# z3lx/waifu2x-tensorrt

Hardware: AMD Instinct MI355X
Metric: upscaled MPix/s, 1080p->4K swin_unet/art fp16 (higher is better)
Workload: dtype f16; 1 GPU; configs[2]: swin_unet/art scale4 noise3 batch4 tile256 fp16, 1920x1080 frame, blend=0.0625 (45 tiles, 12 batches); synthetic-weight graph of that architecture, frame resident in HBM; frames_per_rank=132, parallelism=frame-sharded x1, no collectives; timing barrier over gloo, mode=frames, tiles_per_network_pass=48, tile_groups_per_pass=2

## Files before the change

include/w2x/c_api.h:

```cpp
#ifndef W2X_C_API_H
#define W2X_C_API_H

#include <stddef.h>
#include <stdint.h>

#ifdef __cplusplus
extern "C" {
#endif

typedef struct w2x_engine w2x_engine;

enum { W2X_PRECISION_TF32 = 0, W2X_PRECISION_FP16 = 1, W2X_PRECISION_FP32 = 2 };

enum { W2X_RESIZE_BICUBIC = 0, W2X_RESIZE_BILINEAR = 1 };
enum { W2X_YUV_BT601 = 0, W2X_YUV_BT709 = 1, W2X_YUV_BT2020 = 2 };
enum { W2X_YUV_LIMITED = 0, W2X_YUV_FULL = 1 };

typedef struct w2x_build_config {
    int deviceId, precision;
    int minBatchSize, optBatchSize, maxBatchSize;
    int minChannels, optChannels, maxChannels;
    int minWidth, optWidth, maxWidth;
    int minHeight, optHeight, maxHeight;
} w2x_build_config;
// ... 17 lines not shown
int w2x_render(w2x_engine* e, const uint8_t* src, int rows, int cols, size_t src_step, uint8_t* dst, size_t dst_step);
int w2x_render16(w2x_engine* e, const uint16_t* src, int rows, int cols, size_t src_step, uint16_t* dst, size_t dst_step);
int w2x_render_resized(w2x_engine* e, const uint8_t* src, int rows, int cols, size_t src_step, uint8_t* dst, int dst_rows, int dst_cols, size_t dst_step, int filter);
int w2x_render16_resized(w2x_engine* e, const uint16_t* src, int rows, int cols, size_t src_step, uint16_t* dst, int dst_rows, int dst_cols, size_t dst_step, int filter);
int w2x_render_strip(w2x_engine* e, const uint8_t* src, int rows, int cols, size_t src_step, uint8_t* dst, size_t dst_step, int part, int parts);
int w2x_render_sharded(w2x_engine* const* engines, int count, const uint8_t* src, int rows, int cols, size_t src_step, uint8_t* dst, size_t dst_step);
int w2x_shard_plan(int in_w, int in_h, int out_w, int out_h, int tile_in, int tile_out, int scaling, double overlap_x, double overlap_y,
                   int part, int parts, int* out16);
int w2x_shard_compute(w2x_engine* e, const uint8_t* src, int rows, int cols, size_t src_step, int part, int parts);
const void* w2x_shard_slab(w2x_engine* e, size_t* bytes);
int w2x_shard_finish(w2x_engine* e, uint8_t* dst, int out_rows, int out_cols, size_t dst_step, int part, int parts, const void* const* slabs, const int* devices);
int w2x_ipc_export(const void* device_ptr, uint8_t* out64);
void* w2x_ipc_open(const uint8_t* handle64, int device);
void w2x_ipc_close(void* p);
int w2x_render_sequence(w2x_engine* e, const uint8_t* const* srcs, int rows, int cols, size_t src_step, uint8_t* const* dsts, size_t dst_step, int count);
int w2x_render_sequence_resized(w2x_engine* e, const uint8_t* const* srcs, int rows, int cols, size_t src_step, uint8_t* const* dsts, int dst_rows, int dst_cols, size_t dst_step,
                                int count, int filter);
int w2x_render_yuv(w2x_engine* e, const void* const* src_planes, const size_t* src_steps, int rows, int cols, int src_bits,
                   void* const* dst_planes, const size_t* dst_steps, int dst_rows, int dst_cols, int dst_bits, int matrix, int range);
int w2x_render_sequence_yuv(w2x_engine* e, const void* const* src_planes, const size_t* src_steps, int rows, int cols, int src_bits,
                            void* const* dst_planes, const size_t* dst_steps, int dst_rows, int dst_cols, int dst_bits, int count, int matrix, int range);
int w2x_render_yuv_resized(w2x_engine* e, const void* const* src_planes, const size_t* src_steps, int rows, int cols, int src_bits,
                           void* const* dst_planes, const size_t* dst_steps, int dst_rows, int dst_cols, int dst_bits, int matrix, int range, int filter);
int w2x_render_sequence_yuv_resized(w2x_engine* e, const void* const* src_planes, const size_t* src_steps, int rows, int cols, int src_bits,
                                    void* const* dst_planes, const size_t* dst_steps, int dst_rows, int dst_cols, int dst_bits, int count, int matrix, int range, int filter);
int w2x_render_rgba(w2x_engine* e, const uint8_t* src, int rows, int cols, size_t src_step, uint8_t* dst, size_t dst_step, int bleed, int skip_uniform_alpha);
int w2x_alpha_bleed_device(w2x_engine* e, const uint8_t* bgra, int rows, int cols, size_t bgra_step, uint8_t* bgr, size_t bgr_step, int radius);
void* w2x_alloc_host(w2x_engine* e, size_t bytes);
void w2x_free_host(w2x_engine* e, void* data);
int w2x_pin_host(w2x_engine* e, void* data, size_t bytes);
void w2x_unpin_host(w2x_engine* e, void* data);
int w2x_strip_plan(int in_w, int in_h, int out_w, int out_h, int tile_in, int tile_out, int scaling, double overlap_x, double overlap_y,
                   int part, int parts, int* out4);
int w2x_infer(w2x_engine* e, const float* input_nchw, float* output_nchw);
int w2x_output_tile_size(w2x_engine* e);
double w2x_plan_flops(w2x_engine* e);
int w2x_pass_tiles(w2x_engine* e);
float w2x_last_render_ms(w2x_engine* e);
float w2x_bench_resident(w2x_engine* e, int iters);
int w2x_resident_output(w2x_engine* e, void* dst, size_t bytes);
int w2x_profile_frame(w2x_engine* e, double* out, int cap);
int w2x_op_times(w2x_engine* e, double* out, int cap);

int w2x_calculate_tiles(int in_w, int in_h, int out_w, int out_h, int tile_in, int tile_out, int scaling,
                        double overlap_x, double overlap_y, int* in_rects, int* out_rects, int cap);
int w2x_tile_weights(int which, int overlap_x, int overlap_y, int size, float* out);
int w2x_resize_weights(int in, int out, int filter, int* first, float* weights, int cap);
int w2x_yuv_plane_sizes(int rows, int cols, int bits, int* plane_rows, int* plane_cols, size_t* plane_bytes);
int w2x_alpha_bleed(const uint8_t* bgr, size_t bgr_step, const uint8_t* alpha, size_t alpha_step, int rows, int cols, int radius, uint8_t* out, size_t out_step);
int w2x_describe_plan(const char* onnx_path, int batch, int tile, char* buf, size_t cap);
int w2x_describe_plan_precision(const char* onnx_path, int batch, int tile, int precision, char* buf, size_t cap);
int w2x_write_engine_file(const char* onnx_path, int batch, int tile, const char* out_path);
int w2x_validate_engine_file(const char* path, char* buf, size_t cap);
int w2x_device_pci_bus_id(int device, char* buf, size_t cap);
void w2x_sha256_hex(const void* data, size_t len, char* out);
const char* w2x_version(void);
int w2x_debug_set(const char* name, int value);

#ifdef __cplusplus
}
#endif
#endif
```

waifu2x-tensorrt_amd/__init__.py:

```python
from .engine import (BuildConfig, RenderConfig, Img2Img, Precision, Severity, lib, lib_path,
                     calculate_tiles, strip_plan, shard_plan, render_sharded, device_pci_bus_id, ipc_open, ipc_close, tile_weights, resize_weights, yuv_plane_sizes, alpha_bleed, describe_plan, write_engine_file, validate_engine_file, sha256_hex, W2xError,
                     debug_switches)

__all__ = ["BuildConfig", "RenderConfig", "Img2Img", "Precision", "Severity", "lib", "lib_path",
           "calculate_tiles", "strip_plan", "shard_plan", "render_sharded", "device_pci_bus_id", "ipc_open", "ipc_close", "tile_weights", "resize_weights", "yuv_plane_sizes", "alpha_bleed", "describe_plan", "write_engine_file", "validate_engine_file", "sha256_hex", "W2xError", "debug_switches"]
```

waifu2x-tensorrt_amd/csrc/c_api.cpp:

```cpp
#include "../../include/w2x/c_api.h"

#include <cstring>
#include <fstream>
#include <vector>
#include <string>

#include "../../include/w2x/img2img.h"
#include "lower.h"
#include "sha256.h"
#include "tiles.h"
#include "kernels.h"

struct w2x_engine {
    w2x::Img2Img engine;
    w2x_message_fn msg = nullptr; void* msg_user = nullptr;
    w2x_progress_fn prog = nullptr; void* prog_user = nullptr;
};

extern "C" {

w2x_engine* w2x_create(void) { try { return new w2x_engine; } catch (...) { return nullptr; } }
void w2x_destroy(w2x_engine* e) { delete e; }

void w2x_set_message_callback(w2x_engine* e, w2x_message_fn fn, void* user) {
    if (!e) return;
    e->msg = fn; e->msg_user = user;
    if (fn) e->engine.setMessageCallback([e](w2x::Severity s, const std::string& m) { if (e->msg) e->msg((int)s, m.c_str(), e->msg_user); });
    else e->engine.setMessageCallback(nullptr);
}
void w2x_set_progress_callback(w2x_engine* e, w2x_progress_fn fn, void* user) {
    if (!e) return;
    e->prog = fn; e->prog_user = user;
    if (fn) e->engine.setProgressCallback([e](int c, int t, double s) { if (e->prog) e->prog(c, t, s, e->prog_user); });
    else e->engine.setProgressCallback(nullptr);
}

int w2x_build(w2x_engine* e, const char* onnx_path, const w2x_build_config* c) {
    if (!e || !onnx_path || !c) return 0;
    w2x::BuildConfig b;
    b.deviceId = c->deviceId; b.precision = c->precision == W2X_PRECISION_FP16 ? w2x::Precision::FP16 : c->precision == W2X_PRECISION_FP32 ? w2x::Precision::FP32 : w2x::Precision::TF32;
    b.minBatchSize = c->minBatchSize; b.optBatchSize = c->optBatchSize; b.maxBatchSize = c->maxBatchSize;
    b.minChannels = c->minChannels; b.optChannels = c->optChannels; b.maxChannels = c->maxChannels;
    b.minWidth = c->minWidth; b.optWidth = c->optWidth; b.maxWidth = c->maxWidth;
    b.minHeight = c->minHeight; b.optHeight = c->optHeight; b.maxHeight = c->maxHeight;
    return e->engine.build(onnx_path, b) ? 1 : 0;
}

int w2x_load(w2x_engine* e, const char* onnx_path, const w2x_render_config* c) {
    if (!e || !onnx_path || !c) return 0;
    w2x::RenderConfig r;
    r.deviceId = c->deviceId; r.precision = c->precision == W2X_PRECISION_FP16 ? w2x::Precision::FP16 : c->precision == W2X_PRECISION_FP32 ? w2x::Precision::FP32 : w2x::Precision::TF32;
    r.batchSize = c->batchSize; r.channels = c->channels; r.height = c->height; r.width = c->width; r.scaling = c->scaling;
    r.overlapX = c->overlapX; r.overlapY = c->overlapY; r.tta = c->tta != 0; r.ttaBugCompat = c->ttaBugCompat != 0;
    return e->engine.load(onnx_path, r) ? 1 : 0;
}

int w2x_render(w2x_engine* e, const uint8_t* src, int rows, int cols, size_t src_step, uint8_t* dst, size_t dst_step) {
    if (!e) return 0;
    w2x::Image s; s.data = const_cast<uint8_t*>(src); s.rows = rows; s.cols = cols; s.step = src_step;
    w2x::Image d; d.data = dst; d.step = dst_step;
// ... 224 lines not shown
    memcpy(out, m.data(), m.size() * sizeof(float));
    return 1;
}

int w2x_describe_plan(const char* onnx_path, int batch, int tile, char* buf, size_t cap) { return w2x_describe_plan_precision(onnx_path, batch, tile, W2X_PRECISION_FP16, buf, cap); }

int w2x_describe_plan_precision(const char* onnx_path, int batch, int tile, int precision, char* buf, size_t cap) {
    std::string s; int ok = 1;
    try {
        w2x::Plan plan = w2x::build_plan(onnx_path, batch, 3, tile, tile, precision != W2X_PRECISION_FP16);
        plan.userB = batch;
        const auto bytes = plan.serialize();
        s = w2x::Plan::deserialize(bytes.data(), bytes.size()).describe();
    }
    catch (const std::exception& e) { s = std::string("ERROR: ") + e.what(); ok = 0; }
    if (buf && cap) { size_t n = s.size() < cap - 1 ? s.size() : cap - 1; memcpy(buf, s.data(), n); buf[n] = 0; }
    return ok;
}

int w2x_validate_engine_file(const char* path, char* buf, size_t cap) {
    std::string s = "ok"; int ok = 1;
    try {
        std::ifstream f(path, std::ios::binary | std::ios::ate);
        if (!f.is_open()) throw std::runtime_error("could not open engine file");
        std::vector<char> bytes((size_t)f.tellg());
        f.seekg(0); f.read(bytes.data(), (std::streamsize)bytes.size());
        (void)w2x::Plan::deserialize((const uint8_t*)bytes.data(), bytes.size());
    } catch (const std::exception& e) { s = e.what(); ok = 0; }
    if (buf && cap) { size_t n = s.size() < cap - 1 ? s.size() : cap - 1; memcpy(buf, s.data(), n); buf[n] = 0; }
    return ok;
}

int w2x_write_engine_file(const char* onnx_path, int batch, int tile, const char* out_path) {
    try {
        w2x::Plan plan = w2x::build_plan(onnx_path, batch, 3, tile, tile);
        plan.userB = batch;
        const auto bytes = plan.serialize();
        std::ofstream f(out_path, std::ios::binary);
        if (!f.is_open()) return 0;
        f.write((const char*)bytes.data(), (std::streamsize)bytes.size());
        return f.good() ? 1 : 0;
    } catch (const std::exception&) { return 0; }
}

int w2x_device_pci_bus_id(int device, char* buf, size_t cap) { return buf && cap >= 16 && w2x::device_pci_bus_id(device, buf, cap) ? 1 : 0; }

void w2x_sha256_hex(const void* data, size_t len, char* out) {
    std::string h = w2x::sha256_hex(data, len);
    memcpy(out, h.c_str(), 65);
}

const char* w2x_version(void) { return "w2x-hip 0.1 (gfx950)"; }

int w2x_debug_set(const char* name, int value) { return w2x::set_switch(name, value) ? 1 : 0; }

}
```

waifu2x-tensorrt_amd/csrc/engine.cpp:

```cpp
#include <hip/hip_runtime.h>
#include <dlfcn.h>

#include <algorithm>
#include <array>
#include <chrono>
#include <cmath>
#include <cstdio>
#include <cstdlib>
#include <cstring>
#include <deque>
#include <filesystem>
#include <fstream>
#include <map>
#include <sstream>
#include <tuple>

#include "../../include/w2x/img2img.h"
#include "common.h"
#include "fragorder.h"
#include "kernels.h"
#include "lower.h"
#include "plan.h"
#include "sha256.h"
#include "switches.h"
#include "tiles.h"

#define W2X_LOG(sev, message) impl->log(sev, message, __FUNCTION__, __LINE__)
#define W2X_LOG_AS(who, sev, message) impl->log(sev, message, who, __LINE__)

namespace w2x {

namespace {

inline void hipAssert(hipError_t e) {
    if (e != hipSuccess) throw std::runtime_error(hipGetErrorString(e));
}

std::string hipGetDeviceName(int deviceId) {
    hipDeviceProp_t prop{};
    hipAssert(hipGetDeviceProperties(&prop, deviceId));
    std::string arch = prop.gcnArchName;
    return arch + " x" + std::to_string(prop.multiProcessorCount);
}

int physical_device(int logical) {
    std::vector<int> map;
    if (const char* e = getenv("W2X_DEVICE_MAP")) { std::stringstream ss(e); std::string tok; while (std::getline(ss, tok, ',')) if (!tok.empty()) map.push_back(atoi(tok.c_str())); }
    return logical >= 0 && logical < (int)map.size() ? map[logical] : logical;
}

struct DeviceGuard {
    int prev = -1, dev = -1;
    explicit DeviceGuard(int d) : dev(d) {
        if (d < 0) return;
        if (hipGetDevice(&prev) != hipSuccess) { (void)hipGetLastError(); prev = -1; }
        if (prev != d) hipAssert(hipSetDevice(d));
    }
    ~DeviceGuard() { if (dev >= 0 && prev >= 0 && prev != dev) (void)hipSetDevice(prev); }
    DeviceGuard(const DeviceGuard&) = delete;
    DeviceGuard& operator=(const DeviceGuard&) = delete;
};

std::string device_ordinal_problem(int logical, int physical) {
    int count = 0;
    if (hipGetDeviceCount(&count) != hipSuccess) { (void)hipGetLastError(); count = 0; }
    if (count <= 0) return "no HIP device is visible to this process (hipGetDeviceCount = 0): this library has no CPU path";
    if (physical >= 0 && physical < count) return "";
    std::string m = "device id " + std::to_string(logical);
    if (physical != logical) m += " (W2X_DEVICE_MAP -> " + std::to_string(physical) + ")";
    return m + " does not exist: this process sees " + std::to_string(count) + " HIP device" + (count == 1 ? "" : "s") + " (valid ids 0.." + std::to_string(count - 1) + ")";
}

}
// ... 100 lines not shown
    MessageCallback messageCallback{};
    ProgressCallback progressCallback{};

    void log(Severity s, const std::string& m) { if (messageCallback) messageCallback(s, m); }
    void log(Severity s, const std::string& m, const std::string& fn, int line) { if (messageCallback) messageCallback(s, "[" + fn + "@" + std::to_string(line) + "] " + m); }
    void log(int current, int total, double speed) { if (progressCallback) progressCallback(current, total, speed); }

    bool loaded = false;
    int device = -1;
    bool poison = false;
    bool check_general = false;
    bool use_graphs = true;
    Plan plan;
    RenderConfig cfg;
    hipStream_t stream = nullptr;
    hipEvent_t ev0 = nullptr, ev1 = nullptr;
    int (*roctx_push)(const char*) = nullptr; int (*roctx_pop)() = nullptr;
    hipEvent_t ev_shard = nullptr;
    static constexpr int kMaxRenderParts = 4;
    hipEvent_t ev_part[kMaxRenderParts] = {nullptr, nullptr, nullptr, nullptr};
    int pipeline_parts = 3;
    size_t shard_halo_slots = 0;
    int shard_rows = 0, shard_cols = 0;
    hipStream_t gstream[3] = {nullptr, nullptr, nullptr};
    hipEvent_t ev_fork = nullptr, ev_join[3] = {nullptr, nullptr, nullptr};
    int groups = 2;
    std::vector<void*> tensors, blobs;
    std::vector<void*> frag_blobs;
    std::vector<void*> perm_blobs;
    std::vector<int> pool_blocks;
    void* arena_base = nullptr; size_t arena_bytes = 0;
    std::vector<GemmParams> gemm;
    int final_op = -1;
    enum LaunchKind { L_OP, L_HEAD, L_STEM, L_UP, L_MLP32, L_ATTN32 };
    struct Launch {
        LaunchKind kind = L_OP;
        int first = 0, last = 0;
        int timed = 0;
        double flops = 0;
        int family = 0;
        std::array<void*, 4> planes{{nullptr, nullptr, nullptr, nullptr}};
    };
    std::vector<Launch> launches;

    bool deep = false;
    uint8_t* d_frame = nullptr; size_t frame_cap = 0;
    uint8_t* d_out = nullptr; size_t out_cap = 0;
    void* d_slab = nullptr; size_t slab_cap = 0;
    void* d_slab2 = nullptr; size_t slab2_cap = 0;
    hipEvent_t ev_g0[2] = {nullptr, nullptr}, ev_cmp[2] = {nullptr, nullptr};
    bool rolling = false;
    bool rolling_ok = true;
    TileSlot* d_slots = nullptr; size_t slots_cap = 0;
    float *d_rampx = nullptr, *d_rampy = nullptr;
    int ovx = 0, ovy = 0;
    float* d_blob_in = nullptr; float* d_blob_out = nullptr;
    uint8_t* d_frame2 = nullptr; size_t frame2_cap = 0;
    uint8_t* d_out2 = nullptr; size_t out2_cap = 0;
    hipStream_t s_up = nullptr, s_dn = nullptr;
    hipEvent_t ev_up[2] = {nullptr, nullptr}, ev_comp[2] = {nullptr, nullptr}, ev_dn[2] = {nullptr, nullptr};
    float* d_canvas = nullptr; size_t canvas_cap = 0;
    struct ResizeTables {
        int inW = 0, inH = 0, outW = 0, outH = 0, filter = 0;
        int *fx = nullptr, *fy = nullptr; float *wx = nullptr, *wy = nullptr;
        int kx = 0, ky = 0, rows_max = 0;
    };
    std::deque<ResizeTables> rs_tables;
    const ResizeTables* rs = nullptr;
    struct YuvJob { YuvCoefs in, out; int in_bits = 8, out_bits = 8, key = 0; };
    const YuvJob* yuv = nullptr;
    uint8_t* d_bgr = nullptr; size_t bgr_cap = 0;
    uint8_t* d_alpha = nullptr; size_t alpha_cap = 0;
    unsigned* d_minmax = nullptr; unsigned* h_minmax = nullptr;
    hipEvent_t ev_minmax = nullptr;
    bool rgba = false;
    std::vector<void*> pinned;
    std::vector<void*> host_allocs;
    std::vector<TileSlot> h_slots;

    bool profiling = false;
    struct Stamp { int kind; hipEvent_t a, b; double flops; int op; };
    std::vector<double> op_ms;
    std::vector<Stamp> stamps;
    void stamp_begin(int kind, double flops, int op = -1) {
        if (!profiling) return;
        Stamp st{kind, nullptr, nullptr, flops, op};
        hipAssert(hipEventCreate(&st.a)); hipAssert(hipEventCreate(&st.b));
        hipAssert(hipEventRecord(st.a, stream));
        stamps.push_back(st);
    }
    void stamp_end() { if (profiling) hipAssert(hipEventRecord(stamps.back().b, stream)); }

    void ensure_copy_streams() {
        if (s_up) return;
        hipAssert(hipStreamCreateWithFlags(&s_up, hipStreamNonBlocking));
        hipAssert(hipStreamCreateWithFlags(&s_dn, hipStreamNonBlocking));
        for (int b = 0; b < 2; ++b) { hipAssert(hipEventCreateWithFlags(&ev_up[b], hipEventDisableTiming)); hipAssert(hipEventCreateWithFlags(&ev_comp[b], hipEventDisableTiming)); hipAssert(hipEventCreateWithFlags(&ev_dn[b], hipEventDisableTiming)); }
    }

    bool one_part_stale = false;
    void one_part_slots() {
        if (!one_part_stale) return;
        const int steps = cfg.tta ? 8 : 1, B = plan.B, S = plan.B / plan.userB;
        const int batchCount = (int)std::lround(std::ceil((double)(last_strip.tile_count * steps) / plan.userB));
        const size_t stepCount = (size_t)((batchCount + S - 1) / S) * B;
        h_slots.resize(stepCount);
        for (size_t st = 0; st < stepCount; ++st) {
            const int ti = (int)(st / steps), aug = (int)(st % steps);
            TileSlot sl{0, 0, aug, 0};
            if (ti < last_strip.tile_count) { sl.x = last_grid.in[last_strip.first_tile + ti].x; sl.y = last_grid.in[last_strip.first_tile + ti].y; sl.valid = 1; }
            h_slots[st] = sl;
        }
        ensure(d_slots, slots_cap, stepCount * sizeof(TileSlot));
        hipAssert(hipMemcpy(d_slots, h_slots.data(), stepCount * sizeof(TileSlot), hipMemcpyHostToDevice));
        ensure(d_slab, slab_cap, stepCount * plan.Tout * plan.Tout * 4 * plan.elt);
        one_part_stale = false;
    }
    int last_rows = 0, last_cols = 0, last_batches = 0;
    TileGrid last_grid;
    StripPlan last_strip;
    float last_ms = 0.f;

    static constexpr int kRgbaKey = 64;
    using GraphKey = std::tuple<const void*, const void*, const void*, const void*, int, int, int, int>;
    struct PassGraphs { hipGraphExec_t g[4] = {nullptr, nullptr, nullptr, nullptr}; int n = 0; };
    std::map<GraphKey, PassGraphs> graphs;
    std::map<GraphKey, int> graph_seen;
    long graph_replays = 0, eager_passes = 0;
    void drop_graphs() {
        for (auto& kv : graphs) for (int k = 0; k < kv.second.n; ++k) if (kv.second.g[k]) (void)hipGraphExecDestroy(kv.second.g[k]);
        graphs.clear(); graph_seen.clear();
    }

    ~Impl() {
        release();
        for (void* h : host_allocs) if (hipHostFree(h) != hipSuccess) (void)hipGetLastError();
    }

    void release() {
        std::unique_ptr<DeviceGuard> guard;
        if (device >= 0) { try { guard.reset(new DeviceGuard(device)); } catch (...) {} }
        drop_graphs();
        if (arena_base) { (void)hipFree(arena_base); arena_base = nullptr; }
        for (void* p : blobs) if (p) (void)hipFree(p);
        for (void* p : frag_blobs) if (p) (void)hipFree(p);
        frag_blobs.clear();
        for (void* p : perm_blobs) if (p) (void)hipFree(p);
        perm_blobs.clear();
        for (const Launch& L : launches) for (void* p : L.planes) if (p) (void)hipFree(p);
        launches.clear();
        tensors.clear(); blobs.clear(); gemm.clear();
        for (void* h : pinned) if (hipHostUnregister(h) != hipSuccess) (void)hipGetLastError();
        pinned.clear();
        for (hipEvent_t* e : {&ev_up[0], &ev_up[1], &ev_comp[0], &ev_comp[1], &ev_dn[0], &ev_dn[1]}) if (*e) { (void)hipEventDestroy(*e); *e = nullptr; }
        if (s_up) { (void)hipStreamDestroy(s_up); s_up = nullptr; }
        if (s_dn) { (void)hipStreamDestroy(s_dn); s_dn = nullptr; }
        frame2_cap = out2_cap = 0;
        for (ResizeTables& t : rs_tables) for (void* q : {(void*)t.fx, (void*)t.fy, (void*)t.wx, (void*)t.wy}) if (q) (void)hipFree(q);
        rs_tables.clear(); rs = nullptr;
        if (d_canvas) { (void)hipFree(d_canvas); d_canvas = nullptr; }
        canvas_cap = 0;
        for (void** q : {(void**)&d_bgr, (void**)&d_alpha, (void**)&d_minmax}) if (*q) { (void)hipFree(*q); *q = nullptr; }
        bgr_cap = alpha_cap = 0; rgba = false;
        if (h_minmax) { if (hipHostFree(h_minmax) != hipSuccess) (void)hipGetLastError(); h_minmax = nullptr; }
        if (ev_minmax) { (void)hipEventDestroy(ev_minmax); ev_minmax = nullptr; }
        for (void** p : {(void**)&d_frame, (void**)&d_out, (void**)&d_frame2, (void**)&d_out2, &d_slab, &d_slab2, (void**)&d_slots, (void**)&d_rampx, (void**)&d_rampy, (void**)&d_blob_in, (void**)&d_blob_out})
            if (*p) { (void)hipFree(*p); *p = nullptr; }
        frame_cap = out_cap = slab_cap = slab2_cap = slots_cap = 0;
        shard_rows = shard_cols = 0; shard_halo_slots = 0; rolling = false; one_part_stale = false;
        last_rows = last_cols = last_batches = 0;
        if (ev0) { (void)hipEventDestroy(ev0); ev0 = nullptr; }
        if (ev1) { (void)hipEventDestroy(ev1); ev1 = nullptr; }
        if (ev_shard) { (void)hipEventDestroy(ev_shard); ev_shard = nullptr; }
        for (hipEvent_t& e : ev_part) if (e) { (void)hipEventDestroy(e); e = nullptr; }
        for (hipEvent_t& e : ev_g0) if (e) { (void)hipEventDestroy(e); e = nullptr; }
        for (hipEvent_t& e : ev_cmp) if (e) { (void)hipEventDestroy(e); e = nullptr; }
        if (ev_fork) { (void)hipEventDestroy(ev_fork); ev_fork = nullptr; }
        for (hipEvent_t& e : ev_join) if (e) { (void)hipEventDestroy(e); e = nullptr; }
        for (hipStream_t& st : gstream) if (st) { (void)hipStreamDestroy(st); st = nullptr; }
        if (stream) { (void)hipStreamDestroy(stream); stream = nullptr; }
        loaded = false;
    }

    TView tview(const View& v) const {
        TView t;
        if (v.t < 0) return t;
        const TensorDesc& d = plan.tensors[v.t];
        t.p = tensors[v.t]; t.Hs = d.H; t.Ws = d.W; t.Cs = d.C; t.y0 = v.y0; t.x0 = v.x0;
        return t;
    }

    struct TensorUse { std::array<int, 6> rd; std::array<int, 3> wr; };
    static TensorUse tensor_use(const Op& op) {
        TensorUse u; u.rd.fill(-1); u.wr.fill(-1);
        switch (op.kind) {
            case OP_GEMM: u.rd = {{op.g.a.t, op.g.res.t, op.g.res2.t, op.g.stats_in, op.g.se_scale, op.g.res_scale}}; u.wr = {{op.g.out.t, op.g.stats_out, op.g.pool_out}}; break;
            case OP_ATTN: u.rd[0] = op.at.qkv; u.wr[0] = op.at.out; break;
            case OP_SE: u.rd[0] = op.se.pool; u.wr[0] = op.se.scale; break;
            case OP_SCALE_ADD: u.rd = {{op.se.pool, op.se.scale, -1, -1, -1, -1}}; u.wr[0] = op.se.pool; break;
            case OP_MLP: u.rd[0] = op.m.x; u.wr = {{op.m.y, op.m.stats_out, -1}}; break;
            case OP_SWINATTN: u.rd[0] = op.sa.x; u.wr = {{op.sa.y, op.sa.stats_out, -1}}; break;
            default: break;
        }
        return u;
    }
    struct Lifetimes { std::vector<int> first, last; };
    Lifetimes lifetimes(const std::vector<Launch>& ls) const {
        const int nops = (int)plan.ops.size();
        Lifetimes lt{std::vector<int>(plan.tensors.size(), nops), std::vector<int>(plan.tensors.size(), -1)};
        for (const Launch& L : ls)
            for (int i = L.first; i <= L.last; ++i) {
                const TensorUse u = tensor_use(plan.ops[i]);
                auto touch = [&](int t) { if (t >= 0) { lt.first[t] = std::min(lt.first[t], L.first); lt.last[t] = std::max(lt.last[t], L.last); } };
                for (int t : u.rd) touch(t);
                for (int t : u.wr) touch(t);
            }
        lt.first[plan.in_tensor] = -1;
        lt.last[plan.out_tensor] = nops;
        return lt;
    }
    static bool passes_on(const Lifetimes& lt, int t, int i) { return t >= 0 && lt.first[t] == i && lt.last[t] == i + 1; }
// ... 190 lines not shown
            if (op.kind != OP_GEMM) continue;
            const GemmOp& g = op.g;
            GemmParams& p = gemm[i];
            p.a = tview(g.a); p.amode = g.amode; p.kh = g.kh; p.kw = g.kw; p.stride = g.stride;
            p.B = plan.B; p.Mrows = g.Mrows; p.aW = g.aW;
            p.win_table = g.win_table >= 0 ? (const int*)blobs[g.win_table] : nullptr;
            p.K = g.K; p.N = g.N; p.Kw = round_up(g.K, 8);
            p.wt = blobs[g.w]; p.wt_frag = frag_blobs[g.w]; p.wt_perm = perm_blobs[g.w]; p.bias = (const float*)blobs[g.bias];
            p.ln = g.ln; p.csum = g.csum >= 0 ? (const float*)blobs[g.csum] : nullptr;
            p.stats_in = g.stats_in >= 0 ? (const float*)tensors[g.stats_in] : nullptr;
            p.act = g.act; p.alpha = g.alpha; p.has_clip = g.has_clip; p.clip_lo = g.clip_lo; p.clip_hi = g.clip_hi;
            p.res = tview(g.res); p.res2 = tview(g.res2); p.out = tview(g.out);
            p.omode = g.omode; p.r = g.r; p.Cout = g.Cout;
            p.stats_out = g.stats_out >= 0 ? (float*)tensors[g.stats_out] : nullptr; p.ln_eps = g.ln_eps;
            p.pool_out = g.pool_out >= 0 ? (float*)tensors[g.pool_out] : nullptr;
            p.a_scale = g.se_scale >= 0 ? (const float*)tensors[g.se_scale] : nullptr;
            p.res_scale = g.res_scale >= 0 ? (const float*)tensors[g.res_scale] : nullptr;
            if ((p.a_scale || p.res_scale) && plan.elt != 2) throw std::runtime_error("plan: folded gates in an fp32 plan");
            if (g.out.t == plan.out_tensor) final_op = (int)i;
            if (p.ln && (!p.stats_in || !p.csum)) throw std::runtime_error("plan: LayerNorm op without statistics");
            if (p.stats_out && p.Cout != p.out.Cs) throw std::runtime_error("plan: statistics over padded rows");
            if (p.pool_out && p.omode != O_ROWS) throw std::runtime_error("plan: pooling on a scattered output");
            if (p.omode == O_PIXSHUF && p.N != p.r * p.r * p.out.Cs) throw std::runtime_error("plan: pixel-shuffle width mismatch");
            if (p.omode != O_PIXSHUF && p.N != p.out.Cs) throw std::runtime_error("plan: output width mismatch");
            if ((p.amode == A_WIN || p.omode == O_WIN) && !p.win_table) throw std::runtime_error("plan: missing window table");
            if (p.a.Cs != 4 && (p.a.Cs % 8)) throw std::runtime_error("plan: unaligned input channels");
        }
        if (final_op < 0) throw std::runtime_error("plan: the output tensor is not produced by a fused op");
        auto head_supported = [&](const GemmParams& g) {
            return g.wt_frag && g.out.Cs == 4 && g.a.y0 == 0 && g.a.x0 == 0 && g.a.Ws == g.aW && (long)g.a.Hs * g.a.Ws == g.Mrows && g.Mrows % 32 == 0 && g.aW >= 32 && pixgemm_supported(g) &&
                   (!g.has_clip || (f16_to_f32(f32_to_f16(g.clip_lo)) == g.clip_lo && f16_to_f32(f32_to_f16(g.clip_hi)) == g.clip_hi));
        };
        launches.clear();
        for (const Launch& L : candidates) {
            const GemmParams& p = gemm[L.last]; const GemmParams& q = gemm[L.first];
            const bool ok = L.kind == L_HEAD ? head_supported(p) : L.kind == L_STEM ? conv48_stem_supported(p, q) || conv3_stem_supported(p, q) : L.kind == L_UP ? conv3_up_supported(p, q) : true;
            if (ok) launches.push_back(L);
            else for (int i = L.first; i <= L.last; ++i) launches.push_back(launch(L_OP, i, i));
        }
        for (Launch& L : launches)
            if (L.kind == L_MLP32 || L.kind == L_ATTN32) {
                const GemmOp& g1 = plan.ops[L.first].g; const GemmOp& g2 = plan.ops[L.last].g;
                upload_planes(plan.blobs[g1.w].data, g1.N, g1.K, L.planes[0], L.planes[1]);
                upload_planes(plan.blobs[g2.w].data, g2.N, g2.K, L.planes[2], L.planes[3]);
            }
        hipAssert(hipStreamSynchronize(stream));
    }

    int ng_now = 1;
    size_t arena_part() const { return ((arena_bytes / ng_now) + 255) / 256 * 256; }
    uint8_t* group_ptr(const void* full, int grp) const {
        return full ? (uint8_t*)arena_base + (size_t)grp * arena_part() + (size_t)((const uint8_t*)full - (const uint8_t*)arena_base) / ng_now : nullptr;
    }
    void run_network(void* out_override, int live = -1, int grp = -1, hipStream_t s = nullptr) {
        if (!s) s = stream;
        const int cap = grp < 0 ? plan.B : plan.B / ng_now;
        if (live < 0 || live > cap) live = cap;
        auto tp = [&](int t) -> uint8_t* { return t < 0 ? nullptr : grp < 0 ? (uint8_t*)tensors[t] : group_ptr(tensors[t], grp); };
        auto gp = [&](int i) {
            GemmParams p = gemm[i];
            p.B = live;
            if (grp >= 0) {
                auto shift = [&](auto*& ptr) { ptr = (std::remove_reference_t<decltype(ptr)>)group_ptr(ptr, grp); };
                shift(p.a.p); shift(p.res.p); shift(p.res2.p); shift(p.out.p); shift(p.stats_in); shift(p.stats_out); shift(p.pool_out); shift(p.a_scale); shift(p.res_scale);
            }
            if (i == final_op && out_override) p.out.p = out_override;
            return p;
        };
        for (const Launch& L : launches) try {
            const Op& op = plan.ops[L.first];
            struct Range { Impl* e; bool on; ~Range() { if (on) e->roctx_pop(); } } range{this, roctx_push != nullptr};
            if (range.on) roctx_push(launch_label(L).c_str());
            auto issue = [&](auto&& f) { stamp_begin(L.family, L.flops, L.timed); hipAssert(f()); stamp_end(); };
            switch (L.kind) {
                case L_HEAD: {
                    const GemmParams g = gp(L.last);
                    MlpParams p = mlp_params(op, live, tp);
                    p.ti_w = g.wt_frag; p.ti_b = g.bias; p.ti_out = g.out.p; p.ti_Hs = g.out.Hs; p.ti_Ws = g.out.Ws; p.ti_Mrows = g.Mrows; p.ti_aW = g.aW;
                    p.ti_clip = g.has_clip; p.ti_lo = g.clip_lo; p.ti_hi = g.clip_hi;
                    issue([&] { return launch_mlp(p, s); });
                    break;
                }
                case L_STEM: case L_UP: {
                    const GemmParams p = gp(L.last), q = gp(L.first);
                    issue([&] { return L.kind == L_UP ? launch_conv3_up(p, q, s) : q.N == 48 ? launch_conv48_stem(p, q, s) : launch_conv3_stem(p, q, s); });
                    break;
                }
                case L_MLP32: {
                    const GemmParams p = gp(L.first), q = gp(L.last);
                    Mlp32Params m;
                    m.x = (const float*)p.a.p; m.y = (float*)q.out.p; m.M = (long)live * p.Mrows; m.C = p.K; m.stats_in = p.stats_in;
                    m.w1h = L.planes[0]; m.w1l = L.planes[1]; m.w2h = L.planes[2]; m.w2l = L.planes[3];
                    m.b1 = p.bias; m.b2 = q.bias; m.stats_out = q.stats_out; m.eps_out = q.ln_eps;
                    issue([&] { return launch_mlp32(m, s); });
                    break;
                }
                case L_ATTN32: {
                    const GemmParams p = gp(L.first), q = gp(L.last);
                    const AttnOp& a = plan.ops[L.first + 1].at;
                    SwinAttn32Params m;
                    m.x = (const float*)p.a.p; m.y = (float*)q.out.p; m.res = (const float*)q.res.p; m.B = live; m.nwin = a.nwin; m.C = p.K; m.pix_per_item = p.Mrows;
                    m.table_in = p.win_table; m.table_out = q.win_table; m.stats_in = p.stats_in;
                    m.wqkv_h = L.planes[0]; m.wqkv_l = L.planes[1]; m.wproj_h = L.planes[2]; m.wproj_l = L.planes[3];
                    m.bqkv = p.bias; m.bproj = q.bias; m.scale = a.scale; m.bias = (const float*)blobs[a.bias]; m.maskid = (const int*)blobs[a.maskid];
                    m.stats_out = q.stats_out; m.eps_out = q.ln_eps;
                    issue([&] { return launch_swinattn32(m, s); });
                    break;
                }
                case L_OP: switch (op.kind) {
                    case OP_GEMM: {
                        const GemmParams p = gp(L.first);
                        if (op.g.pool_out >= 0) pool_blocks[op.g.pool_out] = plan.elt == 2 && conv3_supported(p) ? conv3_tiles(p) : 0;
                        issue([&] { return plan.elt == 4 ? launch_gemm_f32(p, s, cfg.precision == Precision::FP32) : pixgemm_supported(p) ? launch_pixgemm(p, s) : conv3_supported(p) ? launch_conv3(p, s) : conv3h_supported(p) ? launch_conv3h(p, s) : conv48_supported(p) ? launch_conv48(p, s) : stem_supported(p) ? launch_stem(p, s) : launch_gemm(p, s); });
                        if (check_general && plan.elt == 2 && (pixgemm_supported(p) || conv3_supported(p) || conv3h_supported(p) || conv48_supported(p) || stem_supported(p))) check_against_general(p, L.first, live);
                        break;
                    }
                    case OP_ATTN: {
                        const AttnOp& a = op.at;
                        AttnParams p;
                        p.qkv = tp(a.qkv); p.out = tp(a.out); p.B = live; p.nwin = a.nwin; p.heads = a.heads; p.hd = a.hd;
                        p.ntok = a.ws * a.ws; p.scale = a.scale; p.bias = blobs[a.bias]; p.maskid = (const int*)blobs[a.maskid];
                        issue([&] { return plan.elt == 4 ? launch_attn_f32(p, s) : launch_attn(p, s); });
                        break;
                    }
                    case OP_SWINATTN: {
                        const SwinAttnOp& a = op.sa;
                        const TensorDesc& d = plan.tensors[a.x];
                        SwinAttnParams p;
                        p.x = tp(a.x); p.y = tp(a.y); p.table = (const int*)blobs[a.table]; p.H = a.H; p.W = a.W; p.ry = a.ry; p.rx = a.rx; p.B = live; p.nwin = a.nwin; p.C = a.C; p.hd = a.hd;
                        p.wqkv = blobs[a.wqkv]; p.bqkv = (const float*)blobs[a.bqkv]; p.scale = a.scale; p.bias32 = (const float*)blobs[a.bias]; p.maskid = (const int*)blobs[a.maskid];
                        p.wproj = blobs[a.wproj]; p.bproj = (const float*)blobs[a.bproj]; p.eps = a.eps;
                        p.wqkv_frag = frag_blobs[a.wqkv]; p.wproj_frag = frag_blobs[a.wproj];
                        p.stats_out = (float*)tp(a.stats_out); p.eps_out = a.eps_out;
                        if (d.C != a.C || plan.tensors[a.y].C != a.C || d.H * d.W != a.nwin * a.ws * a.ws) throw std::runtime_error("plan: attention geometry mismatch");
                        issue([&] { return launch_swin_attn(p, s); });
                        break;
                    }
                    case OP_MLP: {
                        const MlpParams p = mlp_params(op, live, tp);
                        issue([&] { return launch_mlp(p, s); });
                        break;
                    }
                    case OP_SE: {
                        const SeOp& se = op.se;
                        SeParams p;
                        p.pool = (const float*)tp(se.pool); p.scale = (float*)tp(se.scale); p.B = live; p.C = se.C;
                        p.Cs = plan.tensors[se.pool].C; p.Cmid = se.Cmid; p.inv_count = se.inv_count; p.nblocks = pool_blocks[se.pool] > 0 ? pool_blocks[se.pool] : se.nblocks; p.Mrows = se.Mrows;
                        p.w1 = (const float*)blobs[se.w1]; p.b1 = (const float*)blobs[se.b1]; p.w2 = (const float*)blobs[se.w2]; p.b2 = (const float*)blobs[se.b2];
                        issue([&] { return launch_se(p, s); });
                        break;
                    }
                    case OP_SCALE_ADD: {
                        const TensorDesc& d = plan.tensors[op.se.pool];
                        issue([&] { return launch_scale(tp(op.se.pool), (const float*)tp(op.se.scale), live, d.H * d.W, d.C, plan.elt == 4, s); });
                        break;
                    }
                    default: throw std::runtime_error("plan: unknown op kind");
                }
            }
        } catch (const std::exception& e) {
            throw std::runtime_error("op " + launch_label(L) + ": " + e.what());
        }
    }
    std::string launch_label(const Launch& L) const {
        std::string m = std::to_string(L.first) + (L.last > L.first ? "-" + std::to_string(L.last) : "") + " [";
        for (int i = L.first; i <= L.last; ++i) m += (i > L.first ? " + " : "") + plan.ops[i].name;
        return m + "]";
    }
    template <class TP> MlpParams mlp_params(const Op& op, int live, const TP& tp) const {
        const MlpOp& m = op.m;
        const TensorDesc& d = plan.tensors[m.x];
        MlpParams p;
        p.x = tp(m.x); p.y = tp(m.y); p.M = (long)live * d.H * d.W; p.C = m.C;
        p.w1 = blobs[m.w1]; p.b1 = (const float*)blobs[m.b1]; p.w2 = blobs[m.w2]; p.b2 = (const float*)blobs[m.b2];
        p.w1_frag = frag_blobs[m.w1]; p.w2_frag = frag_blobs[m.w2]; p.frag32 = mlp_frag32(m.C);
        p.eps = m.eps; p.stats_out = (float*)tp(m.stats_out); p.eps_out = m.eps_out;
        if (d.C != m.C || plan.tensors[m.y].C != m.C) throw std::runtime_error("plan: MLP width mismatch");
        return p;
    }
    void check_against_general(const GemmParams& p, int i, int live) {
        const Op& op = plan.ops[i];
        const TensorDesc& od = plan.tensors[op.g.out.t];
        const size_t n = (size_t)live * od.H * od.W * od.C;
        std::vector<uint16_t> a(n), b(n);
        void* tmp = nullptr;
        hipAssert(hipMalloc(&tmp, n * 2));
        hipAssert(hipStreamSynchronize(stream));
        hipAssert(hipMemcpy(a.data(), p.out.p, n * 2, hipMemcpyDeviceToHost));
        hipAssert(hipMemcpy(tmp, p.out.p, n * 2, hipMemcpyDeviceToDevice));
        GemmParams q = p; q.out.p = tmp; q.pool_out = nullptr;
        hipAssert(launch_gemm(q, stream));
        hipAssert(hipStreamSynchronize(stream));
        hipAssert(hipMemcpy(b.data(), tmp, n * 2, hipMemcpyDeviceToHost));
        hipAssert(hipFree(tmp));
        double md = 0; size_t at = 0, bad = 0;
        for (size_t k = 0; k < n; ++k) { const double d = std::fabs(f16_to_f32(a[k]) - f16_to_f32(b[k])); if (d > 0.01) ++bad; if (d > md) { md = d; at = k; } }
        log(Severity::warn, "pixgemm check op " + std::to_string(i) + " [" + op.name + "]: max|d|=" + std::to_string(md) + " at pixel " + std::to_string(at / od.C) +
            " ch " + std::to_string(at % od.C) + " (x=" + std::to_string(at / od.C % od.W) + ", y=" + std::to_string(at / od.C / od.W % od.H) + "), " + std::to_string(bad) + " of " + std::to_string(n) + " off by > 0.01");
    }

    template <class T> void ensure(T*& p, size_t& cap, size_t bytes) {
        if (bytes <= cap) return;
        drop_graphs();
        if (p) hipAssert(hipFree(p));
        p = nullptr; cap = 0;
        hipAssert(hipMalloc((void**)&p, bytes));
        cap = bytes;
    }

    void run_frame(int rows, int cols, const TileGrid& grid, bool report, const StripPlan& sp) {
        run_passes(rows, cols, sp.tile_count, 0, report, 0, true);
        if (rs) { compose_canvas(rows, cols, grid, stream); if (yuv) resample_yuv(stream); else resample(stream); return; }
        if (yuv) { compose_yuv(rows, cols, grid, stream); return; }
        compose_rect(rows, cols, grid, sp.x0, sp.x1, 0, 0, sp.first_tile);
    }

    bool can_roll(int tile_count) const {
        const int steps = cfg.tta ? 8 : 1, B = plan.B;
        const int last_live = tile_count * steps - (tile_count * steps - 1) / B * B;
        return rolling_ok && groups == 2 && use_graphs && !profiling && !check_general && !poison && gstream[0] && last_live >= 8 && B % 2 == 0;
    }
    void run_rolling_frame(int rows, int cols, const TileGrid& grid, const StripPlan& sp, int which, hipEvent_t out_free) {
        for (int k = 0; k < 2; ++k) {
            if (!ev_g0[k]) hipAssert(hipEventCreateWithFlags(&ev_g0[k], hipEventDisableTiming));
            if (!ev_cmp[k]) hipAssert(hipEventCreateWithFlags(&ev_cmp[k], hipEventDisableTiming));
        }
        struct Swap { Impl* e; void* slab; size_t cap; bool on; ~Swap() { if (on) { std::swap(e->d_slab, e->d_slab2); std::swap(e->slab_cap, e->slab2_cap); } e->rolling = false; } } sw{this, d_slab, slab_cap, which == 1};
        if (which == 1) { std::swap(d_slab, d_slab2); std::swap(slab_cap, slab2_cap); }
        rolling = true;
// ... 23 lines not shown
    void run_passes(int rows, int cols, int tile_count, size_t slab_slot0, bool report, size_t slots_off, bool fresh, int batch0 = 0, int batch_total = 0, int pass0 = 0, int pass1 = -1) {
        const int B = plan.B, T = plan.T, To = plan.Tout;
        const int steps = cfg.tta ? 8 : 1;
        const int userB = plan.userB, S = B / userB;
        const int batchCount = (int)std::lround(std::ceil((double)(tile_count * steps) / userB));
        const int passCount = (batchCount + S - 1) / S;
        const size_t slot_bytes = (size_t)To * To * 4 * plan.elt;
        if (poison && fresh) {
            hipAssert(hipMemsetAsync(arena_base, 0x7E, arena_bytes, stream));
            hipAssert(hipMemsetAsync(d_slab, 0x7E, slab_cap, stream));
        }
        const bool graphable = use_graphs && !profiling && !check_general;
        for (int bi = pass0; bi < (pass1 < 0 ? passCount : std::min(pass1, passCount)); ++bi) {
            const auto t0 = std::chrono::steady_clock::now();
            const int live = std::max(0, std::min(B, tile_count * steps - bi * B));
            void* const slab_out = (uint8_t*)d_slab + (slab_slot0 + (size_t)bi * B) * slot_bytes;
            GatherParams gp0;
            gp0.frame = d_frame; gp0.rows = rows; gp0.cols = cols; gp0.step = (size_t)cols * 3 * (deep ? 2 : 1); gp0.deep = deep ? 1 : 0;
            gp0.out = tensors[plan.in_tensor]; gp0.slots = d_slots + slots_off + (size_t)bi * B; gp0.B = B; gp0.T = T; gp0.fp32 = plan.elt == 4;
            const int NG = groups;
            struct NgReset { int& r; ~NgReset() { r = 1; } } ng_reset{ng_now};
            ng_now = NG;
            const bool split = NG > 1 && !profiling && !check_general && live >= 4 * NG && B % NG == 0 && (size_t)NG * arena_part() <= arena_bytes + 1024;
            ng_now = 1;
            int first[5] = {0, 0, 0, 0, 0};
            for (int grp = 0; grp < NG; ++grp) first[grp + 1] = first[grp] + live / NG + (grp < live % NG ? 1 : 0);
            if (split) {
                if (!ev_fork) hipAssert(hipEventCreateWithFlags(&ev_fork, hipEventDisableTiming));
                for (int k = 0; k + 1 < NG; ++k) if (!gstream[k]) {
                    hipAssert(hipStreamCreateWithFlags(&gstream[k], hipStreamNonBlocking));
                    hipAssert(hipEventCreateWithFlags(&ev_join[k], hipEventDisableTiming));
                }
            }
            auto group_stream = [&](int grp) { return grp ? gstream[grp - 1] : stream; };
            auto gather = [&](const GatherParams& gp, hipStream_t gs) {
                if (rgba) {
                    GatherRgbaParams rp;
                    rp.bgr = d_bgr; rp.bgr_step = (size_t)cols * 3; rp.alpha = d_alpha; rp.alpha_step = (size_t)cols; rp.rows = rows; rp.cols = cols;
                    rp.out = gp.out; rp.fp32 = gp.fp32; rp.slots = gp.slots; rp.B = gp.B; rp.T = gp.T;
                    hipAssert(launch_gather_rgba(rp, gs));
                    return;
                }
                if (!yuv) { hipAssert(launch_gather(gp, gs)); return; }
                GatherYuvParams yp;
                yp.src = yuv_layout(d_frame, rows, cols, yuv->in_bits); yp.k = yuv->in;
                yp.out = gp.out; yp.fp32 = gp.fp32; yp.slots = gp.slots; yp.B = gp.B; yp.T = gp.T;
                hipAssert(launch_gather_yuv(yp, gs));
            };
            auto gather_group = [&](int grp, hipStream_t gs) {
                GatherParams gp = gp0;
                gp.out = group_ptr(tensors[plan.in_tensor], grp); gp.slots = gp0.slots + (size_t)first[grp]; gp.B = first[grp + 1] - first[grp];
                gather(gp, gs);
            };
            auto network_group = [&](int grp, hipStream_t gs) { run_network((uint8_t*)slab_out + (size_t)first[grp] * slot_bytes, first[grp + 1] - first[grp], grp, gs); };
            auto fork = [&] { hipAssert(hipEventRecord(ev_fork, stream)); for (int grp = 1; grp < NG; ++grp) hipAssert(hipStreamWaitEvent(gstream[grp - 1], ev_fork, 0)); };
            auto join = [&] { for (int grp = 1; grp < NG; ++grp) { hipAssert(hipEventRecord(ev_join[grp - 1], gstream[grp - 1])); hipAssert(hipStreamWaitEvent(stream, ev_join[grp - 1], 0)); } };
            auto run_pass = [&] {
                if (!split) {
                    stamp_begin(3, 0);
                    gather(gp0, stream);
                    stamp_end();
                    run_network(slab_out, live);
                    return;
                }
                ng_now = NG;
                for (int grp = 0; grp < NG; ++grp) gather_group(grp, stream);
                fork();
                for (int grp = 0; grp < NG; ++grp) network_group(grp, group_stream(grp));
                join();
                ng_now = 1;
            };
            auto run_group = [&](int grp) { ng_now = NG; gather_group(grp, group_stream(grp)); network_group(grp, group_stream(grp)); ng_now = 1; };
            const bool per_group = split;
            const bool no_join = rolling && split;
            auto run_eager = [&] { if (per_group) { fork(); for (int grp = 0; grp < NG; ++grp) run_group(grp); if (!no_join) join(); } else { if (rolling && gstream[0]) { join(); } run_pass(); } };
            if (!graphable) run_eager();
            else {
                const GraphKey key{d_frame, d_slots + slots_off + (size_t)bi * B, slab_out, arena_base, rows, cols, live, rgba ? kRgbaKey : yuv ? yuv->key : deep ? 1 : 0};
                auto replay = [&](const PassGraphs& pg) {
                    if (pg.n == 1) { if (rolling && gstream[0]) join(); hipAssert(hipGraphLaunch(pg.g[0], stream)); return; }
                    fork();
                    for (int grp = 0; grp < pg.n; ++grp) hipAssert(hipGraphLaunch(pg.g[grp], group_stream(grp)));
                    if (!no_join) join();
                };
                auto it = graphs.find(key);
                if (it != graphs.end()) { replay(it->second); ++graph_replays; }
                else if (graph_seen.size() >= 4096 && !graph_seen.count(key)) { graph_seen.clear(); run_eager(); ++eager_passes; }
                else if (graph_seen[key]++ == 0 && !(rolling && !graphs.empty())) { run_eager(); ++eager_passes; }
                else {
                    if (graphs.size() >= 1024) drop_graphs();
                    PassGraphs pg;
                    std::string why;
                    const int ncap = per_group ? NG : 1;
                    for (int c = 0; c < ncap && why.empty(); ++c) {
                        hipStream_t cs = per_group ? group_stream(c) : stream;
                        hipGraph_t graph = nullptr; hipGraphExec_t exec = nullptr;
                        hipError_t ge = hipStreamBeginCapture(cs, hipStreamCaptureModeThreadLocal);
                        if (ge != hipSuccess) { why = std::string("begin capture: ") + hipGetErrorString(ge); break; }
                        try { if (per_group) run_group(c); else run_pass(); } catch (const std::exception& e) { why = std::string("capture: ") + e.what(); }
                        ge = hipStreamEndCapture(cs, &graph);
                        if (why.empty() && ge != hipSuccess) why = std::string("end capture: ") + hipGetErrorString(ge);
                        if (why.empty()) { ge = hipGraphInstantiate(&exec, graph, nullptr, nullptr, 0); if (ge != hipSuccess) why = std::string("instantiation: ") + hipGetErrorString(ge); }
                        if (graph) (void)hipGraphDestroy(graph);
                        if (why.empty()) pg.g[pg.n++] = exec;
                    }
                    if (!why.empty()) {
                        (void)hipGetLastError();
                        for (int c = 0; c < pg.n; ++c) (void)hipGraphExecDestroy(pg.g[c]);
                        use_graphs = false;
                        log(Severity::warn, "hipGraph " + why + " - passes stay on plain launches");
                        run_eager(); ++eager_passes;
                    } else {
                        graphs[key] = pg;
                        replay(pg); ++graph_replays;
                    }
// ... 40 lines not shown
        ComposeYuvParams yp;
        ComposeParams& cp = yp.c;
        cp.tiles = d_slab; cp.fp32 = plan.elt == 4;
        cp.outW = cols * cfg.scaling; cp.outH = rows * cfg.scaling; cp.To = To;
        cp.nx = grid.nx; cp.ny = grid.ny; cp.stride_x = To - grid.outOvX; cp.stride_y = To - grid.outOvY;
        const bool overlapping = cfg.overlapX != 0 || cfg.overlapY != 0;
        cp.ovx = overlapping ? ovx : 0; cp.ovy = overlapping ? ovy : 0;
        cp.ramp_x = d_rampx; cp.ramp_y = d_rampy; cp.tta = cfg.tta ? 1 : 0; cp.tta_bug_compat = cfg.ttaBugCompat ? 1 : 0;
        yp.dst = yuv_layout(d_out, cp.outH, cp.outW, yuv->out_bits); yp.k = yuv->out;
        stamp_begin(4, 0);
        hipAssert(launch_compose_yuv(yp, on));
        stamp_end();
    }
    void upload_and_bleed(const Image& src, int radius) {
        const int rows = src.rows, cols = src.cols;
        ensure(d_frame, frame_cap, (size_t)rows * cols * 4);
        ensure(d_bgr, bgr_cap, (size_t)rows * cols * 3);
        ensure(d_alpha, alpha_cap, (size_t)rows * cols);
        if (!d_minmax) hipAssert(hipMalloc((void**)&d_minmax, 2 * sizeof(unsigned)));
        hipAssert(hipMemcpy2DAsync(d_frame, (size_t)cols * 4, src.data, src.step, (size_t)cols * 4, rows, hipMemcpyHostToDevice, stream));
        hipAssert(hipMemsetAsync(d_minmax, 0, 2 * sizeof(unsigned), stream));
        AlphaBleedParams bp;
        bp.bgra = d_frame; bp.step = (size_t)cols * 4; bp.rows = rows; bp.cols = cols; bp.radius = radius;
        bp.bgr = d_bgr; bp.bgr_step = (size_t)cols * 3; bp.alpha = d_alpha; bp.alpha_step = (size_t)cols; bp.minmax = d_minmax;
        hipAssert(launch_alpha_bleed(bp, stream));
    }
    void compose_rgba(int rows, int cols, const TileGrid& grid, size_t alpha_slot0, bool uniform, unsigned value) {
        const int To = plan.Tout;
        ComposeRgbaParams rp;
        ComposeParams& cp = rp.c;
        cp.tiles = d_slab; cp.fp32 = plan.elt == 4; cp.dst = d_out; cp.dst_step = (size_t)cols * cfg.scaling * 4;
        cp.outW = cols * cfg.scaling; cp.outH = rows * cfg.scaling; cp.To = To;
        cp.nx = grid.nx; cp.ny = grid.ny; cp.stride_x = To - grid.outOvX; cp.stride_y = To - grid.outOvY;
        const bool overlapping = cfg.overlapX != 0 || cfg.overlapY != 0;
        cp.ovx = overlapping ? ovx : 0; cp.ovy = overlapping ? ovy : 0;
        cp.ramp_x = d_rampx; cp.ramp_y = d_rampy; cp.tta = cfg.tta ? 1 : 0; cp.tta_bug_compat = cfg.ttaBugCompat ? 1 : 0;
        rp.alpha_tiles = uniform ? nullptr : (const uint8_t*)d_slab + alpha_slot0 * (size_t)To * To * 4 * plan.elt;
        rp.alpha_value = value;
        hipAssert(launch_compose_rgba(rp, stream));
    }
    void sequence_slots(const TileGrid& grid, const StripPlan& sp) {
        const int steps = cfg.tta ? 8 : 1, B = plan.B, S = plan.B / plan.userB;
        const int batchCount = (int)std::lround(std::ceil((double)(sp.tile_count * steps) / plan.userB));
        const int stepCount = ((batchCount + S - 1) / S) * B;
        h_slots.resize(stepCount);
        for (int st = 0; st < stepCount; ++st) {
            int ti = st / steps, aug = st % steps;
            TileSlot sl{0, 0, aug, 0};
            if (ti < sp.tile_count) { sl.x = grid.in[ti].x; sl.y = grid.in[ti].y; sl.valid = 1; }
            h_slots[st] = sl;
        }
        ensure(d_slots, slots_cap, (size_t)stepCount * sizeof(TileSlot));
        hipAssert(hipMemcpyAsync(d_slots, h_slots.data(), (size_t)stepCount * sizeof(TileSlot), hipMemcpyHostToDevice, stream));
        ensure(d_slab, slab_cap, (size_t)stepCount * plan.Tout * plan.Tout * 4 * plan.elt);
        hipAssert(hipStreamSynchronize(stream));
    }
    template <class Up, class Down>
    float run_sequence(int count, int rows, int cols, const TileGrid& grid, const StripPlan& sp, const Up& up, const Down& down) {
        uint8_t* const frames[2] = {d_frame, d_frame2};
        uint8_t* const outs[2] = {d_out, d_out2};
        struct Restore { Impl* im; uint8_t* f; uint8_t* o; ~Restore() { im->d_frame = f; im->d_out = o; } } restore{this, frames[0], outs[0]};
        const bool roll = count > 1 && can_roll(sp.tile_count);
        if (roll) ensure(d_slab2, slab2_cap, slab_cap);
        hipAssert(hipStreamSynchronize(stream));
        hipAssert(hipEventRecord(ev0, stream));
        for (int i = 0; i < count; ++i) {
            const int b = i & 1;
            if (i >= 2) hipAssert(hipStreamWaitEvent(s_up, ev_comp[b], 0));
            up(i, frames[b], s_up);
            hipAssert(hipEventRecord(ev_up[b], s_up));
            hipAssert(hipStreamWaitEvent(stream, ev_up[b], 0));
            d_frame = frames[b]; d_out = outs[b];
            if (roll) {
                run_rolling_frame(rows, cols, grid, sp, b, i >= 2 ? ev_dn[b] : nullptr);
                hipAssert(hipEventRecord(ev_comp[b], gstream[0]));
            } else {
                if (i >= 2) hipAssert(hipStreamWaitEvent(stream, ev_dn[b], 0));
                run_frame(rows, cols, grid, false, sp);
                hipAssert(hipEventRecord(ev_comp[b], stream));
            }
            hipAssert(hipStreamWaitEvent(s_dn, ev_comp[b], 0));
            down(i, outs[b], s_dn);
            hipAssert(hipEventRecord(ev_dn[b], s_dn));
        }
        if (roll) end_rolling();
        hipAssert(hipEventRecord(ev1, stream));
        hipAssert(hipStreamSynchronize(s_dn));
        hipAssert(hipStreamSynchronize(stream));
        hipAssert(hipStreamSynchronize(s_up));
        float total_ms = 0.f;
        hipAssert(hipEventElapsedTime(&total_ms, ev0, ev1));
        return total_ms;
    }
    static YuvPlanes yuv_layout(uint8_t* base, int rows, int cols, int bits) {
        const size_t bps = bits > 8 ? 2 : 1;
        const int cw = (cols + 1) / 2, ch = (rows + 1) / 2;
        YuvPlanes f;
        f.rows = rows; f.cols = cols; f.bits = bits;
        f.step[0] = ((size_t)cols * bps + 15) / 16 * 16; f.step[1] = f.step[2] = ((size_t)cw * bps + 15) / 16 * 16;
        f.p[0] = base; f.p[1] = base + f.step[0] * rows; f.p[2] = f.p[1] + f.step[1] * ch;
        return f;
    }
    static size_t yuv_bytes(int rows, int cols, int bits) { const YuvPlanes f = yuv_layout(nullptr, rows, cols, bits); return f.step[0] * rows + 2 * f.step[1] * ((rows + 1) / 2); }
    void resample(hipStream_t on) {
        ResampleParams rp;
        rp.canvas = d_canvas; rp.inW = rs->inW; rp.inH = rs->inH;
// ... 268 lines not shown
        impl->ensure_canvas((size_t)rows * s * cols * s * 3 * sizeof(float));
    }
    impl->deep = bps == 2;
    TileGrid grid = calculate_tiles(cols, rows, cols * s, rows * s, plan.T, plan.T, plan.Tout, plan.Tout, s, cfg.overlapX, cfg.overlapY);
    if (grid.count <= 0) { W2X_LOG_AS(who, error, "Tile grid is empty."); return false; }
    for (const Rect& r : grid.out) if (r.w <= 0 || r.h <= 0) { W2X_LOG_AS(who, error, "Tile grid does not fit the output (scaling does not match the model)."); return false; }
    const StripPlan sp = strip_plan(grid, cols * s, plan.Tout, part, parts);
    if (sp.tile_count == 0) return true;
    const int steps = cfg.tta ? 8 : 1, B = plan.B, S = plan.B / plan.userB;
    constexpr int kMaxParts = Impl::kMaxRenderParts;
    int npart = 1;
    int first_of[kMaxParts + 1] = {0, sp.tile_count, 0, 0, 0};
    if (parts == 1 && !resized && impl->pipeline_parts > 1 && sp.tile_count >= 16 && grid.outOvX < plan.Tout - grid.outOvX && grid.outOvY < plan.Tout - grid.outOvY) {
        int q = 1; while ((q * steps) % plan.userB) ++q;
        const int want = std::min({impl->pipeline_parts, kMaxParts, sp.tile_count / 8});
        int n = 0;
        const int body = want >= 2 ? (sp.tile_count - std::max(8, sp.tile_count / 5)) / q * q : 0;
        for (int k = 1; k < want; ++k) {
            const int t = k + 1 == want ? body : (int)((long)k * body / (want - 1)) / q * q;
            if (t > first_of[n] && t < sp.tile_count) first_of[++n] = t;
        }
        first_of[++n] = sp.tile_count;
        npart = n;
    }
    int tiles_of[kMaxParts] = {}, batches_of[kMaxParts] = {}, batches_before[kMaxParts] = {};
    size_t slots_off[kMaxParts] = {}; size_t stepTotal = 0; int batch_total = 0;
    for (int k = 0; k < npart; ++k) {
        tiles_of[k] = first_of[k + 1] - first_of[k];
        batches_of[k] = (int)std::lround(std::ceil((double)(tiles_of[k] * steps) / plan.userB));
        batches_before[k] = batch_total; batch_total += batches_of[k];
        slots_off[k] = stepTotal;
        stepTotal += (size_t)((batches_of[k] + S - 1) / S) * B;
    }
    int x_split = cols;
    if (npart > 1) {
        int xm = 0;
        for (int t = 0; t < first_of[1]; ++t) xm = std::max(xm, grid.in[sp.first_tile + t].x + plan.T);
        if (xm > 0 && xm < cols - 64) x_split = xm;
    }
    hipAssert(hipMemcpy2DAsync(impl->d_frame, (size_t)cols * 3 * bps, src.data, src.step, (size_t)x_split * 3 * bps, rows, hipMemcpyHostToDevice, stream));
    impl->h_slots.resize(stepTotal);
    for (int k = 0; k < npart; ++k) {
        const int t0 = first_of[k];
        const size_t n = (k + 1 < npart ? slots_off[k + 1] : stepTotal) - slots_off[k];
        for (size_t st = 0; st < n; ++st) {
            const int ti = (int)(st / steps), aug = (int)(st % steps);
            TileSlot sl{0, 0, aug, 0};
            if (ti < tiles_of[k]) { sl.x = grid.in[sp.first_tile + t0 + ti].x; sl.y = grid.in[sp.first_tile + t0 + ti].y; sl.valid = 1; }
            impl->h_slots[slots_off[k] + st] = sl;
        }
    }
    impl->ensure(impl->d_slots, impl->slots_cap, stepTotal * sizeof(TileSlot));
    hipAssert(hipMemcpyAsync(impl->d_slots, impl->h_slots.data(), stepTotal * sizeof(TileSlot), hipMemcpyHostToDevice, stream));
    const size_t one_part_steps = (size_t)(((int)std::lround(std::ceil((double)(sp.tile_count * steps) / plan.userB)) + S - 1) / S) * B;
    impl->ensure(impl->d_slab, impl->slab_cap, std::max((size_t)first_of[npart - 1] * steps + (stepTotal - slots_off[npart - 1]), one_part_steps) * plan.Tout * plan.Tout * 4 * plan.elt);

    hipAssert(hipEventRecord(impl->ev0, stream));
    if (npart == 1) {
        impl->run_frame(rows, cols, grid, true, sp);
        hipAssert(hipEventRecord(impl->ev1, stream));
        const int dx0 = resized ? 0 : sp.x0, dx1 = resized ? dst.cols : sp.x1;
        hipAssert(hipMemcpy2DAsync(dst.data + (size_t)dx0 * 3 * bps, dst.step, impl->d_out + (size_t)dx0 * 3 * bps, (size_t)dst.cols * 3 * bps, (size_t)(dx1 - dx0) * 3 * bps, dst.rows, hipMemcpyDeviceToHost, stream));
        hipAssert(hipStreamSynchronize(stream));
    } else {
        impl->ensure_copy_streams();
        for (int k = 0; k < npart; ++k) if (!impl->ev_part[k]) hipAssert(hipEventCreateWithFlags(&impl->ev_part[k], hipEventDisableTiming));
        ShardPlan part_plan[kMaxParts];
        for (int k = 0; k < npart; ++k) {
            ShardPlan q; q.first_tile = first_of[k]; q.tile_count = tiles_of[k];
            const int sx = plan.Tout - grid.outOvX, sy = plan.Tout - grid.outOvY;
            auto x_of = [&](int i) { return i >= grid.nx ? cols * s : i * sx; };
            auto y_of = [&](int j) { return j >= grid.ny ? rows * s : j * sy; };
            auto add = [&](int i0, int i1, int j0, int j1) { if (i0 < i1 && j0 < j1) q.rect[q.nrect++] = Rect{x_of(i0), y_of(j0), x_of(i1) - x_of(i0), y_of(j1) - y_of(j0)}; };
            const int t0 = q.first_tile, t1 = t0 + q.tile_count;
            const int c0 = t0 / grid.ny, r0 = t0 % grid.ny, c1 = t1 / grid.ny, r1 = t1 % grid.ny;
            if (c0 == c1) add(c0, c0 + 1, r0, r1);
            else { int full0 = c0; if (r0) { add(c0, c0 + 1, r0, grid.ny); full0 = c0 + 1; } add(full0, c1, 0, grid.ny); if (r1) add(c1, c1 + 1, 0, r1); }
            part_plan[k] = q;
        }
        hipStream_t dn = impl->s_up;
        auto download_part = [&](int k) {
            hipAssert(hipStreamWaitEvent(dn, impl->ev_part[k], 0));
            for (int r = 0; r < part_plan[k].nrect; ++r) {
                const Rect& rc = part_plan[k].rect[r];
                hipAssert(hipMemcpy2DAsync(dst.data + (size_t)rc.y * dst.step + (size_t)rc.x * 3 * bps, dst.step, impl->d_out + ((size_t)rc.y * dst.cols + rc.x) * 3 * bps, (size_t)dst.cols * 3 * bps,
                                           (size_t)rc.w * 3 * bps, rc.h, hipMemcpyDeviceToHost, dn));
            }
        };
        bool roll = true;
        for (int k = 0; k < npart; ++k) roll = roll && impl->can_roll(tiles_of[k]);
        struct Unroll { Impl* e; ~Unroll() { e->rolling = false; } } unroll{impl.get()};
        if (roll) for (int k = 0; k < 2; ++k) if (!impl->ev_g0[k]) hipAssert(hipEventCreateWithFlags(&impl->ev_g0[k], hipEventDisableTiming));
        for (int k = 0; k < npart; ++k) {
            if (k == 1 && x_split < cols) hipAssert(hipStreamWaitEvent(stream, impl->ev_up[0], 0));
            impl->rolling = roll;
            impl->run_passes(rows, cols, tiles_of[k], (size_t)first_of[k] * steps, true, slots_off[k], k == 0, batches_before[k], batch_total);
            impl->rolling = false;
            if (k == 0 && x_split < cols) {
                hipAssert(hipMemcpy2DAsync(impl->d_frame + (size_t)x_split * 3 * bps, (size_t)cols * 3 * bps, src.data + (size_t)x_split * 3 * bps, src.step, (size_t)(cols - x_split) * 3 * bps, rows,
                                           hipMemcpyHostToDevice, impl->s_dn));
                hipAssert(hipEventRecord(impl->ev_up[0], impl->s_dn));
            }
            hipStream_t cs = stream;
            if (roll) {
                cs = impl->gstream[0];
                hipAssert(hipEventRecord(impl->ev_g0[k & 1], stream));
                hipAssert(hipStreamWaitEvent(cs, impl->ev_g0[k & 1], 0));
            }
            for (int r = 0; r < part_plan[k].nrect; ++r) {
                const Rect& rc = part_plan[k].rect[r];
                impl->compose_rect(rows, cols, grid, rc.x, rc.x + rc.w, rc.y, rc.y + rc.h, 0, cs);
            }
            hipAssert(hipEventRecord(impl->ev_part[k], cs));
            if (k + 1 == npart) { if (roll) impl->end_rolling(); hipAssert(hipEventRecord(impl->ev1, stream)); }
        }
        for (int k = 0; k < npart; ++k) download_part(k);
        hipAssert(hipStreamSynchronize(dn));
        hipAssert(hipStreamSynchronize(stream));
    }
    hipAssert(hipEventElapsedTime(&impl->last_ms, impl->ev0, impl->ev1));
    impl->last_rows = rows; impl->last_cols = cols; impl->last_grid = grid; impl->last_strip = sp;
    impl->one_part_stale = npart > 1;
    if (resized) impl->last_rows = impl->last_cols = 0;
    if (parts == 1 && impl->slab2_cap < impl->slab_cap && impl->can_roll(sp.tile_count)) impl->ensure(impl->d_slab2, impl->slab2_cap, impl->slab_cap);
    return true;
} catch (const std::exception& e) {
    impl->drain_after_error();
    W2X_LOG_AS(who, error, "Render failed unexpectedly: " + std::string(e.what()) + ".");
    return false;
}

struct ShardPeer { const void* slab = nullptr; size_t halo_slots = 0; int device = -1; hipEvent_t ev = nullptr; int first_tile = 0, tile_count = 0; };

static void shard_phase1(Img2Img::Impl& e, const Image& src, const TileGrid& grid, const ShardPlan& sp, bool report) {
    const int rows = src.rows, cols = src.cols, s = e.cfg.scaling, steps = e.cfg.tta ? 8 : 1;
    const size_t slot_bytes = (size_t)e.plan.Tout * e.plan.Tout * 4 * e.plan.elt;
    e.deep = false;
    e.ensure(e.d_frame, e.frame_cap, (size_t)rows * cols * 3);
    e.ensure(e.d_out, e.out_cap, (size_t)rows * s * cols * s * 3);
    hipAssert(hipMemcpy2DAsync(e.d_frame, (size_t)cols * 3, src.data, src.step, (size_t)cols * 3, rows, hipMemcpyHostToDevice, e.stream));
    const int B = e.plan.B, S = e.plan.B / e.plan.userB;
    const int batchCount = (int)std::lround(std::ceil((double)(sp.tile_count * steps) / e.plan.userB));
    const int stepCount = ((batchCount + S - 1) / S) * B;
    e.h_slots.resize(stepCount);
    for (int st = 0; st < stepCount; ++st) {
        const int ti = st / steps, aug = st % steps;
        TileSlot sl{0, 0, aug, 0};
        if (ti < sp.tile_count) { sl.x = grid.in[sp.first_tile + ti].x; sl.y = grid.in[sp.first_tile + ti].y; sl.valid = 1; }
        e.h_slots[st] = sl;
    }
    e.ensure(e.d_slots, e.slots_cap, (size_t)stepCount * sizeof(TileSlot));
    hipAssert(hipMemcpyAsync(e.d_slots, e.h_slots.data(), (size_t)stepCount * sizeof(TileSlot), hipMemcpyHostToDevice, e.stream));
    e.shard_halo_slots = (size_t)(sp.first_tile - sp.halo_first) * steps;
    e.ensure(e.d_slab, e.slab_cap, (e.shard_halo_slots + (size_t)stepCount) * slot_bytes);
    hipAssert(hipEventRecord(e.ev0, e.stream));
    e.run_passes(rows, cols, sp.tile_count, e.shard_halo_slots, report, 0, true);
    if (!e.ev_shard) hipAssert(hipEventCreateWithFlags(&e.ev_shard, hipEventDisableTiming));
    hipAssert(hipEventRecord(e.ev_shard, e.stream));
}

static void shard_phase2(Img2Img::Impl& e, int k, const std::vector<ShardPlan>& sp, const std::vector<ShardPeer>& peers, const TileGrid& grid, int rows, int cols, Image& dst) {
    const int steps = e.cfg.tta ? 8 : 1, To = e.plan.Tout;
    const size_t px = (size_t)4 * e.plan.elt, slot_bytes = (size_t)To * To * px;
    const bool overlapping = e.cfg.overlapX != 0 || e.cfg.overlapY != 0;
    int waited = -1;
    bool peer2d = true;
    for (int g = sp[k].halo_first; g < sp[k].first_tile && overlapping; ++g) {
        int q = k - 1;
        while (q >= 0 && !(sp[q].tile_count > 0 && g >= sp[q].first_tile && g < sp[q].first_tile + sp[q].tile_count)) --q;
        if (q < 0 || !peers[q].slab) throw std::runtime_error("shard plan: tile " + std::to_string(g) + " has no owner");
        const ShardPeer& o = peers[q];
        if (q != waited) {
            if (o.ev) hipAssert(hipStreamWaitEvent(e.stream, o.ev, 0));
            waited = q;
            peer2d = o.device == e.device;
            if (!peer2d) {
                int can = 0;
                if (o.device >= 0 && hipDeviceCanAccessPeer(&can, e.device, o.device) == hipSuccess && can) {
                    const hipError_t pe = hipDeviceEnablePeerAccess(o.device, 0);
                    peer2d = pe == hipSuccess || pe == hipErrorPeerAccessAlreadyEnabled;
                }
                (void)hipGetLastError();
            }
        }
        for (int a = 0; a < steps; ++a) {
            const uint8_t* from = (const uint8_t*)o.slab + (o.halo_slots + (size_t)(g - sp[q].first_tile) * steps + a) * slot_bytes;
            uint8_t* to = (uint8_t*)e.d_slab + ((size_t)(g - sp[k].halo_first) * steps + a) * slot_bytes;
            if (!peer2d) {
                if (o.device >= 0) hipAssert(hipMemcpyPeerAsync(to, e.device, from, o.device, slot_bytes, e.stream));
                else hipAssert(hipMemcpyAsync(to, from, slot_bytes, hipMemcpyDefault, e.stream));
                continue;
            }
            int bx = std::min(To, grid.outOvX), by = std::min(To, grid.outOvY);
            if (steps > 1) bx = by = std::max(bx, by);
            const size_t pitch = (size_t)To * px;
            auto cols_band = [&](int x0) { if (bx > 0) hipAssert(hipMemcpy2DAsync(to + (size_t)x0 * px, pitch, from + (size_t)x0 * px, pitch, (size_t)bx * px, To, hipMemcpyDeviceToDevice, e.stream)); };
            auto rows_band = [&](int y0) { if (by > 0) hipAssert(hipMemcpyAsync(to + (size_t)y0 * pitch, from + (size_t)y0 * pitch, (size_t)by * pitch, hipMemcpyDeviceToDevice, e.stream)); };
            cols_band(To - bx); rows_band(To - by);
            if (steps > 1) { cols_band(0); rows_band(0); }
        }
    }
    for (int r = 0; r < sp[k].nrect; ++r) {
        const Rect& rc = sp[k].rect[r];
        e.compose_rect(rows, cols, grid, rc.x, rc.x + rc.w, rc.y, rc.y + rc.h, sp[k].halo_first);
    }
// ... 280 lines not shown
    const float total_ms = impl->run_sequence(count, rows, cols, grid, sp,
        [&](int i, uint8_t* dev, hipStream_t on) { copy_planes(srcs[i], dev, rows, cols, true, on); },
        [&](int i, uint8_t* dev, hipStream_t on) { copy_planes(dsts[i], dev, out_rows, out_cols, false, on); });
    impl->last_ms = total_ms / count;
    impl->last_rows = impl->last_cols = 0;
    return true;
} catch (const std::exception& e) {
    impl->drain_after_error();
    W2X_LOG_AS(who, error, "Render failed unexpectedly: " + std::string(e.what()) + ".");
    return false;
}

bool Img2Img::renderRgba(const Image& src, Image& dst, const RgbaOptions& opt) try {
    const char* who = "renderRgba";
    if (!impl->loaded) { W2X_LOG_AS(who, error, "Render called before a successful load."); return false; }
    DeviceGuard guard(impl->device);
    const RenderConfig& cfg = impl->cfg;
    const Plan& plan = impl->plan;
    const int rows = src.rows, cols = src.cols, s = cfg.scaling;
    if (src.depth != 8 || dst.depth != 8) { W2X_LOG_AS(who, error, "RGBA input and output images must be 8-bit."); return false; }
    if (!src.data || rows <= 0 || cols <= 0 || src.step < (size_t)cols * 4) { W2X_LOG_AS(who, error, "Input image is empty or has an invalid step."); return false; }
    if (!dst.data || dst.rows != rows * s || dst.cols != cols * s || dst.step < (size_t)dst.cols * 4) {
        W2X_LOG_AS(who, error, "Output image has invalid size: expected " + std::to_string(cols * s) + "x" + std::to_string(rows * s) + ".");
        return false;
    }
    if (opt.bleed < 0 || opt.bleed > kBleedMaxRadius) { W2X_LOG_AS(who, error, "Alpha bleed radius " + std::to_string(opt.bleed) + " is not in [0, " + std::to_string(kBleedMaxRadius) + "]."); return false; }
    hipStream_t stream = impl->stream;
    TileGrid grid = calculate_tiles(cols, rows, cols * s, rows * s, plan.T, plan.T, plan.Tout, plan.Tout, s, cfg.overlapX, cfg.overlapY);
    if (grid.count <= 0) { W2X_LOG_AS(who, error, "Tile grid is empty."); return false; }
    for (const Rect& r : grid.out) if (r.w <= 0 || r.h <= 0) { W2X_LOG_AS(who, error, "Tile grid does not fit the output (scaling does not match the model)."); return false; }
    const int steps = cfg.tta ? 8 : 1, B = plan.B, S = plan.B / plan.userB, N = grid.count;
    auto batches_of = [&](int tiles) { return (int)std::lround(std::ceil((double)(tiles * steps) / plan.userB)); };
    const size_t stepTotal = (size_t)((batches_of(2 * N) + S - 1) / S) * B;
    struct RgbaScope { Impl* im; ~RgbaScope() { im->rgba = false; } } rgba_scope{impl.get()};
    impl->deep = false;
    impl->last_rows = impl->last_cols = 0;
    impl->ensure(impl->d_out, impl->out_cap, (size_t)dst.rows * dst.cols * 4);
    impl->upload_and_bleed(src, opt.bleed);
    if (opt.skipUniformAlpha) {
        if (!impl->h_minmax) hipAssert(hipHostMalloc((void**)&impl->h_minmax, 2 * sizeof(unsigned), hipHostMallocDefault));
        if (!impl->ev_minmax) hipAssert(hipEventCreateWithFlags(&impl->ev_minmax, hipEventDisableTiming));
        hipAssert(hipMemcpyAsync(impl->h_minmax, impl->d_minmax, 2 * sizeof(unsigned), hipMemcpyDeviceToHost, stream));
        hipAssert(hipEventRecord(impl->ev_minmax, stream));
    }
    impl->h_slots.resize(stepTotal);
    for (size_t st = 0; st < stepTotal; ++st) {
        const int ti = (int)(st / steps), aug = (int)(st % steps);
        TileSlot sl{0, 0, aug, 0};
        if (ti < 2 * N) { sl.x = grid.in[ti % N].x; sl.y = grid.in[ti % N].y; sl.valid = ti < N ? kSlotColour : kSlotAlpha; }
        impl->h_slots[st] = sl;
    }
    impl->ensure(impl->d_slots, impl->slots_cap, stepTotal * sizeof(TileSlot));
    hipAssert(hipMemcpyAsync(impl->d_slots, impl->h_slots.data(), stepTotal * sizeof(TileSlot), hipMemcpyHostToDevice, stream));
    impl->ensure(impl->d_slab, impl->slab_cap, stepTotal * plan.Tout * plan.Tout * 4 * plan.elt);
    impl->one_part_stale = false;
    hipAssert(hipEventRecord(impl->ev0, stream));
    impl->rgba = true;
    bool uniform = false; unsigned value = 255;
    if (!opt.skipUniformAlpha) impl->run_passes(rows, cols, 2 * N, 0, true, 0, true);
    else {
        const int F = N * steps / B;
        const auto t0 = std::chrono::steady_clock::now();
        impl->run_passes(rows, cols, 2 * N, 0, false, 0, true, 0, 0, 0, F);
        hipAssert(hipEventSynchronize(impl->ev_minmax));
        uniform = impl->h_minmax[0] + impl->h_minmax[1] == 255u;
        value = impl->h_minmax[0];
        const int tiles = uniform ? N : 2 * N, batchCount = batches_of(tiles);
        const double ms = std::chrono::duration<double, std::milli>(std::chrono::steady_clock::now() - t0).count();
        for (int k = 0; k < std::min(F * S, batchCount); ++k) impl->log(k + 1, batchCount, 1000.0 * F * S / std::max(ms, 1e-6));
        impl->run_passes(rows, cols, tiles, 0, true, 0, false, 0, 0, F, -1);
    }
    impl->compose_rgba(rows, cols, grid, (size_t)N * steps, uniform, value);
    hipAssert(hipEventRecord(impl->ev1, stream));
    hipAssert(hipMemcpy2DAsync(dst.data, dst.step, impl->d_out, (size_t)dst.cols * 4, (size_t)dst.cols * 4, dst.rows, hipMemcpyDeviceToHost, stream));
    hipAssert(hipStreamSynchronize(stream));
    hipAssert(hipEventElapsedTime(&impl->last_ms, impl->ev0, impl->ev1));
    return true;
} catch (const std::exception& e) {
    impl->drain_after_error();
    W2X_LOG_AS("renderRgba", error, "Render failed unexpectedly: " + std::string(e.what()) + ".");
    return false;
}

bool Img2Img::alphaBleed(const Image& bgra, Image& bgr, int radius) try {
    const char* who = "alphaBleed";
    if (!impl->loaded) { W2X_LOG_AS(who, error, "Alpha bleed called before a successful load."); return false; }
    DeviceGuard guard(impl->device);
    const int rows = bgra.rows, cols = bgra.cols;
    if (bgra.depth != 8 || bgr.depth != 8) { W2X_LOG_AS(who, error, "RGBA input and output images must be 8-bit."); return false; }
    if (!bgra.data || rows <= 0 || cols <= 0 || bgra.step < (size_t)cols * 4) { W2X_LOG_AS(who, error, "Input image is empty or has an invalid step."); return false; }
    if (!bgr.data || bgr.rows != rows || bgr.cols != cols || bgr.step < (size_t)cols * 3) { W2X_LOG_AS(who, error, "Output image has invalid size: expected " + std::to_string(cols) + "x" + std::to_string(rows) + "."); return false; }
    if (radius < 0 || radius > kBleedMaxRadius) { W2X_LOG_AS(who, error, "Alpha bleed radius " + std::to_string(radius) + " is not in [0, " + std::to_string(kBleedMaxRadius) + "]."); return false; }
    impl->last_rows = impl->last_cols = 0;
    impl->upload_and_bleed(bgra, radius);
    hipAssert(hipMemcpy2DAsync(bgr.data, bgr.step, impl->d_bgr, (size_t)cols * 3, (size_t)cols * 3, rows, hipMemcpyDeviceToHost, impl->stream));
    hipAssert(hipStreamSynchronize(impl->stream));
    return true;
} catch (const std::exception& e) {
    impl->drain_after_error();
    W2X_LOG_AS("alphaBleed", error, "Alpha bleed failed unexpectedly: " + std::string(e.what()) + ".");
    return false;
}

void* Img2Img::allocHost(size_t bytes) try {
    if (!bytes) return nullptr;
    std::unique_ptr<DeviceGuard> guard;
// ... 132 lines not shown
```

waifu2x-tensorrt_amd/csrc/k_mlp2.hip:

```cpp
#include "kernels.h"
#ifndef W2X_GELU_DEG
#define W2X_GELU_DEG 4
#endif

#include <cstdlib>

#ifndef W2X_MLP192_TT
#define W2X_MLP192_TT 2
#endif
#ifndef W2X_MLP192_NW
#define W2X_MLP192_NW 4
#endif
#ifndef W2X_MLP192_WPS
#define W2X_MLP192_WPS 2
#endif
#ifndef W2X_MLP192_KEEP
#define W2X_MLP192_KEEP 0
#endif

namespace w2x {
namespace {

typedef _Float16 half8 __attribute__((ext_vector_type(8)));
typedef _Float16 half2v __attribute__((ext_vector_type(2)));
// ... 63 lines not shown
}

#define W2X_PHASE_FENCE() asm volatile("" ::: "memory")
#define W2X_RING_FENCE() asm volatile("" ::: "memory")

#ifndef W2X_MLP2Q_PIPE
#define W2X_MLP2Q_PIPE 0
#endif
#ifndef W2X_MLP2Q_EXP
#define W2X_MLP2Q_EXP 0
#endif
#ifndef W2X_MLP2Q_EARLY0
#define W2X_MLP2Q_EARLY0 0
#endif
#ifndef W2X_MLP2Q_SPLITACC
#define W2X_MLP2Q_SPLITACC 0
#endif
template <int C, int TT, int NW>
struct Mlp2Cfg {
    static constexpr int RW = 16 * TT;
    static constexpr int NWV = NW;
    static constexpr int BM = NWV * RW;
    static constexpr int LDX = C + 8;
    static constexpr int PPR = C / 8;
    static constexpr int KS = C / 32;
    static constexpr int NT = C / 16;
    static constexpr int NCH = 2 * C / 32;
    static constexpr int NP = RW * PPR / 64;
    static constexpr int SLAB = RW * LDX * 2;
    static constexpr int NF = 2 * KS + NT;
    static constexpr int WBUF = NF * 1024;
    static constexpr int RING = 6;
    static constexpr bool KEEP = C == 96 || (W2X_MLP192_KEEP && NW != 4);
    static constexpr int WORK = KEEP ? NWV * SLAB + 2 * WBUF : (NWV * SLAB > 2 * WBUF ? NWV * SLAB : 2 * WBUF);
    static constexpr int BIAS_OFF = WORK;
    static constexpr int SMEM = WORK + 3 * C * 4;
    static_assert(NF % NWV == 0 && NF % RING == 0 && 2 * KS >= RING, "fragments per wave / ring slots");
    static_assert(RW * PPR % 64 == 0, "flat piece count");
};

template <int C, int TT, int NW>
__global__ __launch_bounds__(NW * 64, (C == 96 ? 3 : W2X_MLP192_WPS) * NW / 4) void mlp2_kernel(const MlpParams p) {
    using K = Mlp2Cfg<C, TT, NW>;
    constexpr int RW = K::RW, LDX = K::LDX, PPR = K::PPR, KS = K::KS, NT = K::NT, NCH = K::NCH, NP = K::NP, NF = K::NF, RING = K::RING;
    constexpr int NFW = NF / K::NWV;

    extern __shared__ __attribute__((aligned(16))) unsigned char smem[];
    const int tid = threadIdx.x, lane = tid & 63;
    const int wv = __builtin_amdgcn_readfirstlane(tid >> 6);
    const int fr = lane & 15, g = lane >> 4;
    _Float16* Xw = (_Float16*)(smem + wv * K::SLAB);
    unsigned char* const WBb = smem + (K::KEEP ? K::NWV * K::SLAB : 0);

    const long row0 = ((long)blockIdx.x * K::NWV + wv) * RW;
    const long nrows = p.M - row0 < RW ? p.M - row0 : RW;
    const unsigned xbytes = (unsigned)(p.M * (C * 2));
    const __amdgpu_buffer_rsrc_t XB = __builtin_amdgcn_make_buffer_rsrc(const_cast<void*>(p.x), 0, xbytes, 0x00020000);
    const __amdgpu_buffer_rsrc_t YB = __builtin_amdgcn_make_buffer_rsrc(p.y, 0, xbytes, 0x00020000);
    const unsigned vo = nrows > 0 ? (unsigned)row0 * (C * 2) + lane * 16u : 0xFFFFC000u;
    const _Float16* __restrict__ W1 = (const _Float16*)p.w1_frag + lane * 8;
    const _Float16* __restrict__ W2 = (const _Float16*)p.w2_frag + lane * 8;

    auto frag_src = [&](int ch, int f) { return f < 2 * KS ? W1 + (size_t)(ch * 2 * KS + f) * 512 : W2 + (size_t)(ch * NT + (f - 2 * KS)) * 512; };
    auto stage = [&](int ch) {
#pragma unroll
        for (int i = 0; i < NFW; ++i) {
            const int f = wv * NFW + i;
            __builtin_amdgcn_global_load_lds((const void*)frag_src(ch, f), (__attribute__((address_space(3))) void*)(WBb + (size_t)(ch & 1) * K::WBUF + (size_t)f * 1024), 16, 0, 0);
        }
    };
    auto lds_frag = [&](int ch, int j) {
        const int f = j < 2 * KS ? (j & 1) * KS + (j >> 1) : j;
        return *(const half8*)(WBb + (size_t)(ch & 1) * K::WBUF + (size_t)f * 1024 + lane * 16);
    };
    if (K::KEEP) stage(0);
    for (int i = tid; i < 3 * C; i += K::NWV * 64) ((float*)(smem + K::BIAS_OFF))[i] = i < 2 * C ? p.b1[i] : p.b2[i - 2 * C];
    const float* B1s = (const float*)(smem + K::BIAS_OFF) + g * 4;
    const float* B2s = B1s + 2 * C;

    {
        half8 xr[NP];
#pragma unroll
        for (int k = 0; k < NP; ++k) xr[k] = __builtin_bit_cast(half8, __builtin_amdgcn_raw_buffer_load_b128(XB, vo + k * 1024u, 0, 0));
#pragma unroll
        for (int k = 0; k < NP; ++k) {
            const int idx = k * 64 + lane, r = idx / PPR, c = idx - r * PPR;
            *(half8*)(Xw + r * LDX + c * 8) = xr[k];
        }
    }
    W2X_PHASE_FENCE();
    half8 xreg[TT][KS];
#pragma unroll
    for (int tt = 0; tt < TT; ++tt) {
        half8 raw[KS];
        float s = 0.f, q = 0.f;
#pragma unroll
        for (int ks = 0; ks < KS; ++ks) { raw[ks] = *(const half8*)(Xw + (tt * 16 + fr) * LDX + ks * 32 + g * 8); sum_sq8(raw[ks], s, q); }
        s = rows_sum(s);
        q = rows_sum(q);
        const float mean = s * (1.f / C);
        const float rstd = __builtin_amdgcn_rsqf(fmaxf(q * (1.f / C) - mean * mean, 0.f) + p.eps);
        const float nm = -mean * rstd;
#pragma unroll
        for (int ks = 0; ks < KS; ++ks) xreg[tt][ks] = norm8(raw[ks], rstd, nm);
    }
    W2X_PHASE_FENCE();
// ... 376 lines not shown
    for (int nt = 0; nt < NT; ++nt)
#pragma unroll
        for (int q = 0; q < 4; ++q)
            *(half4*)(Xw + r32 * LDX + nt * 32 + q * 8 + h * 4) = (half4){(_Float16)acc2[nt][4 * q], (_Float16)acc2[nt][4 * q + 1], (_Float16)acc2[nt][4 * q + 2], (_Float16)acc2[nt][4 * q + 3]};
    W2X_PHASE_FENCE();
#pragma unroll
    for (int k = 0; k < NP; ++k) {
        const int idx = k * 64 + lane, r = idx / PPR, c = idx - r * PPR;
        const half8 o = *(const half8*)(Xw + r * LDX + c * 8) + xres[k];
        if (!(W2X_MLP2Q_EXP & 32) || o[0] == (_Float16)12345.f) __builtin_amdgcn_raw_buffer_store_b128(__builtin_bit_cast(uint4v, o), YB, vo + k * 1024u, 0, 0);
        if (p.stats_out) *(half8*)(Xw + r * LDX + c * 8) = o;
    }
    W2X_PHASE_FENCE();
    if (p.stats_out && lane < nrows) {
        float s = 0.f, q = 0.f;
#pragma unroll
        for (int c = 0; c < PPR; ++c) sum_sq8(*(const half8*)(Xw + lane * LDX + c * 8), s, q);
        const float mean = s * (1.f / C);
        p.stats_out[2 * (row0 + lane)] = mean;
        p.stats_out[2 * (row0 + lane) + 1] = __builtin_amdgcn_rsqf(fmaxf(q * (1.f / C) - mean * mean, 0.f) + p.eps_out);
    }
}

template <int C, int NW>
hipError_t launch_mlp2q_c(const MlpParams& p, hipStream_t s) {
    using K = Mlp2Cfg<C, 2, NW>;
    constexpr int SMEMQ = W2X_MLP2Q_EARLY0 ? K::NWV * K::SLAB + K::WBUF + 3 * C * 4 : K::SMEM;
    static unsigned lds_ok = 0;
    if (hipError_t e = ensure_dynamic_lds((const void*)mlp2q_kernel<C, NW>, SMEMQ, lds_ok); e != hipSuccess) return e;
    const long max_rows = (long)((0xFFF00000u / (C * 2)) / K::BM) * K::BM;
    for (long r0 = 0; r0 < p.M; r0 += max_rows) {
        MlpParams q = p;
        q.M = p.M - r0 < max_rows ? p.M - r0 : max_rows;
        q.x = (const char*)p.x + (size_t)r0 * C * 2; q.y = (char*)p.y + (size_t)r0 * C * 2;
        if (p.stats_out) q.stats_out = p.stats_out + 2 * r0;
        dim3 grid((unsigned)((q.M + K::BM - 1) / K::BM));
        hipLaunchKernelGGL((mlp2q_kernel<C, NW>), grid, dim3(K::NWV * 64), SMEMQ, s, q);
        if (hipError_t e = hipGetLastError(); e != hipSuccess) return e;
    }
    return hipSuccess;
}

template <int C, int TT, int NW>
hipError_t launch_mlp2_c(const MlpParams& p, hipStream_t s) {
    using K = Mlp2Cfg<C, TT, NW>;
    static unsigned lds_ok = 0;
    if (hipError_t e = ensure_dynamic_lds((const void*)mlp2_kernel<C, TT, NW>, K::SMEM, lds_ok); e != hipSuccess) return e;
    const long max_rows = (long)((0xFFF00000u / (C * 2)) / K::BM) * K::BM;
    for (long r0 = 0; r0 < p.M; r0 += max_rows) {
        MlpParams q = p;
        q.M = p.M - r0 < max_rows ? p.M - r0 : max_rows;
        q.x = (const char*)p.x + (size_t)r0 * C * 2; q.y = (char*)p.y + (size_t)r0 * C * 2;
        if (p.stats_out) q.stats_out = p.stats_out + 2 * r0;
        dim3 grid((unsigned)((q.M + K::BM - 1) / K::BM));
        hipLaunchKernelGGL((mlp2_kernel<C, TT, NW>), grid, dim3(K::NWV * 64), K::SMEM, s, q);
        if (hipError_t e = hipGetLastError(); e != hipSuccess) return e;
    }
    return hipSuccess;
}

}

bool mlp96q_supported(const MlpParams& p);
hipError_t launch_mlp96q(const MlpParams& p, hipStream_t s);

hipError_t launch_mlp2(const MlpParams& p, hipStream_t s) {
    if (p.C == 96 && p.frag32) return mlp96q_supported(p) ? launch_mlp96q(p, s) : hipErrorInvalidValue;
    if (p.C == 96) return launch_mlp2_c<96, 2, 4>(p, s);
    if (p.C == 192 && p.frag32) return launch_mlp2q_c<192, 4>(p, s);
    if (p.C == 192) return launch_mlp2_c<192, W2X_MLP192_TT, W2X_MLP192_NW>(p, s);
    return hipErrorInvalidValue;
}

}
```

waifu2x-tensorrt_amd/csrc/k_mlp96q.hip:

```cpp
#include "kernels.h"
#ifndef W2X_GELU_DEG
#define W2X_GELU_DEG 4
#endif

#include <algorithm>

#ifndef W2X_MLP_EXP
#define W2X_MLP_EXP 0
#endif
#ifndef W2X_MLP_PREFETCH
#define W2X_MLP_PREFETCH 1
#endif
#ifndef W2X_MLP96_PRIO
#define W2X_MLP96_PRIO 1
#endif
#ifndef W2X_MLP_STAGGER
#define W2X_MLP_STAGGER 0
#endif
#ifndef W2X_MLP_PFCH
#define W2X_MLP_PFCH 5
#endif

namespace w2x {
namespace {
// ... 88 lines not shown
constexpr int NF = KS;
static_assert(NF == NT * 2, "one ring serves both products");
constexpr int WBYTES = (W1F + W2F) * 1024;
constexpr int BIAS_OFF = WBYTES + NWV * SLAB;
#ifndef W2X_MLP96_DYN
#define W2X_MLP96_DYN 1
#endif
static_assert(!W2X_MLP96_DYN || W2X_MLP_PREFETCH, "the tile counter is read where the next tile's rows are requested: without the prefetch a wave would stop after its first tile");
constexpr int CTR_OFF = BIAS_OFF + 3 * C * 4;
constexpr int SMEM96Q = CTR_OFF + 16;
static_assert(RW * PPR % 64 == 0, "flat piece count");
static_assert(SMEM96Q <= 160 * 1024, "LDS budget");

template <bool TOIMG>
__global__ __launch_bounds__(NTHR, 3) void mlp96q_kernel(const MlpParams p, int ntiles) {
    extern __shared__ __attribute__((aligned(16))) unsigned char smem[];
    const int tid = threadIdx.x, lane = tid & 63;
    const int wv = __builtin_amdgcn_readfirstlane(tid >> 6);
    const int r32 = lane & 31, h = lane >> 5;
    const _Float16* WL = (const _Float16*)smem + lane * 8;
    _Float16* Xw = (_Float16*)(smem + WBYTES + wv * SLAB);

    {
        const uint4v* w1 = (const uint4v*)p.w1_frag;
        const uint4v* w2 = (const uint4v*)p.w2_frag;
        uint4v* dst = (uint4v*)smem;
        constexpr int N1 = W1F * 64, NALL = (W1F + W2F) * 64;
#pragma unroll
        for (int k = 0; k < NALL / NTHR; ++k) {
            const int i = k * NTHR + tid;
            dst[i] = i < N1 ? w1[i] : w2[i - N1];
        }
        if (tid < 3 * C) ((float*)(smem + BIAS_OFF))[tid] = tid < 2 * C ? p.b1[tid] : p.b2[tid - 2 * C];
        if (tid == 0) *(int*)(smem + CTR_OFF) = 0;
    }
#if W2X_MLP_STAGGER
    for (int k = 0; k < (wv >> 2) * W2X_MLP_STAGGER; ++k) __builtin_amdgcn_s_sleep(127);
#endif
    const float* B1s = (const float*)(smem + BIAS_OFF) + h * 4;
    const float* B2s = B1s + 2 * C;
    __syncthreads();

    half8 wr[NF];
#pragma unroll
    for (int i = 0; i < NF; ++i) wr[i] = *(const half8*)(WL + (size_t)i * 512);
    const int gw = blockIdx.x * NWV + wv, nw = gridDim.x * NWV;
    const unsigned xbytes = (unsigned)(p.M * (C * 2));
    const __amdgpu_buffer_rsrc_t XB = make_rsrc(p.x, xbytes), YB = make_rsrc(p.y, xbytes);
    constexpr unsigned TILE_BYTES = RW * C * 2;
    half8 xr[NP];
#define W2X_FETCH(TILE) { const unsigned vo = (unsigned)((W2X_MLP_EXP & 1) ? ((TILE) & 63) : (TILE)) * TILE_BYTES + lane * 16u;   \
        _Pragma("unroll") for (int k = 0; k < NP; ++k) xr[k] = __builtin_bit_cast(half8, __builtin_amdgcn_raw_buffer_load_b128(XB, vo + k * 1024u, 0, W2X_LD_LAST_AUX)); }
    constexpr bool DYN = W2X_MLP96_DYN && !TOIMG;
    auto grab = [&]() -> int {
        int t = 0;
        if (lane == 0) t = atomicAdd((int*)(smem + CTR_OFF), 1);
        t = __builtin_amdgcn_readfirstlane(t);
        const int tl = (blockIdx.x + (t / NWV) * (int)gridDim.x) * NWV + t % NWV;
        return tl < ntiles ? tl : ntiles;
    };
    int tile = gw, next_tile = ntiles;
    if constexpr (DYN) tile = grab();
    if (tile < ntiles) W2X_FETCH(tile)
#if W2X_MLP_PREFETCH
#pragma unroll
    for (int k = 0; k < NP; ++k) __builtin_amdgcn_raw_buffer_store_b128(uint4v{}, YB, 0xFFFFF000u + k * 16u, 0, 0);
#endif
#pragma unroll 1
    for (; tile < ntiles; tile = DYN ? next_tile : tile + nw) {
        const long row0 = (long)((W2X_MLP_EXP & 1) ? (tile & 63) : tile) * RW;
        const long nrows = p.M - row0 < RW ? p.M - row0 : RW;
#if !W2X_MLP_PREFETCH
        W2X_FETCH(tile)
#endif
#pragma unroll
        for (int k = 0; k < NP; ++k) {
            const int idx = k * 64 + lane, r = idx / PPR, c = idx - r * PPR;
            *(half8*)(Xw + r * LDX + c * 8) = xr[k];
        }
        W2X_PHASE_FENCE();
#if defined(W2X_MLP96_PRIO) && W2X_MLP96_PRIO == 6
        __builtin_amdgcn_s_setprio(1);
#endif
        half8 xreg[KS];
        {
            half8 raw[KS];
            float s = 0.f, q = 0.f;
#pragma unroll
            for (int ks = 0; ks < KS; ++ks) { raw[ks] = *(const half8*)(Xw + r32 * LDX + ks * 16 + h * 8); sum_sq8(raw[ks], s, q); }
            halves_sum2(s, q);
            const float mean = s * (1.f / C);
            const float rstd = __builtin_amdgcn_rsqf(fmaxf(q * (1.f / C) - mean * mean, 0.f) + p.eps);
            const float nm = -mean * rstd;
#pragma unroll
            for (int ks = 0; ks < KS; ++ks) xreg[ks] = norm8(raw[ks], rstd, nm);
        }
        float16v acc2[NT];
#pragma unroll
        for (int nt = 0; nt < NT; ++nt)
#pragma unroll
            for (int q = 0; q < 4; ++q) {
                const float4v b = *(const float4v*)(B2s + nt * 32 + q * 8);
#pragma unroll
                for (int j = 0; j < 4; ++j) acc2[nt][4 * q + j] = b[j];
            }
#if defined(W2X_MLP96_PRIO) && (W2X_MLP96_PRIO == 1 || W2X_MLP96_PRIO == 5)
        __builtin_amdgcn_s_setprio(1);
#elif defined(W2X_MLP96_PRIO) && W2X_MLP96_PRIO == 2
        __builtin_amdgcn_s_setprio(0);
#elif defined(W2X_MLP96_PRIO) && W2X_MLP96_PRIO == 4
        __builtin_amdgcn_s_setprio(3);
#endif
#pragma unroll
        for (int ch = 0; ch < NCH; ++ch) {
            float16v acc1;
#pragma unroll
            for (int q = 0; q < 4; ++q) {
                const float4v b = *(const float4v*)(B1s + ch * 32 + q * 8);
#pragma unroll
                for (int j = 0; j < 4; ++j) acc1[4 * q + j] = b[j];
            }
#pragma unroll
            for (int i = 0; i < NF; ++i) {
                if (!(W2X_MLP_EXP & 4)) acc1 = __builtin_amdgcn_mfma_f32_32x32x16_f16(wr[i], xreg[i], acc1, 0, 0, 0);
                else acc1[i] += (float)xreg[i][0] + (float)wr[i][0];
                if (!(W2X_MLP_EXP & 8)) wr[i] = *(const half8*)(WL + (size_t)(W1F + ch * NF + i) * 512);
                W2X_RING_FENCE();
            }
#if W2X_MLP_PREFETCH
            if (ch == W2X_MLP_PFCH) {
                if constexpr (DYN) { next_tile = grab(); W2X_FETCH(next_tile) } else { W2X_FETCH(tile + nw) }
                W2X_RING_FENCE();
            }
#endif
            half8 a2[2];
#if defined(W2X_MLP96_PRIO) && W2X_MLP96_PRIO == 3
            __builtin_amdgcn_s_setprio(1);
#elif defined(W2X_MLP96_PRIO) && W2X_MLP96_PRIO == 5
            __builtin_amdgcn_s_setprio(0);
#endif
#pragma unroll
            for (int s2 = 0; s2 < 2; ++s2) {
                if (W2X_MLP_EXP & 2) {
                    a2[s2] = (half8){(_Float16)acc1[8 * s2], (_Float16)acc1[8 * s2 + 1], (_Float16)acc1[8 * s2 + 2], (_Float16)acc1[8 * s2 + 3],
                                     (_Float16)acc1[8 * s2 + 4], (_Float16)acc1[8 * s2 + 5], (_Float16)acc1[8 * s2 + 6], (_Float16)acc1[8 * s2 + 7]};
                    continue;
                }
                const float2v g0 = gelu_fast2((float2v){acc1[8 * s2 + 0], acc1[8 * s2 + 1]});
                const float2v g1 = gelu_fast2((float2v){acc1[8 * s2 + 2], acc1[8 * s2 + 3]});
                const float2v g2 = gelu_fast2((float2v){acc1[8 * s2 + 4], acc1[8 * s2 + 5]});
                const float2v g3 = gelu_fast2((float2v){acc1[8 * s2 + 6], acc1[8 * s2 + 7]});
                a2[s2] = (half8){(_Float16)g0[0], (_Float16)g0[1], (_Float16)g1[0], (_Float16)g1[1],
                                 (_Float16)g2[0], (_Float16)g2[1], (_Float16)g3[0], (_Float16)g3[1]};
            }
#if defined(W2X_MLP96_PRIO) && W2X_MLP96_PRIO == 3
            __builtin_amdgcn_s_setprio(0);
#elif defined(W2X_MLP96_PRIO) && W2X_MLP96_PRIO == 5
            __builtin_amdgcn_s_setprio(1);
#endif
            const int nch = ch + 1 < NCH ? ch + 1 : 0;
#pragma unroll
            for (int i = 0; i < NF; ++i) {
                if (!(W2X_MLP_EXP & 4)) acc2[i >> 1] = __builtin_amdgcn_mfma_f32_32x32x16_f16(wr[i], a2[i & 1], acc2[i >> 1], 0, 0, 0);
                else acc2[i >> 1][i] += (float)a2[i & 1][0] + (float)wr[i][1];
                if (!(W2X_MLP_EXP & 8)) wr[i] = *(const half8*)(WL + (size_t)(nch * NF + i) * 512);
                W2X_RING_FENCE();
            }
        }
#if defined(W2X_MLP96_PRIO) && (W2X_MLP96_PRIO == 1 || W2X_MLP96_PRIO >= 4)
        __builtin_amdgcn_s_setprio(0);
#elif defined(W2X_MLP96_PRIO) && W2X_MLP96_PRIO == 2
        __builtin_amdgcn_s_setprio(1);
#endif
        W2X_PHASE_FENCE();
        half8 wfh[2][3];
        if (TOIMG) {
#pragma unroll
            for (int t = 0; t < 2; ++t)
#pragma unroll
                for (int ks = 0; ks < 3; ++ks) wfh[t][ks] = *(const half8*)((const _Float16*)p.ti_w + lane * 8 + (size_t)(t * 3 + ks) * 512);
            W2X_RING_FENCE();
        }
        half8 xres[NP];
#pragma unroll
// ... 60 lines not shown
                            asm("v_pk_max_f16 %0, %1, %2\n\tv_pk_min_f16 %0, %0, %3" : "=&v"(v23) : "v"(v23), "v"(lo2), "v"(hi2));
                        }
                        const half4 px = {v01[0], v01[1], v23[0], v23[1]};
                        if (ok) *(half4*)(Og + ((size_t)(oy * 4 + 2 * th + t) * p.ti_Ws + ox * 4 + g4) * 4) = px;
                    }
                }
            }
        }
        if (!TOIMG && p.stats_out) {
#pragma unroll
            for (int k = 0; k < NP; ++k) {
                const int idx = k * 64 + lane, r = idx / PPR, c = idx - r * PPR;
                *(half8*)(Xw + r * LDX + c * 8) = *(const half8*)(Xw + r * LDX + c * 8) + xres[k];
            }
        }
        W2X_PHASE_FENCE();
        if (!TOIMG && p.stats_out && lane < nrows) {
            float s = 0.f, q = 0.f;
#pragma unroll
            for (int c = 0; c < PPR; ++c) sum_sq8(*(const half8*)(Xw + lane * LDX + c * 8), s, q);
            const float mean = s * (1.f / C);
            p.stats_out[2 * (row0 + lane)] = mean;
            p.stats_out[2 * (row0 + lane) + 1] = __builtin_amdgcn_rsqf(fmaxf(q * (1.f / C) - mean * mean, 0.f) + p.eps_out);
        }
        W2X_PHASE_FENCE();
    }
#undef W2X_FETCH
}

}

bool mlp96q_supported(const MlpParams& p) { return p.C == C && p.w1_frag && p.w2_frag && p.frag32 && (!p.ti_w || (p.ti_b && p.ti_out && !p.stats_out && p.ti_Mrows > 0 && p.ti_Mrows % RW == 0 && p.ti_aW >= RW && p.M < 0x7FFFFFFFl &&
                                                                 (!p.ti_clip || ((float)(_Float16)p.ti_lo == p.ti_lo && (float)(_Float16)p.ti_hi == p.ti_hi)))); }

hipError_t launch_mlp96q(const MlpParams& p, hipStream_t s) {
    static unsigned lds_ok = 0;
    static unsigned lds_ok_t = 0;
    if (hipError_t e = p.ti_w ? ensure_dynamic_lds((const void*)mlp96q_kernel<true>, SMEM96Q, lds_ok_t) : ensure_dynamic_lds((const void*)mlp96q_kernel<false>, SMEM96Q, lds_ok); e != hipSuccess) return e;
    static int cus[32] = {0};
    int dev = 0;
    if (hipError_t e = hipGetDevice(&dev); e != hipSuccess) return e;
    int ncu = __atomic_load_n(&cus[dev & 31], __ATOMIC_RELAXED);
    if (ncu == 0) {
        if (hipError_t e = hipDeviceGetAttribute(&ncu, hipDeviceAttributeMultiprocessorCount, dev); e != hipSuccess) return e;
        __atomic_store_n(&cus[dev & 31], ncu, __ATOMIC_RELAXED);
    }
    const long max_tiles = std::min<long>((long)(kMaxBufBytes / (RW * C * 2)), 0xFFFFFFFFl / (RW * C * 2) - (long)ncu * NWV);
    const long max_rows = max_tiles * RW;
    for (long r0 = 0; r0 < p.M; r0 += max_rows) {
        MlpParams q = p;
        q.M = std::min(max_rows, p.M - r0);
        q.x = (const char*)p.x + (size_t)r0 * C * 2; q.y = (char*)p.y + (size_t)r0 * C * 2;
        if (p.stats_out) q.stats_out = p.stats_out + 2 * r0;
        const long ntiles = (q.M + RW - 1) / RW;
        const int grid = (int)std::min<long>((ntiles + NWV - 1) / NWV, ncu);
        if ((ntiles + (long)grid * NWV) * (long)(RW * C * 2) > 0xFFFFFFFFl) return hipErrorInvalidValue;
        if (p.ti_w) {
            q.ti_row0 = r0;
            hipLaunchKernelGGL(mlp96q_kernel<true>, dim3(grid), dim3(NTHR), SMEM96Q, s, q, (int)ntiles);
        } else hipLaunchKernelGGL(mlp96q_kernel<false>, dim3(grid), dim3(NTHR), SMEM96Q, s, q, (int)ntiles);
        if (hipError_t e = hipGetLastError(); e != hipSuccess) return e;
    }
    return hipSuccess;
}

}
```

waifu2x-tensorrt_amd/csrc/k_swinattn192u.hip:

```cpp
#include "kernels.h"

#include <algorithm>

namespace w2x {
namespace {

typedef _Float16 half8 __attribute__((ext_vector_type(8)));
typedef _Float16 half4 __attribute__((ext_vector_type(4)));
typedef _Float16 half2v __attribute__((ext_vector_type(2)));
typedef float float4v __attribute__((ext_vector_type(4)));
typedef float float2v __attribute__((ext_vector_type(2)));

__device__ __forceinline__ void sum_sq8(const half8 v, float& s, float& q) {
    const half2v one = {(_Float16)1.f, (_Float16)1.f};
    s = 0.f; q = 0.f;
#pragma unroll
    for (int k = 0; k < 4; ++k) {
        const half2v h = {v[2 * k], v[2 * k + 1]};
        s = __builtin_amdgcn_fdot2(h, one, s, false);
        q = __builtin_amdgcn_fdot2(h, h, q, false);
    }
}
typedef unsigned uint4v __attribute__((ext_vector_type(4)));
typedef int int2v __attribute__((ext_vector_type(2)));
// ... 34 lines not shown
        "v_max_f32 %0, %0, %3\n\tv_max_f32 %1, %1, %4\n\tv_max_f32 %2, %2, %5\n\t"
        "v_mov_b32 %3, %0\n\tv_mov_b32 %4, %1\n\tv_mov_b32 %5, %2\n\t"
        "v_permlane32_swap_b32 %0, %3\n\tv_permlane32_swap_b32 %1, %4\n\tv_permlane32_swap_b32 %2, %5\n\t"
        "v_max_f32 %0, %0, %3\n\tv_max_f32 %1, %1, %4\n\tv_max_f32 %2, %2, %5"
        : "+v"(a0), "+v"(a1), "+v"(a2), "=&v"(b0), "=&v"(b1), "=&v"(b2));
}
__device__ __forceinline__ float group_sum32(float v) {
    v += __builtin_bit_cast(float, __builtin_amdgcn_update_dpp(0, __builtin_bit_cast(int, v), 0xB1, 0xF, 0xF, true));
    v += __builtin_bit_cast(float, __builtin_amdgcn_update_dpp(0, __builtin_bit_cast(int, v), 0x4E, 0xF, 0xF, true));
    v += __builtin_bit_cast(float, __builtin_amdgcn_update_dpp(0, __builtin_bit_cast(int, v), 0x141, 0xF, 0xF, true));
    v += __builtin_bit_cast(float, __builtin_amdgcn_update_dpp(0, __builtin_bit_cast(int, v), 0x140, 0xF, 0xF, true));
    float a = v, b = v; swap16(a, b);
    return a + b;
}

#ifndef W2X_A192U_RING
#define W2X_A192U_RING 6
#endif
#ifndef W2X_A192U_WPC
#define W2X_A192U_WPC 3
#endif
#ifndef W2X_A192U_EXP
#define W2X_A192U_EXP 0
#endif
#ifndef W2X_A192U_BIAS_EARLY
#define W2X_A192U_BIAS_EARLY 1
#endif
constexpr int C = 192, HD = 32, NH = 6, NTOK = 36, G = 2, R = G * NTOK, RT = 5, RP = RT * 16;
constexpr int SLAB = 48, RPX = G * SLAB;
constexpr int LDX = C + 8;
constexpr int XS = RPX * LDX;
constexpr int NPAD = G * 12;
constexpr int DUMMY = XS * 2;
constexpr int PIX_OFF = DUMMY + LDX * 2;
constexpr int BQ_OFF = PIX_OFF + (R + NPAD) * 8;
constexpr int SMEM192U = BQ_OFF + 3 * C * 4;
constexpr int LPR = 32, PPR = C / 8, RPP = 256 / LPR, NPASS = R / RPP;
static_assert(R % RPP == 0, "row passes");
static_assert(RP * LDX <= XS, "the head-output tile and the output tile fit where the slabs were");
static_assert(SMEM192U * W2X_A192U_WPC <= 160 * 1024, "LDS per CU");

__device__ __forceinline__ int slab_row(int t) { return t < 32 ? t : 32 + 4 * (t - 32); }

__global__ __launch_bounds__(256, W2X_A192U_WPC) void swin_attn192u_kernel(const SwinAttnParams p) {
    extern __shared__ __attribute__((aligned(16))) unsigned char smem[];
    _Float16* Xs = (_Float16*)smem;
    int2v* Pix = (int2v*)(smem + PIX_OFF);

    const int tid = threadIdx.x, lane = tid & 63;
    const int wv = __builtin_amdgcn_readfirstlane(tid >> 6);
    const int fr = lane & 15, g = lane >> 4;

    const int iw0 = blockIdx.x * G, iw1 = iw0 + 1, itotal = p.B * p.nwin;
    const bool wok0 = iw0 < itotal, wok1 = iw1 < itotal;
    const int HW = p.nwin * NTOK;
    const int wb0 = iw0 / p.nwin, wb1 = iw1 / p.nwin;
    const int pixbase0 = wb0 * HW, pixbase1 = wb1 * HW;
    const int wl0 = iw0 - wb0 * p.nwin, wl1 = iw1 - wb1 * p.nwin;
    const int nwx = p.W / 6;
    const int wy0 = wl0 / nwx, wx0 = wl0 - wy0 * nwx, wy1 = wl1 / nwx, wx1 = wl1 - wy1 * nwx;
    const unsigned xbytes = (unsigned)p.B * (unsigned)HW * (C * 2);
    const __amdgpu_buffer_rsrc_t X = make_rsrc(p.x, xbytes), Y = make_rsrc(p.y, xbytes);
    const _Float16* __restrict__ Wqkv = (const _Float16*)p.wqkv_frag;
    const _Float16* __restrict__ Wproj = (const _Float16*)p.wproj_frag;
    const float4v zero4 = {0.f, 0.f, 0.f, 0.f};
    const half8 zero8 = {};

    const int hA = wv, hC = 4 + (wv >> 1), wC = wv & 1;
    const int amask0 = wok0 ? p.maskid[wl0] : 0, amask1 = wok1 ? p.maskid[wl1] : 0;

    constexpr int RING = W2X_A192U_RING, NFRAG = 108;
    const __amdgpu_buffer_rsrc_t WQ = make_rsrc(Wqkv, 3u * C * C * 2u), WP = make_rsrc(Wproj, (unsigned)C * C * 2u);
    const unsigned wl16 = lane * 16u;
    auto wfrag = [&](int q) {
        const int u = q / 36, j = q - u * 36;
        const int H = u < 2 ? hA : hC;
        const int M = j < 24 ? (j & 1) : 2, ks = j < 24 ? j >> 2 : (j - 24) >> 1, ft = j < 24 ? (j >> 1) & 1 : (j - 24) & 1;
        return __builtin_bit_cast(half8, __builtin_amdgcn_raw_buffer_load_b128(WQ, wl16, (unsigned)((M * NH + H) * 12 + ft * 6 + ks) * 1024u, 0));
    };
    float4v bq_stage = zero4;
    if (tid < 3 * C / 4) bq_stage = *(const float4v*)(p.bqkv + tid * 4);
    const float* Bq = (const float*)(smem + BQ_OFF);
    half8 wr[RING];
#pragma unroll
    for (int i = 0; i < RING; ++i) wr[i] = wfrag(i);
#define W2X_RING_NEXT(Q) do { if ((Q) + RING < NFRAG) { wr[(Q) % RING] = wfrag((Q) + RING); asm volatile("" ::: "memory"); } } while (0)

    if (tid < R + NPAD) {
        int pix = -1, srow;
        if (tid >= R) {
            const int k = tid - R, w = k >= 12 ? 1 : 0, kk = k - 12 * w;
            srow = (w * SLAB + 33 + (kk / 3) * 4 + (kk % 3)) * LDX * 2;
        } else {
            const int w = tid >= NTOK ? 1 : 0, t = tid - w * NTOK;
            srow = (w * SLAB + slab_row(t)) * LDX * 2;
            if (w == 0 ? wok0 : wok1) {
                if (p.ry >= 0) {
                    const int ty = t / 6, tx = t - ty * 6;
                    int y = (w == 0 ? wy0 : wy1) * 6 + ty + p.ry, x = (w == 0 ? wx0 : wx1) * 6 + tx + p.rx;
                    y -= y >= p.H ? p.H : 0; x -= x >= p.W ? p.W : 0;
                    pix = (w == 0 ? pixbase0 : pixbase1) + y * p.W + x;
                } else pix = (w == 0 ? pixbase0 : pixbase1) + p.table[(w == 0 ? wl0 : wl1) * NTOK + t];
            }
        }
        Pix[tid] = (int2v){pix < 0 ? (int)kNoRow : (int)((unsigned)pix * (unsigned)(C * 2)), srow};
    }
    if (tid < 3 * C / 4) *(float4v*)(smem + BQ_OFF + tid * 16) = bq_stage;
    __syncthreads();

    {
        const int li = tid & (LPR - 1), rsub = tid / LPR;
        const unsigned lane_off = li < PPR ? li * 16u : kNoRow;
        half8 xr[NPASS];
// ... 232 lines not shown
        }
#pragma unroll
        for (int mt = 0; mt < RT; ++mt) {
            const half8 of = *(const half8*)(Os + (mt * 16 + fr) * LDX + ks * 32 + g * 8);
#pragma unroll
            for (int t = 0; t < 3; ++t) acc[mt][t] = __builtin_amdgcn_mfma_f32_16x16x32_f16(wp[ks & 1][t], of, acc[mt][t], 0, 0, 0);
        }
    }
    __syncthreads();
#pragma unroll
    for (int mt = 0; mt < RT; ++mt)
#pragma unroll
        for (int t = 0; t < 3; ++t)
            *(half4*)(Xs + (mt * 16 + fr) * LDX + (wv * 3 + t) * 16 + g * 4) = (half4){(_Float16)acc[mt][t][0], (_Float16)acc[mt][t][1], (_Float16)acc[mt][t][2], (_Float16)acc[mt][t][3]};
    __syncthreads();

    {
        const int li = li_r, rsub = rsub_r;
#pragma unroll
        for (int ps = 0; ps < NPASS; ++ps) {
            const int r = ps * RPP + rsub;
            const bool ok = my_off[ps] != kNoRow;
            half8 o = *(const half8*)(Xs + r * LDX + li * 8) + xres[ps];
            __builtin_amdgcn_raw_buffer_store_b128(__builtin_bit_cast(uint4v, o), Y, my_off[ps], 0, W2X_ST_AUX);
            if (p.stats_out) {
                if (!ok) o = half8{};
                const size_t pix = my_off[ps] / (C * 2);
                float s, q;
                sum_sq8(o, s, q);
                s = group_sum32(s);
                q = group_sum32(q);
                const float mean = s * (1.f / C);
                if (ok && li == 0) { p.stats_out[2 * pix] = mean; p.stats_out[2 * pix + 1] = __builtin_amdgcn_rsqf(fmaxf(q * (1.f / C) - mean * mean, 0.f) + p.eps_out); }
            }
        }
    }
}

}

hipError_t launch_swin_attn192u(const SwinAttnParams& p, hipStream_t s) {
    auto kern = swin_attn192u_kernel;
    static unsigned lds_ok = 0;
    if (hipError_t e = ensure_dynamic_lds((const void*)kern, SMEM192U, lds_ok); e != hipSuccess) return e;
    const size_t img_bytes = (size_t)p.nwin * NTOK * C * 2;
    if (img_bytes == 0 || img_bytes > kMaxBufBytes) return hipErrorInvalidValue;
    const int per_run = (int)std::min<size_t>((size_t)p.B, kMaxBufBytes / img_bytes);
    for (int b0 = 0; b0 < p.B; b0 += per_run) {
        SwinAttnParams q = p;
        q.B = std::min(per_run, p.B - b0);
        q.x = (const char*)p.x + (size_t)b0 * img_bytes;
        q.y = (char*)p.y + (size_t)b0 * img_bytes;
        if (p.stats_out) q.stats_out = p.stats_out + (size_t)b0 * p.nwin * NTOK * 2;
        const long total_win = (long)q.B * q.nwin;
        hipLaunchKernelGGL(kern, dim3((unsigned)((total_win + G - 1) / G)), dim3(256), SMEM192U, s, q);
        if (hipError_t e = hipGetLastError(); e != hipSuccess) return e;
    }
    return hipSuccess;
}

}
```

waifu2x-tensorrt_amd/csrc/k_swinattn96.hip:

```cpp
#include "kernels.h"

#include <algorithm>


namespace w2x {
namespace {

typedef _Float16 half8 __attribute__((ext_vector_type(8)));
typedef _Float16 half4 __attribute__((ext_vector_type(4)));
typedef _Float16 half2v __attribute__((ext_vector_type(2)));
typedef float float4v __attribute__((ext_vector_type(4)));
typedef float float2v __attribute__((ext_vector_type(2)));
typedef int int2v __attribute__((ext_vector_type(2)));
typedef unsigned uint4v __attribute__((ext_vector_type(4)));

constexpr unsigned kNoRow = 0xFFFFFFFFu;
constexpr size_t kMaxBufBytes = 0xFFFFFF00u;
__device__ __forceinline__ __amdgpu_buffer_rsrc_t make_rsrc(const void* p, unsigned bytes) {
    return __builtin_amdgcn_make_buffer_rsrc(const_cast<void*>(p), 0, bytes, 0x00020000);
}

__device__ __forceinline__ void sum_sq8(const half8 v, float& s, float& q) {
    const half2v one = {(_Float16)1.f, (_Float16)1.f};
    s = 0.f; q = 0.f;
// ... 69 lines not shown
constexpr int SMEM96 = BQ_OFF + 3 * C * 4;
constexpr int DUMMY = XS * 2;
constexpr int LPR = 16, PPR = C / 8, RPP = NTHR / LPR, NPASS = RP / RPP;
static_assert(NPASS == 5, "the row sums are reduced as 3 + 2 passes");

__device__ __forceinline__ int slab_row(int t) { return t < 32 ? t : 32 + 4 * (t - 32); }

__device__ __forceinline__ void probs(const float4v s0, const float4v s1, float s2, float mx, half8& p01, half4& p2) {
    const float2v m2 = {mx, mx};
    const float2v a0 = (float2v){s0[0], s0[1]} - m2, a1 = (float2v){s0[2], s0[3]} - m2;
    const float2v c0 = (float2v){s1[0], s1[1]} - m2, c1 = (float2v){s1[2], s1[3]} - m2;
    p01 = (half8){(_Float16)__builtin_amdgcn_exp2f(a0[0]), (_Float16)__builtin_amdgcn_exp2f(a0[1]), (_Float16)__builtin_amdgcn_exp2f(a1[0]), (_Float16)__builtin_amdgcn_exp2f(a1[1]),
                  (_Float16)__builtin_amdgcn_exp2f(c0[0]), (_Float16)__builtin_amdgcn_exp2f(c0[1]), (_Float16)__builtin_amdgcn_exp2f(c1[0]), (_Float16)__builtin_amdgcn_exp2f(c1[1])};
    p2 = (half4){(_Float16)__builtin_amdgcn_exp2f(s2 - mx), (_Float16)0.f, (_Float16)0.f, (_Float16)0.f};
}
__device__ __forceinline__ half4 lo4(const half8 v) { return (half4){v[0], v[1], v[2], v[3]}; }
__device__ __forceinline__ half4 hi4(const half8 v) { return (half4){v[4], v[5], v[6], v[7]}; }
struct KeysAcc { float4v a, b; };
__device__ __forceinline__ KeysAcc keys_product(const half8 a01, const half4 a2, const half8 p01, const half4 p2, const KeysAcc acc) {
    KeysAcc o;
    o.a = __builtin_amdgcn_mfma_f32_16x16x32_f16(a01, p01, acc.a, 0, 0, 0);
    o.b = __builtin_amdgcn_mfma_f32_16x16x16f16(a2, p2, acc.b, 0, 0, 0);
    return o;
}
__device__ __forceinline__ half4 scaled_output(const KeysAcc o, float inv, const float4v bv) {
    const float2v i2 = {inv, inv};
    float2v o0 = __builtin_elementwise_fma((float2v){o.a[0], o.a[1]}, i2, (float2v){bv[0], bv[1]});
    float2v o1 = __builtin_elementwise_fma((float2v){o.a[2], o.a[3]}, i2, (float2v){bv[2], bv[3]});
    o0 = __builtin_elementwise_fma((float2v){o.b[0], o.b[1]}, i2, o0);
    o1 = __builtin_elementwise_fma((float2v){o.b[2], o.b[3]}, i2, o1);
    return (half4){(_Float16)o0[0], (_Float16)o0[1], (_Float16)o1[0], (_Float16)o1[1]};
}
__device__ __forceinline__ float keys_sum(const half8 p01, const half4 p2) {
    const float4v zero4 = {0.f, 0.f, 0.f, 0.f};
    const half4 ones = {(_Float16)1.f, (_Float16)1.f, (_Float16)1.f, (_Float16)1.f};
    float4v l = __builtin_amdgcn_mfma_f32_16x16x16f16(ones, lo4(p01), zero4, 0, 0, 0);
    l = __builtin_amdgcn_mfma_f32_16x16x16f16(ones, hi4(p01), l, 0, 0, 0);
    return __builtin_amdgcn_mfma_f32_16x16x16f16(ones, p2, l, 0, 0, 0)[0];
}

__global__ __launch_bounds__(NTHR, 4) void swin_attn96_kernel(const SwinAttnParams p) {
    extern __shared__ __attribute__((aligned(16))) unsigned char smem[];
    _Float16* Xs = (_Float16*)smem;
    _Float16* Os = Xs + XS;
    int2v* Pix = (int2v*)(Os + OS);
    int* Cls = (int*)(Pix + RP + NPAD);

    const int tid = threadIdx.x, lane = tid & 63;
    const int wv = __builtin_amdgcn_readfirstlane(tid >> 6);
    const int fr = lane & 15, g = lane >> 4;

    const int wl0 = blockIdx.x * G;
    const int HW = p.nwin * NTOK;
    const unsigned xbytes = (unsigned)p.B * (unsigned)HW * (C * 2);
    const __amdgpu_buffer_rsrc_t X = make_rsrc(p.x, xbytes), Y = make_rsrc(p.y, xbytes);
    const _Float16* __restrict__ Wqkv = (const _Float16*)p.wqkv_frag;
    const _Float16* __restrict__ Wproj = (const _Float16*)p.wproj_frag;
    const float4v zero4 = {0.f, 0.f, 0.f, 0.f};
    const half8 zero8 = {};

    const int hA = wv, hC = 4 + (wv >> 1), wC = wv & 1;

    half8 wq[3], wk[3], wv_[3];
    const __amdgpu_buffer_rsrc_t WQ = make_rsrc(Wqkv, 3u * C * C * 2u), WP = make_rsrc(Wproj, (unsigned)C * C * 2u);
    const __amdgpu_buffer_rsrc_t BP = make_rsrc(p.bproj, (unsigned)C * 4u), RB = make_rsrc(p.bias32, 0x7FFFFFF0u);
    const unsigned l16 = lane * 16u, l4 = lane * 4u, g16 = (lane >> 4) * 16u;
#define W2X_WFRAG(SEL, H, KS) __builtin_bit_cast(half8, __builtin_amdgcn_raw_buffer_load_b128(WQ, l16, (unsigned)(((SEL) * NH + (H)) * 3 + (KS)) * 1024u, 0))
#define W2X_BQKV(OFF) (*(const float4v*)((const float*)(smem + BQ_OFF) + (OFF) + g * 4))
    if (tid < 3 * C / 4) *(float4v*)(smem + BQ_OFF + tid * 16) = *(const float4v*)(p.bqkv + tid * 4);
#define W2X_LOAD_W(H)                                                                           \
    _Pragma("unroll") for (int ks = 0; ks < 3; ++ks) {                                          \
        wq[ks] = W2X_WFRAG(0, H, ks);                                                           \
        wk[ks] = W2X_WFRAG(1, H, ks);                                                           \
        wv_[ks] = W2X_WFRAG(2, H, ks);                                                          \
    }
    W2X_LOAD_W(hA)

    if (tid < RP + NPAD) {
        int pix = -1, srow = DUMMY;
        if (tid >= RP) {
            const int k = tid - RP, w = k >= 12 ? 1 : 0, kk = k - 12 * w;
            srow = (w * SLAB + 33 + (kk / 3) * 4 + (kk % 3)) * LDX * 2;
        } else if (tid < R) {
            const int w = tid >= NTOK ? 1 : 0, t = tid - w * NTOK;
            const int wl = wl0 + w;
            srow = (w * SLAB + slab_row(t)) * LDX * 2;
            if (wl < p.nwin) {
                if (p.ry >= 0) {
                    const int nwx = p.W / 6;
                    const int wy = (int)(((float)wl + 0.5f) * __builtin_amdgcn_rcpf((float)nwx)), wx = wl - wy * nwx;
                    const int ty = (t * 43) >> 8, tx = t - ty * 6;
                    int y = wy * 6 + ty + p.ry, x = wx * 6 + tx + p.rx;
                    y -= y >= p.H ? p.H : 0; x -= x >= p.W ? p.W : 0;
                    pix = (int)blockIdx.y * HW + y * p.W + x;
                } else pix = (int)blockIdx.y * HW + p.table[wl * NTOK + t];
                if (t == 0) Cls[w] = p.maskid[wl];
            } else if (t == 0) Cls[w] = 0;
        }
        Pix[tid] = (int2v){pix < 0 ? (int)kNoRow : (int)((unsigned)pix * (unsigned)(C * 2)), srow};
    }
    __syncthreads();

    {
        const int li = tid & (LPR - 1), rsub = tid / LPR;
        const unsigned lane_off = li < PPR ? li * 16u : kNoRow;
        half8 xr[NPASS];
        int srow[NPASS];
#pragma unroll
        for (int ps = 0; ps < NPASS; ++ps) {
            const int2v pr = Pix[ps * RPP + rsub];
            srow[ps] = pr[1];
            xr[ps] = __builtin_bit_cast(half8, __builtin_amdgcn_raw_buffer_load_b128(X, __builtin_elementwise_add_sat((unsigned)pr[0], lane_off), 0, 0));
        }
        float sm[NPASS], sq[NPASS];
#pragma unroll
        for (int ps = 0; ps < 3; ++ps) sum_sq8(xr[ps], sm[ps], sq[ps]);
        group_sum16_x6(sm[0], sq[0], sm[1], sq[1], sm[2], sq[2]);
#pragma unroll
        for (int ps = 3; ps < 5; ++ps) sum_sq8(xr[ps], sm[ps], sq[ps]);
        group_sum16_x4(sm[3], sq[3], sm[4], sq[4]);
#pragma unroll
        for (int ps = 0; ps < NPASS; ++ps) {
            const float mean = sm[ps] * (1.f / C);
            const float rstd = __builtin_amdgcn_rsqf(fmaxf(sq[ps] * (1.f / C) - mean * mean, 0.f) + p.eps);
            *(half8*)(smem + (li < PPR ? srow[ps] + li * 16 : DUMMY)) = norm8(xr[ps], rstd, -mean * rstd);
        }
#pragma unroll
        for (int k = 0; k < (NPAD + RPP - 1) / RPP; ++k) {
            const int pr = k * RPP + rsub;
            if (pr < NPAD) *(half8*)(smem + (li < PPR ? Pix[RP + pr][1] + li * 16 : DUMMY)) = zero8;
        }
    }
    __syncthreads();

    const float qscale = p.scale * 1.44269504088896341f;
    const float2v qs2 = {qscale, qscale};
    const half4 zeroh4 = {};
    const int xoff = fr * LDX + g * 8;
    const int ul = fr >> 2, ql = fr & 3;
    const int wl_ = ul == 1 ? 1 : ul == 2 ? wC : 0;
// ... 128 lines not shown
        }
#pragma unroll
        for (int ks = 0; ks < 3; ++ks) {
            const half8 of = *(const half8*)(Os + mt * 16 * LDX + xoff + ks * 32);
#pragma unroll
            for (int t = 0; t < 3; ++t) acc[t] = __builtin_amdgcn_mfma_f32_16x16x32_f16(wf[t][ks], of, acc[t], 0, 0, 0);
        }
#pragma unroll
        for (int t = 0; t < 3; ++t)
            *(half4*)(Xs + (mt * 16 + fr) * LDX + (n3 + t) * 16 + g * 4) = (half4){(_Float16)acc[t][0], (_Float16)acc[t][1], (_Float16)acc[t][2], (_Float16)acc[t][3]};
    }
    __syncthreads();

    {
        const int li = tid & (LPR - 1), rsub = tid / LPR;
        const unsigned lane_off = li < PPR ? li * 16u : kNoRow;
        unsigned my_off[NPASS];
#pragma unroll
        for (int ps = 0; ps < NPASS; ++ps) my_off[ps] = __builtin_elementwise_add_sat((unsigned)Pix[ps * RPP + rsub][0], lane_off);
#pragma unroll
        for (int ps = 0; ps < NPASS; ++ps) {
            const int r = ps * RPP + rsub;
            const bool ok = my_off[ps] != kNoRow;
            half8 o = *(const half8*)(Xs + r * LDX + li * 8) + xres[ps];
            __builtin_amdgcn_raw_buffer_store_b128(__builtin_bit_cast(uint4v, o), Y, my_off[ps], 0, W2X_ST_AUX);
            if (p.stats_out) {
                if (!ok) o = half8{};
                const size_t pix = my_off[ps] / (C * 2);
                float s, q;
                sum_sq8(o, s, q);
                s = group_sum16(s);
                q = group_sum16(q);
                const float mean = s * (1.f / C);
                if (ok && li == 0) { p.stats_out[2 * (size_t)pix] = mean; p.stats_out[2 * (size_t)pix + 1] = __builtin_amdgcn_rsqf(fmaxf(q * (1.f / C) - mean * mean, 0.f) + p.eps_out); }
            }
        }
    }
}

}

hipError_t launch_swin_attn96(const SwinAttnParams& p, hipStream_t s) {
    static unsigned lds_ok = 0;
    if (hipError_t e = ensure_dynamic_lds((const void*)swin_attn96_kernel, SMEM96, lds_ok); e != hipSuccess) return e;
    const size_t img_bytes = (size_t)p.nwin * NTOK * C * 2;
    if (img_bytes == 0 || img_bytes > kMaxBufBytes) return hipErrorInvalidValue;
    const int per_run = (int)std::min<size_t>((size_t)p.B, kMaxBufBytes / img_bytes);
    for (int b0 = 0; b0 < p.B; b0 += per_run) {
        SwinAttnParams q = p;
        q.B = std::min(per_run, p.B - b0);
        q.x = (const char*)p.x + (size_t)b0 * img_bytes;
        q.y = (char*)p.y + (size_t)b0 * img_bytes;
        if (p.stats_out) q.stats_out = p.stats_out + (size_t)b0 * p.nwin * NTOK * 2;
        hipLaunchKernelGGL(swin_attn96_kernel, dim3((unsigned)((q.nwin + G - 1) / G), (unsigned)q.B), dim3(NTHR), SMEM96, s, q);
        if (hipError_t e = hipGetLastError(); e != hipSuccess) return e;
    }
    return hipSuccess;
}

}
```

waifu2x-tensorrt_amd/csrc/kernels.h:

```cpp
#pragma once
#include <hip/hip_runtime.h>

#include "support.h"
#include "switches.h"
#include <cstdint>

namespace w2x {

constexpr int kGemmBM = 128;

inline hipError_t ensure_dynamic_lds(const void* fn, int bytes, unsigned& done_mask) {
    int dev = 0;
    hipError_t e = hipGetDevice(&dev);
    if (e != hipSuccess) return e;
    const unsigned bit = 1u << (dev & 31);
    if (__atomic_load_n(&done_mask, __ATOMIC_ACQUIRE) & bit) return hipSuccess;
    e = hipFuncSetAttribute(fn, hipFuncAttributeMaxDynamicSharedMemorySize, bytes);
    if (e == hipSuccess) __atomic_fetch_or(&done_mask, bit, __ATOMIC_RELEASE);
    return e;
}

#ifndef W2X_ST_AUX
#define W2X_ST_AUX 2
#endif
#ifndef W2X_LD_LAST_AUX
#define W2X_LD_LAST_AUX 2
#endif
#ifdef __HIPCC__
template <class T> __device__ __forceinline__ void w2x_store_out(T* p, const T v) {
#if W2X_ST_AUX == 2
    __builtin_nontemporal_store(v, p);
#else
    *p = v;
#endif
}
#endif

struct TView {
    void* p = nullptr;
    int Hs = 0, Ws = 0, Cs = 0;
    int y0 = 0, x0 = 0;
};

struct GemmParams {
    TView a;
    int amode = 0, kh = 1, kw = 1, stride = 1;
    int B = 0, Mrows = 0, aW = 0;
    const int* win_table = nullptr;
    int K = 0, N = 0, Kw = 0;
    const void* wt = nullptr;
    const void* wt_frag = nullptr;
    const void* wt_perm = nullptr;
    const float* bias = nullptr;
    const float* csum = nullptr;
    const float* stats_in = nullptr;
    int ln = 0;
    int act = 0; float alpha = 0.f;
    int has_clip = 0; float clip_lo = 0.f, clip_hi = 0.f;
    const float* a_scale = nullptr;
    const float* res_scale = nullptr;
    TView res, res2;
    TView out;
    int omode = 0, r = 1, Cout = 0;
    float* stats_out = nullptr; float ln_eps = 1e-5f;
    float* pool_out = nullptr;
};

struct AttnParams {
    const void* qkv = nullptr; void* out = nullptr;
    int B = 0, nwin = 0, heads = 0, hd = 0, ntok = 0;
    float scale = 1.f;
    const void* bias = nullptr;
    const int* maskid = nullptr;
};

struct MlpParams {
    const void* x = nullptr; void* y = nullptr;
    long M = 0; int C = 0;
    const void* w1 = nullptr;
    const float* b1 = nullptr;
    const void* w2 = nullptr;
    const float* b2 = nullptr;
    float eps = 1e-5f;
    float* stats_out = nullptr; float eps_out = 1e-5f;
    const void* w1_frag = nullptr; const void* w2_frag = nullptr;
    bool frag32 = false;
    const void* ti_w = nullptr;
    const float* ti_b = nullptr;
    void* ti_out = nullptr; int ti_Hs = 0, ti_Ws = 0, ti_Mrows = 0, ti_aW = 0;
    int ti_clip = 0; float ti_lo = 0.f, ti_hi = 0.f;
    long ti_row0 = 0;
};

struct SwinAttnParams {
    const void* x = nullptr; void* y = nullptr;
    const int* table = nullptr;
    int H = 0, W = 0, ry = -1, rx = -1;
    int B = 0, nwin = 0, C = 0, hd = 0;
    const void* wqkv = nullptr;
    const float* bqkv = nullptr;
    float scale = 1.f;
    const float* bias32 = nullptr;
    const int* maskid = nullptr;
    const void* wproj = nullptr;
    const float* bproj = nullptr;
    float eps = 1e-5f;
    float* stats_out = nullptr; float eps_out = 1e-5f;
    const void* wqkv_frag = nullptr; const void* wproj_frag = nullptr;
};

struct SeParams {
    const float* pool = nullptr; float* scale = nullptr;
    int B = 0, C = 0, Cs = 0, Cmid = 0; float inv_count = 0.f;
    int nblocks = 0, Mrows = 0;
    const float *w1 = nullptr, *b1 = nullptr, *w2 = nullptr, *b2 = nullptr;
};

struct TileSlot { int x, y, aug, valid; };

struct GatherParams {
    const uint8_t* frame = nullptr; int rows = 0, cols = 0; size_t step = 0;
    int deep = 0;
    void* out = nullptr;
    int fp32 = 0;
    const TileSlot* slots = nullptr;
    int B = 0, T = 0;
};

struct ComposeParams {
    const void* tiles = nullptr;
    int fp32 = 0;
    uint8_t* dst = nullptr; size_t dst_step = 0;
    int deep = 0;
    int outW = 0, outH = 0;
    int To = 0;
    int nx = 0, ny = 0;
    int stride_x = 0, stride_y = 0;
    int ovx = 0, ovy = 0;
    const float* ramp_x = nullptr;
    const float* ramp_y = nullptr;
    int tta = 0;
    int tta_bug_compat = 0;
    int x0 = 0, x1 = 0; long first_tile = 0;
    int y0 = 0, y1 = 0;
};

hipError_t launch_gemm(const GemmParams& p, hipStream_t s);
bool pixgemm_supported(const GemmParams& p);
hipError_t launch_pixgemm(const GemmParams& p, hipStream_t s);
bool conv3_supported(const GemmParams& p);
bool stem_supported(const GemmParams& p);
hipError_t launch_stem(const GemmParams& p, hipStream_t s);
hipError_t launch_conv3(const GemmParams& p, hipStream_t s);
bool conv3h_supported(const GemmParams& p);
hipError_t launch_conv3h(const GemmParams& p, hipStream_t s);
bool conv48_supported(const GemmParams& p);
hipError_t launch_conv48(const GemmParams& p, hipStream_t s);
bool conv48_stem_supported(const GemmParams& p, const GemmParams& ps);
hipError_t launch_conv48_stem(const GemmParams& p, const GemmParams& ps, hipStream_t s);
bool conv3_stem_supported(const GemmParams& p, const GemmParams& ps);
hipError_t launch_conv3_stem(const GemmParams& p, const GemmParams& ps, hipStream_t s);
// ... 149 lines not shown
```

waifu2x-tensorrt_amd/csrc/support.cpp:

```cpp
#include "support.h"

namespace w2x {

bool swin_attn_supported(int C, int heads, int hd, int ws) {
    return ws == 6 && heads * hd == C && ((C == 96 && hd == 16) || (C == 192 && hd == 32));
}
bool mlp_supported(int C) { return C == 96 || C == 192; }
bool gemm_row_stats_supported(int N) { return N == 32 || N == 48 || N == 64 || N == 96 || N == 128 || N == 192; }
bool attn_supported(int hd, int ntok) {
    if (ntok != 36 && ntok != 64) return false;
    return hd == 8 || hd == 16 || hd == 24 || hd == 32 || hd == 48 || hd == 64;
}

}

#include <algorithm>
#include <cstdlib>
#include <cstring>

#include "switches.h"

namespace w2x {

namespace {
struct Field { const char* name; int Switches::*i; bool Switches::*b; const char* env; int lo, hi; };
const Field kFields[] = {
    {"superbatch", &Switches::superbatch, nullptr, "W2X_SUPERBATCH", 0, 4096},
    {"groups", &Switches::groups, nullptr, "W2X_GROUPS", 1, 4},
    {"render_parts", &Switches::render_parts, nullptr, "W2X_RENDER_PARTS", 1, 4},
    {"no_graph", nullptr, &Switches::no_graph, "W2X_NO_GRAPH", 0, 1},
    {"no_rolling", nullptr, &Switches::no_rolling, "W2X_NO_ROLLING", 0, 1},
    {"poison", nullptr, &Switches::poison, "W2X_POISON", 0, 1},
    {"check_general", nullptr, &Switches::check_general, "W2X_CHECK_GENERAL", 0, 1},
    {"roctx", nullptr, &Switches::roctx, "W2X_ROCTX", 0, 1},
    {"no_fuse", nullptr, &Switches::no_fuse, nullptr, 0, 1},
    {"no_fuse_attn", nullptr, &Switches::no_fuse_attn, nullptr, 0, 1},
    {"no_se_fold", nullptr, &Switches::no_se_fold, nullptr, 0, 1},
    {"no_fuse_head", nullptr, &Switches::no_fuse_head, nullptr, 0, 1},
    {"no_fuse_stem", nullptr, &Switches::no_fuse_stem, nullptr, 0, 1},
    {"no_fuse_up", nullptr, &Switches::no_fuse_up, nullptr, 0, 1},
    {"no_conv3h_walk", nullptr, &Switches::no_conv3h_walk, nullptr, 0, 1},
    {"no_pixgemm", nullptr, &Switches::no_pixgemm, nullptr, 0, 1},
    {"no_conv3", nullptr, &Switches::no_conv3, nullptr, 0, 1},
    {"no_conv3h", nullptr, &Switches::no_conv3h, nullptr, 0, 1},
    {"no_conv48", nullptr, &Switches::no_conv48, nullptr, 0, 1},
    {"no_stem", nullptr, &Switches::no_stem, nullptr, 0, 1},
    {"attn_valu", nullptr, &Switches::attn_valu, nullptr, 0, 1},
};
void assign(Switches& s, const Field& f, long v) {
    v = std::min<long>(f.hi, std::max<long>(f.lo, v));
    if (f.i) s.*(f.i) = (int)v; else s.*(f.b) = v != 0;
}
}

Switches& switches() { static Switches s; return s; }

void switches_from_env() {
    Switches& s = switches();
    const Switches d;
    for (const Field& f : kFields) {
        if (!f.env) continue;
        const char* e = getenv(f.env);
        if (f.i) s.*(f.i) = e ? (int)std::min<long>(f.hi, std::max<long>(f.lo, atol(e))) : d.*(f.i);
        else s.*(f.b) = e != nullptr;
    }
}

bool set_switch(const char* name, long value) {
    if (!name) return false;
    for (const Field& f : kFields) if (!strcmp(f.name, name)) { assign(switches(), f, value); return true; }
    return false;
}

std::string switches_nondefault() {
    const Switches& s = switches();
    const Switches d;
    std::string out;
    for (const Field& f : kFields) {
        const bool same = f.i ? s.*(f.i) == d.*(f.i) : s.*(f.b) == d.*(f.b);
        if (same) continue;
        if (!out.empty()) out += ' ';
        out += f.name;
        if (f.i) out += "=" + std::to_string(s.*(f.i));
    }
    return out;
}

}
```

waifu2x-tensorrt_amd/csrc/switches.h:

```cpp
#pragma once
#include <string>

namespace w2x {

struct Switches {
    int superbatch = 0;
    int groups = 2;
    int render_parts = 3;
    bool no_graph = false;
    bool no_rolling = false;
    bool poison = false;
    bool check_general = false;
    bool roctx = false;
    bool no_fuse = false;
    bool no_fuse_attn = false;
    bool no_se_fold = false;
    bool no_fuse_head = false;
    bool no_fuse_stem = false;
    bool no_fuse_up = false;
    bool no_conv3h_walk = false;
    bool no_pixgemm = false, no_conv3 = false, no_conv3h = false, no_conv48 = false, no_stem = false;
    bool attn_valu = false;
};

Switches& switches();
void switches_from_env();
bool set_switch(const char* name, long value);
std::string switches_nondefault();

}
```

waifu2x-tensorrt_amd/engine.py:

```python
from __future__ import annotations

import ctypes as C
import enum
import os
from dataclasses import dataclass

import numpy as np

_HERE = os.path.dirname(os.path.abspath(__file__))
lib_path = os.path.join(_HERE, "libw2x.so")


class W2xError(RuntimeError):
    pass


class Precision(enum.IntEnum):
    TF32 = 0
    FP16 = 1
    FP32 = 2


RESIZE_FILTERS = {"bicubic": 0, "bilinear": 1}

# ... 103 lines not shown
    L.w2x_set_message_callback.argtypes = [vp, _MSG_FN, vp]
    L.w2x_set_progress_callback.argtypes = [vp, _PROG_FN, vp]
    L.w2x_build.argtypes = [vp, C.c_char_p, C.POINTER(_BuildConfig)]; L.w2x_build.restype = C.c_int
    L.w2x_load.argtypes = [vp, C.c_char_p, C.POINTER(_RenderConfig)]; L.w2x_load.restype = C.c_int
    L.w2x_render.argtypes = [vp, vp, C.c_int, C.c_int, C.c_size_t, vp, C.c_size_t]; L.w2x_render.restype = C.c_int
    L.w2x_render16.argtypes = [vp, vp, C.c_int, C.c_int, C.c_size_t, vp, C.c_size_t]; L.w2x_render16.restype = C.c_int
    L.w2x_render_resized.argtypes = [vp, vp, C.c_int, C.c_int, C.c_size_t, vp, C.c_int, C.c_int, C.c_size_t, C.c_int]; L.w2x_render_resized.restype = C.c_int
    L.w2x_render16_resized.argtypes = [vp, vp, C.c_int, C.c_int, C.c_size_t, vp, C.c_int, C.c_int, C.c_size_t, C.c_int]; L.w2x_render16_resized.restype = C.c_int
    L.w2x_render_sequence_resized.argtypes = [vp, vp, C.c_int, C.c_int, C.c_size_t, vp, C.c_int, C.c_int, C.c_size_t, C.c_int, C.c_int]; L.w2x_render_sequence_resized.restype = C.c_int
    L.w2x_resize_weights.argtypes = [C.c_int, C.c_int, C.c_int, vp, vp, C.c_int]; L.w2x_resize_weights.restype = C.c_int
    L.w2x_render_yuv.argtypes = [vp, vp, vp, C.c_int, C.c_int, C.c_int, vp, vp, C.c_int, C.c_int, C.c_int, C.c_int, C.c_int]; L.w2x_render_yuv.restype = C.c_int
    L.w2x_render_sequence_yuv.argtypes = [vp, vp, vp, C.c_int, C.c_int, C.c_int, vp, vp, C.c_int, C.c_int, C.c_int, C.c_int, C.c_int, C.c_int]
    L.w2x_render_sequence_yuv.restype = C.c_int
    L.w2x_render_yuv_resized.argtypes = L.w2x_render_yuv.argtypes + [C.c_int]; L.w2x_render_yuv_resized.restype = C.c_int
    L.w2x_render_sequence_yuv_resized.argtypes = L.w2x_render_sequence_yuv.argtypes + [C.c_int]; L.w2x_render_sequence_yuv_resized.restype = C.c_int
    L.w2x_render_rgba.argtypes = [vp, vp, C.c_int, C.c_int, C.c_size_t, vp, C.c_size_t, C.c_int, C.c_int]; L.w2x_render_rgba.restype = C.c_int
    L.w2x_alpha_bleed_device.argtypes = [vp, vp, C.c_int, C.c_int, C.c_size_t, vp, C.c_size_t, C.c_int]; L.w2x_alpha_bleed_device.restype = C.c_int
    L.w2x_alpha_bleed.argtypes = [vp, C.c_size_t, vp, C.c_size_t, C.c_int, C.c_int, C.c_int, vp, C.c_size_t]; L.w2x_alpha_bleed.restype = C.c_int
    L.w2x_yuv_plane_sizes.argtypes = [C.c_int, C.c_int, C.c_int, vp, vp, vp]; L.w2x_yuv_plane_sizes.restype = C.c_int
    L.w2x_render_strip.argtypes = [vp, vp, C.c_int, C.c_int, C.c_size_t, vp, C.c_size_t, C.c_int, C.c_int]; L.w2x_render_strip.restype = C.c_int
    L.w2x_render_sequence.argtypes = [vp, vp, C.c_int, C.c_int, C.c_size_t, vp, C.c_size_t, C.c_int]; L.w2x_render_sequence.restype = C.c_int
    L.w2x_alloc_host.argtypes = [vp, C.c_size_t]; L.w2x_alloc_host.restype = vp
    L.w2x_free_host.argtypes = [vp, vp]; L.w2x_free_host.restype = None
    L.w2x_pin_host.argtypes = [vp, vp, C.c_size_t]; L.w2x_pin_host.restype = C.c_int
    L.w2x_unpin_host.argtypes = [vp, vp]; L.w2x_unpin_host.restype = None
    L.w2x_strip_plan.argtypes = [C.c_int] * 7 + [C.c_double, C.c_double, C.c_int, C.c_int, vp]; L.w2x_strip_plan.restype = C.c_int
    L.w2x_render_sharded.argtypes = [vp, C.c_int, vp, C.c_int, C.c_int, C.c_size_t, vp, C.c_size_t]; L.w2x_render_sharded.restype = C.c_int
    L.w2x_shard_compute.argtypes = [vp, vp, C.c_int, C.c_int, C.c_size_t, C.c_int, C.c_int]; L.w2x_shard_compute.restype = C.c_int
    L.w2x_shard_slab.argtypes = [vp, vp]; L.w2x_shard_slab.restype = vp
    L.w2x_shard_finish.argtypes = [vp, vp, C.c_int, C.c_int, C.c_size_t, C.c_int, C.c_int, vp, vp]; L.w2x_shard_finish.restype = C.c_int
    L.w2x_ipc_export.argtypes = [vp, vp]; L.w2x_ipc_export.restype = C.c_int
    L.w2x_ipc_open.argtypes = [vp, C.c_int]; L.w2x_ipc_open.restype = vp
    L.w2x_ipc_close.argtypes = [vp]; L.w2x_ipc_close.restype = None
    L.w2x_shard_plan.argtypes = [C.c_int] * 7 + [C.c_double, C.c_double, C.c_int, C.c_int, vp]; L.w2x_shard_plan.restype = C.c_int
    L.w2x_infer.argtypes = [vp, vp, vp]; L.w2x_infer.restype = C.c_int
    L.w2x_output_tile_size.argtypes = [vp]; L.w2x_output_tile_size.restype = C.c_int
    L.w2x_pass_tiles.argtypes = [vp]; L.w2x_pass_tiles.restype = C.c_int
    L.w2x_plan_flops.argtypes = [vp]; L.w2x_plan_flops.restype = C.c_double
    L.w2x_last_render_ms.argtypes = [vp]; L.w2x_last_render_ms.restype = C.c_float
    L.w2x_bench_resident.argtypes = [vp, C.c_int]; L.w2x_bench_resident.restype = C.c_float
    L.w2x_resident_output.argtypes = [vp, vp, C.c_size_t]; L.w2x_resident_output.restype = C.c_int
    L.w2x_profile_frame.argtypes = [vp, vp, C.c_int]; L.w2x_profile_frame.restype = C.c_int
    L.w2x_op_times.argtypes = [vp, vp, C.c_int]; L.w2x_op_times.restype = C.c_int
    L.w2x_calculate_tiles.argtypes = [C.c_int] * 7 + [C.c_double, C.c_double, vp, vp, C.c_int]; L.w2x_calculate_tiles.restype = C.c_int
    L.w2x_tile_weights.argtypes = [C.c_int, C.c_int, C.c_int, C.c_int, vp]; L.w2x_tile_weights.restype = C.c_int
    L.w2x_describe_plan.argtypes = [C.c_char_p, C.c_int, C.c_int, C.c_char_p, C.c_size_t]; L.w2x_describe_plan.restype = C.c_int
    L.w2x_describe_plan_precision.argtypes = [C.c_char_p, C.c_int, C.c_int, C.c_int, C.c_char_p, C.c_size_t]; L.w2x_describe_plan_precision.restype = C.c_int
    L.w2x_write_engine_file.argtypes = [C.c_char_p, C.c_int, C.c_int, C.c_char_p]; L.w2x_write_engine_file.restype = C.c_int
    L.w2x_validate_engine_file.argtypes = [C.c_char_p, C.c_char_p, C.c_size_t]; L.w2x_validate_engine_file.restype = C.c_int
    L.w2x_device_pci_bus_id.argtypes = [C.c_int, C.c_char_p, C.c_size_t]; L.w2x_device_pci_bus_id.restype = C.c_int
    L.w2x_sha256_hex.argtypes = [vp, C.c_size_t, C.c_char_p]
    L.w2x_version.restype = C.c_char_p
    L.w2x_debug_set.argtypes = [C.c_char_p, C.c_int]; L.w2x_debug_set.restype = C.c_int
    _lib = L
    return L


EXPORTED_SYMBOLS = [
    "w2x_create", "w2x_destroy", "w2x_set_message_callback", "w2x_set_progress_callback", "w2x_build", "w2x_load",
    "w2x_render", "w2x_render16", "w2x_infer", "w2x_output_tile_size", "w2x_plan_flops", "w2x_pass_tiles", "w2x_last_render_ms", "w2x_bench_resident", "w2x_resident_output", "w2x_profile_frame", "w2x_op_times",
    "w2x_render_resized", "w2x_render16_resized", "w2x_render_sequence_resized", "w2x_resize_weights",
    "w2x_render_yuv", "w2x_render_sequence_yuv", "w2x_yuv_plane_sizes", "w2x_render_yuv_resized", "w2x_render_sequence_yuv_resized",
    "w2x_render_rgba", "w2x_alpha_bleed_device", "w2x_alpha_bleed",
    "w2x_render_strip", "w2x_strip_plan", "w2x_render_sharded", "w2x_shard_plan", "w2x_shard_compute", "w2x_shard_slab", "w2x_shard_finish", "w2x_ipc_export", "w2x_ipc_open", "w2x_ipc_close", "w2x_render_sequence", "w2x_alloc_host", "w2x_free_host", "w2x_pin_host", "w2x_unpin_host", "w2x_calculate_tiles", "w2x_tile_weights", "w2x_describe_plan", "w2x_describe_plan_precision", "w2x_write_engine_file", "w2x_validate_engine_file", "w2x_device_pci_bus_id", "w2x_sha256_hex", "w2x_version", "w2x_debug_set"]


class Img2Img:

    def __init__(self):
        self._L = lib()
        self._h = self._L.w2x_create()
        if not self._h:
            raise W2xError("w2x_create failed")
        self.messages: list[tuple[int, str]] = []
        self._user_msg = None
        self._user_prog = None
        self._msg_cb = _MSG_FN(self._on_msg)
        self._prog_cb = _PROG_FN(self._on_prog)
        self._L.w2x_set_message_callback(self._h, self._msg_cb, None)
        self._L.w2x_set_progress_callback(self._h, self._prog_cb, None)

    def _on_msg(self, sev, msg, _):
        m = msg.decode(errors="replace")
        self.messages.append((sev, m))
        if self._user_msg:
            self._user_msg(Severity(sev), m)

    def _on_prog(self, cur, total, speed, _):
        if self._user_prog:
            self._user_prog(cur, total, speed)

    def close(self):
        if self._h:
            self._L.w2x_destroy(self._h)
            self._h = None

    def __del__(self):
        try:
            self.close()
        except Exception:
            pass

    def setMessageCallback(self, cb):
        self._user_msg = cb

    def setProgressCallback(self, cb):
        self._user_prog = cb

    def last_error(self) -> str:
        errs = [m for s, m in self.messages if s <= Severity.error]
        return errs[-1] if errs else ""

    def build(self, path: str, config: BuildConfig) -> bool:
        c = _BuildConfig(*[int(getattr(config, f[0])) for f in _BuildConfig._fields_])
        return bool(self._L.w2x_build(self._h, os.fsencode(path), C.byref(c)))

# ... 426 lines not shown
    return n, a[:n].copy(), b[:n].copy()


def tile_weights(which, ovx, ovy, size):
    L = lib()
    out = np.empty((size, size), np.float32)
    if not L.w2x_tile_weights(which, ovx, ovy, size, out.ctypes.data):
        raise W2xError("bad arguments")
    return out


def resize_weights(in_size: int, out_size: int, filter: str = "bicubic"):
    L = lib()
    fid = _filter_id(filter)
    taps = L.w2x_resize_weights(int(in_size), int(out_size), fid, None, None, 0)
    if taps <= 0:
        raise W2xError(f"invalid resize {in_size} -> {out_size}")
    first = np.zeros(out_size, np.int32)
    w = np.zeros((out_size, taps), np.float32)
    if L.w2x_resize_weights(int(in_size), int(out_size), fid, first.ctypes.data, w.ctypes.data, w.size) != taps:
        raise W2xError("w2x_resize_weights failed")
    return first, w


def alpha_bleed(bgr: np.ndarray, alpha: np.ndarray, radius: int) -> np.ndarray:
    if bgr.dtype != np.uint8 or bgr.ndim != 3 or bgr.shape[2] != 3 or (bgr.size and (bgr.strides[2] != 1 or bgr.strides[1] != 3)):
        raise ValueError("bgr must be a uint8 [rows, cols, 3] array with packed pixels")
    if alpha.dtype != np.uint8 or alpha.shape != bgr.shape[:2] or (alpha.size and alpha.strides[1] != 1):
        raise ValueError("alpha must be a uint8 [rows, cols] array of the frame's size with packed rows")
    out = np.empty(bgr.shape, np.uint8)
    if not lib().w2x_alpha_bleed(bgr.ctypes.data if bgr.size else None, bgr.strides[0], alpha.ctypes.data if alpha.size else None, alpha.strides[0],
                                 bgr.shape[0], bgr.shape[1], int(radius), out.ctypes.data if out.size else None, out.strides[0]):
        raise W2xError(f"invalid alpha bleed: a {bgr.shape[1]}x{bgr.shape[0]} frame at radius {radius}")
    return out


def yuv_plane_sizes(rows: int, cols: int, bits: int):
    pr, pc, pb = (C.c_int * 3)(), (C.c_int * 3)(), (C.c_size_t * 3)()
    if not lib().w2x_yuv_plane_sizes(int(rows), int(cols), int(bits), pr, pc, pb):
        raise W2xError(f"invalid YUV frame {rows}x{cols} at {bits} bits")
    return list(pr), list(pc), list(pb)


def describe_plan(onnx_path, batch, tile, precision=None) -> str:
    L = lib()
    buf = C.create_string_buffer(1 << 20)
    ok = L.w2x_describe_plan_precision(os.fsencode(onnx_path), batch, tile, int(Precision.FP16 if precision is None else precision), buf, len(buf))
    s = buf.value.decode(errors="replace")
    if not ok:
        raise W2xError(s)
    return s


def write_engine_file(onnx_path, batch, tile, out_path) -> bool:
    return bool(lib().w2x_write_engine_file(os.fsencode(onnx_path), batch, tile, os.fsencode(out_path)))


def validate_engine_file(path) -> tuple[bool, str]:
    buf = C.create_string_buffer(4096)
    ok = lib().w2x_validate_engine_file(os.fsencode(path), buf, len(buf))
    return bool(ok), buf.value.decode(errors="replace")


def sha256_hex(data: bytes) -> str:
    L = lib()
    out = C.create_string_buffer(65)
    L.w2x_sha256_hex(data, len(data), out)
    return out.value.decode()
```

Measured before the change: 4476 MPix/s.

## Skip MLP and attention work on dead regions of cropped edge tiles

Adds a backward liveness analysis over the plan that computes, for each op, the output extents that actually feed the kept region of each tile. Per-slot extents are uploaded to the device and passed to the MLP and Swin attention kernels, which exit early for row blocks lying wholly outside the live area. This targets wasted compute on partially cropped edge tiles. It adds host-side extent computation with caching, an extra upload per setup, and per-block checks in the kernels.

```diff
diff --git a/include/w2x/c_api.h b/include/w2x/c_api.h
--- a/include/w2x/c_api.h
+++ b/include/w2x/c_api.h
@@ -93,6 +93,9 @@
 int w2x_describe_plan_precision(const char* onnx_path, int batch, int tile, int precision, char* buf, size_t cap);
 int w2x_write_engine_file(const char* onnx_path, int batch, int tile, const char* out_path);
 int w2x_validate_engine_file(const char* path, char* buf, size_t cap);
+enum { W2X_EXTENT_INTS = 25 };
+int w2x_dead_skip_extents(const char* onnx_path, int batch, int tile, int in_w, int in_h, int scaling, double overlap_x, double overlap_y, int tile_index, int tta,
+                          int* out, int cap);
 int w2x_device_pci_bus_id(int device, char* buf, size_t cap);
 void w2x_sha256_hex(const void* data, size_t len, char* out);
 const char* w2x_version(void);
diff --git a/waifu2x-tensorrt_amd/__init__.py b/waifu2x-tensorrt_amd/__init__.py
--- a/waifu2x-tensorrt_amd/__init__.py
+++ b/waifu2x-tensorrt_amd/__init__.py
@@ -1,6 +1,6 @@
 from .engine import (BuildConfig, RenderConfig, Img2Img, Precision, Severity, lib, lib_path,
-                     calculate_tiles, strip_plan, shard_plan, render_sharded, device_pci_bus_id, ipc_open, ipc_close, tile_weights, resize_weights, yuv_plane_sizes, alpha_bleed, describe_plan, write_engine_file, validate_engine_file, sha256_hex, W2xError,
+                     calculate_tiles, strip_plan, shard_plan, render_sharded, device_pci_bus_id, ipc_open, ipc_close, tile_weights, resize_weights, yuv_plane_sizes, alpha_bleed, describe_plan, dead_skip_extents, write_engine_file, validate_engine_file, sha256_hex, W2xError,
                      debug_switches)
 
 __all__ = ["BuildConfig", "RenderConfig", "Img2Img", "Precision", "Severity", "lib", "lib_path",
-           "calculate_tiles", "strip_plan", "shard_plan", "render_sharded", "device_pci_bus_id", "ipc_open", "ipc_close", "tile_weights", "resize_weights", "yuv_plane_sizes", "alpha_bleed", "describe_plan", "write_engine_file", "validate_engine_file", "sha256_hex", "W2xError", "debug_switches"]
+           "calculate_tiles", "strip_plan", "shard_plan", "render_sharded", "device_pci_bus_id", "ipc_open", "ipc_close", "tile_weights", "resize_weights", "yuv_plane_sizes", "alpha_bleed", "describe_plan", "dead_skip_extents", "write_engine_file", "validate_engine_file", "sha256_hex", "W2xError", "debug_switches"]
diff --git a/waifu2x-tensorrt_amd/csrc/c_api.cpp b/waifu2x-tensorrt_amd/csrc/c_api.cpp
--- a/waifu2x-tensorrt_amd/csrc/c_api.cpp
+++ b/waifu2x-tensorrt_amd/csrc/c_api.cpp
@@ -1,4 +1,5 @@
 #include "../../include/w2x/c_api.h"
+#include <mutex>
 
 #include <cstring>
 #include <fstream>
@@ -6,6 +7,7 @@
 #include <string>
 
 #include "../../include/w2x/img2img.h"
+#include "liveness.h"
 #include "lower.h"
 #include "sha256.h"
 #include "tiles.h"
@@ -336,6 +338,44 @@
 
 const char* w2x_version(void) { return "w2x-hip 0.1 (gfx950)"; }
 
+int w2x_dead_skip_extents(const char* onnx_path, int batch, int tile, int in_w, int in_h, int scaling, double overlap_x, double overlap_y, int tile_index, int tta,
+                          int* out, int cap) {
+    try {
+        static std::mutex mu;
+        static std::string key;
+        static w2x::Plan plan;
+        std::lock_guard<std::mutex> lock(mu);
+        const std::string k = std::string(onnx_path ? onnx_path : "") + "|" + std::to_string(batch) + "|" + std::to_string(tile);
+        if (k != key) { plan = w2x::build_plan(onnx_path, batch, 3, tile, tile, false); plan.userB = batch; key = k; }
+        const int nops = (int)plan.ops.size();
+        if (!out || cap < nops * W2X_EXTENT_INTS) return -nops;
+        int kept_w = plan.Tout, kept_h = plan.Tout;
+        bool all = tta != 0 || tile_index < 0 || w2x::switches().no_dead_skip;
+        if (tile_index >= 0) {
+            const w2x::TileGrid g = w2x::calculate_tiles(in_w, in_h, in_w * scaling, in_h * scaling, tile, tile, plan.Tout, plan.Tout, scaling, overlap_x, overlap_y);
+            if (tile_index >= g.count) return 0;
+            kept_w = g.out[tile_index].w; kept_h = g.out[tile_index].h;
+        }
+        const std::vector<w2x::OpExtent> ext = w2x::dead_skip_extents(plan, kept_w, kept_h, all);
+        for (int i = 0; i < nops; ++i) {
+            const w2x::Op& op = plan.ops[i]; const w2x::OpExtent& e = ext[i];
+            int* o = out + (size_t)i * W2X_EXTENT_INTS;
+            int in_t = -1, out_t = -1, res_t = -1, kh = 1, kw = 1, stride = 1, x0 = 0, y0 = 0, r = 1;
+            if (op.kind == w2x::OP_GEMM) {
+                in_t = op.g.a.t; out_t = op.g.out.t; res_t = op.g.res.t; x0 = op.g.a.x0; y0 = op.g.a.y0;
+                if (op.g.amode == w2x::A_CONV) { kh = op.g.kh; kw = op.g.kw; stride = op.g.stride; }
+                if (op.g.omode == w2x::O_PIXSHUF) r = op.g.r;
+            } else if (op.kind == w2x::OP_MLP) { in_t = op.m.x; out_t = op.m.y; }
+            else if (op.kind == w2x::OP_SWINATTN) { in_t = op.sa.x; out_t = op.sa.y; }
+            auto dim = [&](int t, bool w) { return t >= 0 && t < (int)plan.tensors.size() ? (w ? plan.tensors[t].W : plan.tensors[t].H) : 0; };
+            const int v[W2X_EXTENT_INTS] = {op.kind, e.x.n, e.y.n, e.x.c, e.x.w, e.y.c, e.y.w, e.rx, e.ry, e.ws, in_t, out_t, res_t, kh, kw, stride, x0, y0, r,
+                                            dim(in_t, true), dim(in_t, false), dim(out_t, true), dim(out_t, false), (int)e.live_units(), (int)e.total_units()};
+            for (int k = 0; k < W2X_EXTENT_INTS; ++k) o[k] = v[k];
+        }
+        return nops;
+    } catch (const std::exception&) { return 0; }
+}
+
 int w2x_debug_set(const char* name, int value) { return w2x::set_switch(name, value) ? 1 : 0; }
 
 }
diff --git a/waifu2x-tensorrt_amd/csrc/engine.cpp b/waifu2x-tensorrt_amd/csrc/engine.cpp
--- a/waifu2x-tensorrt_amd/csrc/engine.cpp
+++ b/waifu2x-tensorrt_amd/csrc/engine.cpp
@@ -19,6 +19,7 @@
 #include "common.h"
 #include "fragorder.h"
 #include "kernels.h"
+#include "liveness.h"
 #include "lower.h"
 #include "plan.h"
 #include "sha256.h"
@@ -225,6 +226,41 @@
     bool rolling = false;
     bool rolling_ok = true;
     TileSlot* d_slots = nullptr; size_t slots_cap = 0;
+    LiveExt* d_live = nullptr; size_t live_cap = 0, live_stride = 0;
+    std::vector<LiveExt> h_live;
+    std::map<std::pair<int, int>, std::vector<OpExtent>> live_cache;
+    void upload_live(const TileGrid& grid, size_t count, hipStream_t on) {
+        const size_t nops = plan.ops.size();
+        if (!count || !nops) return;
+        if (count > live_stride) {
+            ensure(d_live, live_cap, (nops * count + 8) * sizeof(LiveExt));
+            live_stride = count;
+        }
+        const bool all = switches().no_dead_skip || check_general || cfg.tta;
+        std::map<std::pair<int, int>, int> tile_at;
+        if (!all) for (int t = 0; t < grid.count; ++t) tile_at[{grid.in[t].x, grid.in[t].y}] = t;
+        auto extents = [&](int w, int h) -> const std::vector<OpExtent>& {
+            auto it = live_cache.find({w, h});
+            if (it == live_cache.end()) it = live_cache.emplace(std::make_pair(w, h), dead_skip_extents(plan, w, h, false)).first;
+            return it->second;
+        };
+        const std::vector<OpExtent>& whole = extents(plan.Tout, plan.Tout);
+        h_live.resize(nops * count);
+        for (size_t st = 0; st < count; ++st) {
+            const TileSlot& sl = h_slots[st];
+            const std::vector<OpExtent>* e = &whole;
+            if (!all && sl.valid && sl.aug == 0) {
+                const auto it = tile_at.find({sl.x, sl.y});
+                if (it != tile_at.end()) e = &extents(grid.out[it->second].w, grid.out[it->second].h);
+            }
+            for (size_t i = 0; i < nops; ++i) {
+                const OpExtent& x = (*e)[i];
+                auto u16 = [](int v) { return (uint16_t)std::min(std::max(v, 0), 65535); };
+                h_live[i * count + st] = x.all() ? LiveExt{65535, 0, 65535, 0} : LiveExt{u16(x.x.c), u16(x.x.w), u16(x.y.c), u16(x.y.w)};
+            }
+        }
+        hipAssert(hipMemcpy2DAsync(d_live, live_stride * sizeof(LiveExt), h_live.data(), count * sizeof(LiveExt), count * sizeof(LiveExt), nops, hipMemcpyHostToDevice, on));
+    }
     float *d_rampx = nullptr, *d_rampy = nullptr;
     int ovx = 0, ovy = 0;
     float* d_blob_in = nullptr; float* d_blob_out = nullptr;
@@ -286,6 +322,8 @@
         }
         ensure(d_slots, slots_cap, stepCount * sizeof(TileSlot));
         hipAssert(hipMemcpy(d_slots, h_slots.data(), stepCount * sizeof(TileSlot), hipMemcpyHostToDevice));
+        upload_live(last_grid, stepCount, stream);
+        hipAssert(hipStreamSynchronize(stream));
         ensure(d_slab, slab_cap, stepCount * plan.Tout * plan.Tout * 4 * plan.elt);
         one_part_stale = false;
     }
@@ -337,9 +375,10 @@
         bgr_cap = alpha_cap = 0; rgba = false;
         if (h_minmax) { if (hipHostFree(h_minmax) != hipSuccess) (void)hipGetLastError(); h_minmax = nullptr; }
         if (ev_minmax) { (void)hipEventDestroy(ev_minmax); ev_minmax = nullptr; }
-        for (void** p : {(void**)&d_frame, (void**)&d_out, (void**)&d_frame2, (void**)&d_out2, &d_slab, &d_slab2, (void**)&d_slots, (void**)&d_rampx, (void**)&d_rampy, (void**)&d_blob_in, (void**)&d_blob_out})
+        for (void** p : {(void**)&d_frame, (void**)&d_out, (void**)&d_frame2, (void**)&d_out2, &d_slab, &d_slab2, (void**)&d_slots, (void**)&d_live, (void**)&d_rampx, (void**)&d_rampy, (void**)&d_blob_in, (void**)&d_blob_out})
             if (*p) { (void)hipFree(*p); *p = nullptr; }
         frame_cap = out_cap = slab_cap = slab2_cap = slots_cap = 0;
+        live_cap = live_stride = 0; live_cache.clear();
         shard_rows = shard_cols = 0; shard_halo_slots = 0; rolling = false; one_part_stale = false;
         last_rows = last_cols = last_batches = 0;
         if (ev0) { (void)hipEventDestroy(ev0); ev0 = nullptr; }
@@ -636,11 +675,12 @@
     uint8_t* group_ptr(const void* full, int grp) const {
         return full ? (uint8_t*)arena_base + (size_t)grp * arena_part() + (size_t)((const uint8_t*)full - (const uint8_t*)arena_base) / ng_now : nullptr;
     }
-    void run_network(void* out_override, int live = -1, int grp = -1, hipStream_t s = nullptr) {
+    void run_network(void* out_override, int live = -1, int grp = -1, hipStream_t s = nullptr, const LiveExt* ext = nullptr) {
         if (!s) s = stream;
         const int cap = grp < 0 ? plan.B : plan.B / ng_now;
         if (live < 0 || live > cap) live = cap;
         auto tp = [&](int t) -> uint8_t* { return t < 0 ? nullptr : grp < 0 ? (uint8_t*)tensors[t] : group_ptr(tensors[t], grp); };
+        auto lv = [&](int i) -> const LiveExt* { return ext ? ext + (size_t)i * live_stride : nullptr; };
         auto gp = [&](int i) {
             GemmParams p = gemm[i];
             p.B = live;
@@ -660,6 +700,7 @@
                 case L_HEAD: {
                     const GemmParams g = gp(L.last);
                     MlpParams p = mlp_params(op, live, tp);
+                    p.live = lv(L.last);
                     p.ti_w = g.wt_frag; p.ti_b = g.bias; p.ti_out = g.out.p; p.ti_Hs = g.out.Hs; p.ti_Ws = g.out.Ws; p.ti_Mrows = g.Mrows; p.ti_aW = g.aW;
                     p.ti_clip = g.has_clip; p.ti_lo = g.clip_lo; p.ti_hi = g.clip_hi;
                     issue([&] { return launch_mlp(p, s); });
@@ -716,12 +757,14 @@
                         p.wproj = blobs[a.wproj]; p.bproj = (const float*)blobs[a.bproj]; p.eps = a.eps;
                         p.wqkv_frag = frag_blobs[a.wqkv]; p.wproj_frag = frag_blobs[a.wproj];
                         p.stats_out = (float*)tp(a.stats_out); p.eps_out = a.eps_out;
+                        p.live = lv(L.first);
                         if (d.C != a.C || plan.tensors[a.y].C != a.C || d.H * d.W != a.nwin * a.ws * a.ws) throw std::runtime_error("plan: attention geometry mismatch");
                         issue([&] { return launch_swin_attn(p, s); });
                         break;
                     }
                     case OP_MLP: {
-                        const MlpParams p = mlp_params(op, live, tp);
+                        MlpParams p = mlp_params(op, live, tp);
+                        p.live = lv(L.first);
                         issue([&] { return launch_mlp(p, s); });
                         break;
                     }
@@ -759,6 +802,7 @@
         p.w1 = blobs[m.w1]; p.b1 = (const float*)blobs[m.b1]; p.w2 = blobs[m.w2]; p.b2 = (const float*)blobs[m.b2];
         p.w1_frag = frag_blobs[m.w1]; p.w2_frag = frag_blobs[m.w2]; p.frag32 = mlp_frag32(m.C);
         p.eps = m.eps; p.stats_out = (float*)tp(m.stats_out); p.eps_out = m.eps_out;
+        p.live_W = d.W; p.live_H = d.H;
         if (d.C != m.C || plan.tensors[m.y].C != m.C) throw std::runtime_error("plan: MLP width mismatch");
         return p;
     }
@@ -888,7 +932,8 @@
                 gp.out = group_ptr(tensors[plan.in_tensor], grp); gp.slots = gp0.slots + (size_t)first[grp]; gp.B = first[grp + 1] - first[grp];
                 gather(gp, gs);
             };
-            auto network_group = [&](int grp, hipStream_t gs) { run_network((uint8_t*)slab_out + (size_t)first[grp] * slot_bytes, first[grp + 1] - first[grp], grp, gs); };
+            const LiveExt* const ext0 = d_live && slots_off + (size_t)(bi + 1) * B <= live_stride ? d_live + slots_off + (size_t)bi * B : nullptr;
+            auto network_group = [&](int grp, hipStream_t gs) { run_network((uint8_t*)slab_out + (size_t)first[grp] * slot_bytes, first[grp + 1] - first[grp], grp, gs, ext0 ? ext0 + first[grp] : nullptr); };
             auto fork = [&] { hipAssert(hipEventRecord(ev_fork, stream)); for (int grp = 1; grp < NG; ++grp) hipAssert(hipStreamWaitEvent(gstream[grp - 1], ev_fork, 0)); };
             auto join = [&] { for (int grp = 1; grp < NG; ++grp) { hipAssert(hipEventRecord(ev_join[grp - 1], gstream[grp - 1])); hipAssert(hipStreamWaitEvent(stream, ev_join[grp - 1], 0)); } };
             auto run_pass = [&] {
@@ -896,7 +941,7 @@
                     stamp_begin(3, 0);
                     gather(gp0, stream);
                     stamp_end();
-                    run_network(slab_out, live);
+                    run_network(slab_out, live, -1, nullptr, ext0);
                     return;
                 }
                 ng_now = NG;
@@ -1043,6 +1088,7 @@
         }
         ensure(d_slots, slots_cap, (size_t)stepCount * sizeof(TileSlot));
         hipAssert(hipMemcpyAsync(d_slots, h_slots.data(), (size_t)stepCount * sizeof(TileSlot), hipMemcpyHostToDevice, stream));
+        upload_live(grid, (size_t)stepCount, stream);
         ensure(d_slab, slab_cap, (size_t)stepCount * plan.Tout * plan.Tout * 4 * plan.elt);
         hipAssert(hipStreamSynchronize(stream));
     }
@@ -1417,6 +1463,7 @@
     }
     impl->ensure(impl->d_slots, impl->slots_cap, stepTotal * sizeof(TileSlot));
     hipAssert(hipMemcpyAsync(impl->d_slots, impl->h_slots.data(), stepTotal * sizeof(TileSlot), hipMemcpyHostToDevice, stream));
+    impl->upload_live(grid, stepTotal, stream);
     const size_t one_part_steps = (size_t)(((int)std::lround(std::ceil((double)(sp.tile_count * steps) / plan.userB)) + S - 1) / S) * B;
     impl->ensure(impl->d_slab, impl->slab_cap, std::max((size_t)first_of[npart - 1] * steps + (stepTotal - slots_off[npart - 1]), one_part_steps) * plan.Tout * plan.Tout * 4 * plan.elt);
 
@@ -1516,6 +1563,7 @@
     }
     e.ensure(e.d_slots, e.slots_cap, (size_t)stepCount * sizeof(TileSlot));
     hipAssert(hipMemcpyAsync(e.d_slots, e.h_slots.data(), (size_t)stepCount * sizeof(TileSlot), hipMemcpyHostToDevice, e.stream));
+    e.upload_live(grid, (size_t)stepCount, e.stream);
     e.shard_halo_slots = (size_t)(sp.first_tile - sp.halo_first) * steps;
     e.ensure(e.d_slab, e.slab_cap, (e.shard_halo_slots + (size_t)stepCount) * slot_bytes);
     hipAssert(hipEventRecord(e.ev0, e.stream));
@@ -1902,6 +1950,7 @@
     }
     impl->ensure(impl->d_slots, impl->slots_cap, stepTotal * sizeof(TileSlot));
     hipAssert(hipMemcpyAsync(impl->d_slots, impl->h_slots.data(), stepTotal * sizeof(TileSlot), hipMemcpyHostToDevice, stream));
+    impl->upload_live(grid, stepTotal, stream);
     impl->ensure(impl->d_slab, impl->slab_cap, stepTotal * plan.Tout * plan.Tout * 4 * plan.elt);
     impl->one_part_stale = false;
     hipAssert(hipEventRecord(impl->ev0, stream));
diff --git a/waifu2x-tensorrt_amd/csrc/k_mlp2.hip b/waifu2x-tensorrt_amd/csrc/k_mlp2.hip
--- a/waifu2x-tensorrt_amd/csrc/k_mlp2.hip
+++ b/waifu2x-tensorrt_amd/csrc/k_mlp2.hip
@@ -139,6 +139,10 @@
     _Float16* Xw = (_Float16*)(smem + wv * K::SLAB);
     unsigned char* const WBb = smem + (K::KEEP ? K::NWV * K::SLAB : 0);
 
+    if (p.live) {
+        const long g0 = (long)blockIdx.x * K::BM, left = p.M - g0;
+        if (!live_rows(p.live, p.live_row0 + g0, left < K::BM ? (int)left : K::BM, p.live_W, p.live_H)) return;
+    }
     const long row0 = ((long)blockIdx.x * K::NWV + wv) * RW;
     const long nrows = p.M - row0 < RW ? p.M - row0 : RW;
     const unsigned xbytes = (unsigned)(p.M * (C * 2));
@@ -621,6 +625,7 @@
         q.M = p.M - r0 < max_rows ? p.M - r0 : max_rows;
         q.x = (const char*)p.x + (size_t)r0 * C * 2; q.y = (char*)p.y + (size_t)r0 * C * 2;
         if (p.stats_out) q.stats_out = p.stats_out + 2 * r0;
+        q.live_row0 = p.live_row0 + r0;
         dim3 grid((unsigned)((q.M + K::BM - 1) / K::BM));
         hipLaunchKernelGGL((mlp2_kernel<C, TT, NW>), grid, dim3(K::NWV * 64), K::SMEM, s, q);
         if (hipError_t e = hipGetLastError(); e != hipSuccess) return e;
diff --git a/waifu2x-tensorrt_amd/csrc/k_mlp96q.hip b/waifu2x-tensorrt_amd/csrc/k_mlp96q.hip
--- a/waifu2x-tensorrt_amd/csrc/k_mlp96q.hip
+++ b/waifu2x-tensorrt_amd/csrc/k_mlp96q.hip
@@ -164,22 +164,34 @@
 #define W2X_FETCH(TILE) { const unsigned vo = (unsigned)((W2X_MLP_EXP & 1) ? ((TILE) & 63) : (TILE)) * TILE_BYTES + lane * 16u;   \
         _Pragma("unroll") for (int k = 0; k < NP; ++k) xr[k] = __builtin_bit_cast(half8, __builtin_amdgcn_raw_buffer_load_b128(XB, vo + k * 1024u, 0, W2X_LD_LAST_AUX)); }
     constexpr bool DYN = W2X_MLP96_DYN && !TOIMG;
+    auto tile_live = [&](int tl) -> bool {
+        if (!p.live || tl >= ntiles) return true;
+        const long r0 = (long)tl * RW, left = p.M - r0;
+        return live_rows(p.live, p.live_row0 + r0, left < RW ? (int)left : RW, p.live_W, p.live_H);
+    };
     auto grab = [&]() -> int {
-        int t = 0;
-        if (lane == 0) t = atomicAdd((int*)(smem + CTR_OFF), 1);
-        t = __builtin_amdgcn_readfirstlane(t);
-        const int tl = (blockIdx.x + (t / NWV) * (int)gridDim.x) * NWV + t % NWV;
+        int tl;
+        do {
+            int t = 0;
+            if (lane == 0) t = atomicAdd((int*)(smem + CTR_OFF), 1);
+            t = __builtin_amdgcn_readfirstlane(t);
+            tl = (blockIdx.x + (t / NWV) * (int)gridDim.x) * NWV + t % NWV;
+        } while (!tile_live(tl));
+        return tl < ntiles ? tl : ntiles;
+    };
+    auto stride_from = [&](int tl) -> int {
+        while (!tile_live(tl)) tl += nw;
         return tl < ntiles ? tl : ntiles;
     };
     int tile = gw, next_tile = ntiles;
-    if constexpr (DYN) tile = grab();
+    if constexpr (DYN) tile = grab(); else tile = stride_from(gw);
     if (tile < ntiles) W2X_FETCH(tile)
 #if W2X_MLP_PREFETCH
 #pragma unroll
     for (int k = 0; k < NP; ++k) __builtin_amdgcn_raw_buffer_store_b128(uint4v{}, YB, 0xFFFFF000u + k * 16u, 0, 0);
 #endif
 #pragma unroll 1
-    for (; tile < ntiles; tile = DYN ? next_tile : tile + nw) {
+    for (; tile < ntiles; tile = (DYN || W2X_MLP_PREFETCH) ? next_tile : stride_from(tile + nw)) {
         const long row0 = (long)((W2X_MLP_EXP & 1) ? (tile & 63) : tile) * RW;
         const long nrows = p.M - row0 < RW ? p.M - row0 : RW;
 #if !W2X_MLP_PREFETCH
@@ -241,7 +253,8 @@
             }
 #if W2X_MLP_PREFETCH
             if (ch == W2X_MLP_PFCH) {
-                if constexpr (DYN) { next_tile = grab(); W2X_FETCH(next_tile) } else { W2X_FETCH(tile + nw) }
+                if constexpr (DYN) next_tile = grab(); else next_tile = stride_from(tile + nw);
+                W2X_FETCH(next_tile)
                 W2X_RING_FENCE();
             }
 #endif
@@ -408,6 +421,7 @@
         q.M = std::min(max_rows, p.M - r0);
         q.x = (const char*)p.x + (size_t)r0 * C * 2; q.y = (char*)p.y + (size_t)r0 * C * 2;
         if (p.stats_out) q.stats_out = p.stats_out + 2 * r0;
+        q.live_row0 = p.live_row0 + r0;
         const long ntiles = (q.M + RW - 1) / RW;
         const int grid = (int)std::min<long>((ntiles + NWV - 1) / NWV, ncu);
         if ((ntiles + (long)grid * NWV) * (long)(RW * C * 2) > 0xFFFFFFFFl) return hipErrorInvalidValue;
diff --git a/waifu2x-tensorrt_amd/csrc/k_swinattn192u.hip b/waifu2x-tensorrt_amd/csrc/k_swinattn192u.hip
--- a/waifu2x-tensorrt_amd/csrc/k_swinattn192u.hip
+++ b/waifu2x-tensorrt_amd/csrc/k_swinattn192u.hip
@@ -110,13 +110,20 @@
     const int fr = lane & 15, g = lane >> 4;
 
     const int iw0 = blockIdx.x * G, iw1 = iw0 + 1, itotal = p.B * p.nwin;
-    const bool wok0 = iw0 < itotal, wok1 = iw1 < itotal;
+    bool wok0 = iw0 < itotal, wok1 = iw1 < itotal;
     const int HW = p.nwin * NTOK;
     const int wb0 = iw0 / p.nwin, wb1 = iw1 / p.nwin;
     const int pixbase0 = wb0 * HW, pixbase1 = wb1 * HW;
     const int wl0 = iw0 - wb0 * p.nwin, wl1 = iw1 - wb1 * p.nwin;
     const int nwx = p.W / 6;
     const int wy0 = wl0 / nwx, wx0 = wl0 - wy0 * nwx, wy1 = wl1 / nwx, wx1 = wl1 - wy1 * nwx;
+    if (p.live && p.ry >= 0) {
+        int y0 = wy0 * 6 + p.ry, x0 = wx0 * 6 + p.rx, y1 = wy1 * 6 + p.ry, x1 = wx1 * 6 + p.rx;
+        y0 -= y0 >= p.H ? p.H : 0; x0 -= x0 >= p.W ? p.W : 0; y1 -= y1 >= p.H ? p.H : 0; x1 -= x1 >= p.W ? p.W : 0;
+        wok0 = wok0 && live_token(live_ext_load(p.live, wb0), x0, y0, p.W, p.H);
+        wok1 = wok1 && live_token(live_ext_load(p.live, wb1), x1, y1, p.W, p.H);
+        if (!wok0 && !wok1) return;
+    }
     const unsigned xbytes = (unsigned)p.B * (unsigned)HW * (C * 2);
     const __amdgpu_buffer_rsrc_t X = make_rsrc(p.x, xbytes), Y = make_rsrc(p.y, xbytes);
     const _Float16* __restrict__ Wqkv = (const _Float16*)p.wqkv_frag;
@@ -455,6 +462,7 @@
         q.x = (const char*)p.x + (size_t)b0 * img_bytes;
         q.y = (char*)p.y + (size_t)b0 * img_bytes;
         if (p.stats_out) q.stats_out = p.stats_out + (size_t)b0 * p.nwin * NTOK * 2;
+        if (p.live) q.live = p.live + b0;
         const long total_win = (long)q.B * q.nwin;
         hipLaunchKernelGGL(kern, dim3((unsigned)((total_win + G - 1) / G)), dim3(256), SMEM192U, s, q);
         if (hipError_t e = hipGetLastError(); e != hipSuccess) return e;
diff --git a/waifu2x-tensorrt_amd/csrc/k_swinattn96.hip b/waifu2x-tensorrt_amd/csrc/k_swinattn96.hip
--- a/waifu2x-tensorrt_amd/csrc/k_swinattn96.hip
+++ b/waifu2x-tensorrt_amd/csrc/k_swinattn96.hip
@@ -145,6 +145,17 @@
 
     const int wl0 = blockIdx.x * G;
     const int HW = p.nwin * NTOK;
+    bool lv0 = true, lv1 = wl0 + 1 < p.nwin;
+    if (p.live && p.ry >= 0) {
+        const LiveExt e = live_ext_load(p.live, (int)blockIdx.y);
+        const int nwx = p.W / 6, wy = wl0 / nwx, wx = wl0 - wy * nwx;
+        const int wy1 = wx + 1 == nwx ? wy + 1 : wy, wx1 = wx + 1 == nwx ? 0 : wx + 1;
+        int y0 = wy * 6 + p.ry, x0 = wx * 6 + p.rx, y1 = wy1 * 6 + p.ry, x1 = wx1 * 6 + p.rx;
+        y0 -= y0 >= p.H ? p.H : 0; x0 -= x0 >= p.W ? p.W : 0; y1 -= y1 >= p.H ? p.H : 0; x1 -= x1 >= p.W ? p.W : 0;
+        lv0 = live_token(e, x0, y0, p.W, p.H);
+        lv1 = lv1 && live_token(e, x1, y1, p.W, p.H);
+        if (!lv0 && !lv1) return;
+    }
     const unsigned xbytes = (unsigned)p.B * (unsigned)HW * (C * 2);
     const __amdgpu_buffer_rsrc_t X = make_rsrc(p.x, xbytes), Y = make_rsrc(p.y, xbytes);
     const _Float16* __restrict__ Wqkv = (const _Float16*)p.wqkv_frag;
@@ -178,7 +189,7 @@
             const int w = tid >= NTOK ? 1 : 0, t = tid - w * NTOK;
             const int wl = wl0 + w;
             srow = (w * SLAB + slab_row(t)) * LDX * 2;
-            if (wl < p.nwin) {
+            if (w ? lv1 : lv0) {
                 if (p.ry >= 0) {
                     const int nwx = p.W / 6;
                     const int wy = (int)(((float)wl + 0.5f) * __builtin_amdgcn_rcpf((float)nwx)), wx = wl - wy * nwx;
@@ -413,6 +424,7 @@
         q.x = (const char*)p.x + (size_t)b0 * img_bytes;
         q.y = (char*)p.y + (size_t)b0 * img_bytes;
         if (p.stats_out) q.stats_out = p.stats_out + (size_t)b0 * p.nwin * NTOK * 2;
+        if (p.live) q.live = p.live + b0;
         hipLaunchKernelGGL(swin_attn96_kernel, dim3((unsigned)((q.nwin + G - 1) / G), (unsigned)q.B), dim3(NTHR), SMEM96, s, q);
         if (hipError_t e = hipGetLastError(); e != hipSuccess) return e;
     }
diff --git a/waifu2x-tensorrt_amd/csrc/kernels.h b/waifu2x-tensorrt_amd/csrc/kernels.h
--- a/waifu2x-tensorrt_amd/csrc/kernels.h
+++ b/waifu2x-tensorrt_amd/csrc/kernels.h
@@ -33,6 +33,30 @@
 #else
     *p = v;
 #endif
+}
+#endif
+
+struct LiveExt { uint16_t cx, wx, cy, wy; };
+#ifdef __HIPCC__
+__device__ __forceinline__ LiveExt live_ext_load(const LiveExt* t, int slot) {
+    typedef const unsigned long long __attribute__((address_space(4)))* cptr;
+    const unsigned long long v = ((cptr)(unsigned long long)t)[slot];
+    return LiveExt{(uint16_t)v, (uint16_t)(v >> 16), (uint16_t)(v >> 32), (uint16_t)(v >> 48)};
+}
+__device__ __forceinline__ bool live_token(const LiveExt e, int x, int y, int W, int H) { return (x < e.cx || x >= W - e.wx) && (y < e.cy || y >= H - e.wy); }
+__device__ __forceinline__ bool live_rows(const LiveExt* t, long r0, int n, int W, int H) {
+    const int HW = W * H;
+    if (n > HW) return true;
+    const int img = (int)(r0 / HW);
+    int r = (int)(r0 - (long)img * HW);
+    LiveExt e = live_ext_load(t, img);
+    for (int left = n; left > 0;) {
+        if (r >= HW) { r -= HW; e = live_ext_load(t, img + 1); }
+        const int y = r / W, x0 = r - y * W, x1 = x0 + left < W ? x0 + left : W;
+        if ((y < e.cy || y >= H - e.wy) && (x0 < e.cx || x1 > W - e.wx)) return true;
+        left -= x1 - x0; r += x1 - x0;
+    }
+    return false;
 }
 #endif
 
@@ -90,6 +114,8 @@
     void* ti_out = nullptr; int ti_Hs = 0, ti_Ws = 0, ti_Mrows = 0, ti_aW = 0;
     int ti_clip = 0; float ti_lo = 0.f, ti_hi = 0.f;
     long ti_row0 = 0;
+    const LiveExt* live = nullptr; int live_W = 0, live_H = 0;
+    long live_row0 = 0;
 };
 
 struct SwinAttnParams {
@@ -107,6 +133,7 @@
     float eps = 1e-5f;
     float* stats_out = nullptr; float eps_out = 1e-5f;
     const void* wqkv_frag = nullptr; const void* wproj_frag = nullptr;
+    const LiveExt* live = nullptr;
 };
 
 struct SeParams {
diff --git a/waifu2x-tensorrt_amd/csrc/liveness.cpp b/waifu2x-tensorrt_amd/csrc/liveness.cpp
--- /dev/null
+++ b/waifu2x-tensorrt_amd/csrc/liveness.cpp
@@ -0,0 +1,142 @@
+#include "liveness.h"
+
+#include <algorithm>
+
+namespace w2x {
+
+namespace {
+
+using Axis = std::vector<char>;
+
+Axis expand(const AxisExt& e) {
+    Axis a(e.n, 0);
+    for (int i = 0; i < e.n; ++i) a[i] = i < e.c || i >= e.n - e.w;
+    return a;
+}
+AxisExt to_ext(const Axis& a) {
+    const int n = (int)a.size();
+    AxisExt e; e.n = n;
+    while (e.c < n && a[e.c]) ++e.c;
+    if (e.c == n) return e;
+    while (e.w < n - e.c && a[n - 1 - e.w]) ++e.w;
+    for (int i = e.c; i < n - e.w; ++i) if (a[i]) { e.c = n; e.w = 0; break; }
+    return e;
+}
+int count(const AxisExt& e) { return e.c >= e.n ? e.n : e.c + e.w; }
+int live_windows(const AxisExt& e, int r, int ws) {
+    int k = 0;
+    for (int i = 0; i < e.n / ws; ++i) { const int t = (ws * i + r) % e.n; k += t < e.c || t >= e.n - e.w; }
+    return k;
+}
+void unite(Axis& into, const Axis& a) {
+    if (into.empty()) { into = a; return; }
+    for (size_t i = 0; i < into.size() && i < a.size(); ++i) into[i] |= a[i];
+}
+
+struct Unsupported {};
+
+}
+
+long OpExtent::live_units() const { return ws > 0 ? (long)live_windows(x, rx, ws) * live_windows(y, ry, ws) : (long)count(x) * count(y); }
+long OpExtent::total_units() const { return ws > 0 ? (long)(x.n / ws) * (y.n / ws) : (long)x.n * y.n; }
+
+std::vector<OpExtent> dead_skip_extents(const Plan& plan, int kept_w, int kept_h, bool force_all) {
+    const int nops = (int)plan.ops.size(), nt = (int)plan.tensors.size();
+    std::vector<OpExtent> ext(nops);
+    auto row_map = [&](const Op& op, int& W, int& H) {
+        W = H = 0;
+        if (op.kind == OP_GEMM) { W = op.g.aW; H = op.g.aW > 0 ? op.g.Mrows / op.g.aW : 0; }
+        else if (op.kind == OP_MLP && op.m.x >= 0 && op.m.x < nt) { W = plan.tensors[op.m.x].W; H = plan.tensors[op.m.x].H; }
+        else if (op.kind == OP_SWINATTN) { W = op.sa.W; H = op.sa.H; }
+    };
+    auto set_all = [&] {
+        for (int i = 0; i < nops; ++i) {
+            int W, H; row_map(plan.ops[i], W, H);
+            OpExtent e; e.x = AxisExt{W, W, 0}; e.y = AxisExt{H, H, 0};
+            if (plan.ops[i].kind == OP_SWINATTN) { e.ry = plan.ops[i].sa.ry; e.rx = plan.ops[i].sa.rx; e.ws = plan.ops[i].sa.ws; }
+            ext[i] = e;
+        }
+    };
+    set_all();
+    if (force_all || nops == 0 || plan.elt != 2 || plan.out_tensor < 0 || plan.out_tensor >= nt) return ext;
+    if (kept_w >= plan.Tout && kept_h >= plan.Tout) return ext;
+    if (kept_w <= 0 || kept_h <= 0) return ext;
+    try {
+        std::vector<Axis> nx(nt), ny(nt);
+        auto whole = [&](const View& v) { if (v.t < 0 || v.t >= nt) throw Unsupported{}; const TensorDesc& d = plan.tensors[v.t]; return v.y0 == 0 && v.x0 == 0 && v.H == d.H && v.W == d.W; };
+        auto need = [&](int t, const Axis& ax, const Axis& ay) {
+            if (t < 0 || t >= nt || (int)ax.size() != plan.tensors[t].W || (int)ay.size() != plan.tensors[t].H) throw Unsupported{};
+            unite(nx[t], ax); unite(ny[t], ay);
+        };
+        {
+            const TensorDesc& d = plan.tensors[plan.out_tensor];
+            if (d.W != plan.Tout || d.H != plan.Tout) throw Unsupported{};
+            Axis ax(d.W, 0), ay(d.H, 0);
+            for (int i = 0; i < std::min(kept_w, d.W); ++i) ax[i] = 1;
+            for (int i = 0; i < std::min(kept_h, d.H); ++i) ay[i] = 1;
+            need(plan.out_tensor, ax, ay);
+        }
+        for (int i = nops - 1; i >= 0; --i) {
+            const Op& op = plan.ops[i];
+            int W, H; row_map(op, W, H);
+            if (W <= 0 || H <= 0) throw Unsupported{};
+            OpExtent e; Axis rx_, ry_;
+            if (op.kind == OP_GEMM) {
+                const GemmOp& g = op.g;
+                if (g.ln || g.stats_in >= 0 || g.stats_out >= 0 || g.pool_out >= 0 || g.se_scale >= 0 || g.res_scale >= 0 || g.res2.t >= 0 || g.amode == A_WIN || g.omode == O_WIN ||
+                    (long)W * H != g.Mrows || !whole(g.out)) throw Unsupported{};
+                const int r = g.omode == O_PIXSHUF ? g.r : 1;
+                if (r < 1 || g.out.W != W * r || g.out.H != H * r) throw Unsupported{};
+                const Axis& ox = nx[g.out.t]; const Axis& oy = ny[g.out.t];
+                if (ox.empty() || oy.empty()) throw Unsupported{};
+                rx_.assign(W, 0); ry_.assign(H, 0);
+                for (int k = 0; k < W * r; ++k) if (ox[k]) rx_[k / r] = 1;
+                for (int k = 0; k < H * r; ++k) if (oy[k]) ry_[k / r] = 1;
+                e.x = to_ext(rx_); e.y = to_ext(ry_);
+                rx_ = expand(e.x); ry_ = expand(e.y);
+                if (g.res.t >= 0) {
+                    if (!whole(g.res) || g.res.W != W * r || g.res.H != H * r) throw Unsupported{};
+                    Axis ax(W * r), ay(H * r);
+                    for (int k = 0; k < W * r; ++k) ax[k] = rx_[k / r];
+                    for (int k = 0; k < H * r; ++k) ay[k] = ry_[k / r];
+                    need(g.res.t, ax, ay);
+                }
+                const int s = g.amode == A_CONV ? g.stride : 1, kw = g.amode == A_CONV ? g.kw : 1, kh = g.amode == A_CONV ? g.kh : 1;
+                if (g.a.t < 0 || g.a.t >= nt || s < 1 || kw < 1 || kh < 1) throw Unsupported{};
+                const TensorDesc& d = plan.tensors[g.a.t];
+                if (g.a.x0 < 0 || g.a.y0 < 0 || g.a.x0 + (W - 1) * s + kw > d.W || g.a.y0 + (H - 1) * s + kh > d.H) throw Unsupported{};
+                Axis ax(d.W, 0), ay(d.H, 0);
+                for (int k = 0; k < W; ++k) if (rx_[k]) for (int j = 0; j < kw; ++j) ax[g.a.x0 + s * k + j] = 1;
+                for (int k = 0; k < H; ++k) if (ry_[k]) for (int j = 0; j < kh; ++j) ay[g.a.y0 + s * k + j] = 1;
+                need(g.a.t, ax, ay);
+            } else if (op.kind == OP_MLP) {
+                const MlpOp& m = op.m;
+                if (m.stats_out >= 0 || m.y < 0 || m.y >= nt || plan.tensors[m.y].W != W || plan.tensors[m.y].H != H || nx[m.y].empty()) throw Unsupported{};
+                e.x = to_ext(nx[m.y]); e.y = to_ext(ny[m.y]);
+                need(m.x, expand(e.x), expand(e.y));
+            } else if (op.kind == OP_SWINATTN) {
+                const SwinAttnOp& a = op.sa;
+                if (a.stats_out >= 0 || a.ry < 0 || a.rx < 0 || a.ws <= 0 || W % a.ws || H % a.ws || a.y < 0 || a.y >= nt || plan.tensors[a.y].W != W || plan.tensors[a.y].H != H ||
+                    a.x < 0 || a.x >= nt || plan.tensors[a.x].W != W || plan.tensors[a.x].H != H || nx[a.y].empty()) throw Unsupported{};
+                auto windows = [&](const Axis& o, int n, int roll) {
+                    Axis out(n, 0);
+                    for (int k = 0; k < n / a.ws; ++k) {
+                        bool any = false;
+                        for (int j = 0; j < a.ws; ++j) any = any || o[(a.ws * k + j + roll) % n];
+                        if (any) for (int j = 0; j < a.ws; ++j) out[(a.ws * k + j + roll) % n] = 1;
+                    }
+                    return out;
+                };
+                e.x = to_ext(windows(nx[a.y], W, a.rx)); e.y = to_ext(windows(ny[a.y], H, a.ry));
+                e.ry = a.ry; e.rx = a.rx; e.ws = a.ws;
+                need(a.x, expand(e.x), expand(e.y));
+            } else throw Unsupported{};
+            ext[i] = e;
+        }
+    } catch (const Unsupported&) {
+        set_all();
+    }
+    return ext;
+}
+
+}
diff --git a/waifu2x-tensorrt_amd/csrc/liveness.h b/waifu2x-tensorrt_amd/csrc/liveness.h
--- /dev/null
+++ b/waifu2x-tensorrt_amd/csrc/liveness.h
@@ -0,0 +1,19 @@
+#pragma once
+#include <vector>
+
+#include "plan.h"
+
+namespace w2x {
+
+struct AxisExt { int n = 0, c = 0, w = 0; };
+struct OpExtent {
+    AxisExt x, y;
+    int ry = -1, rx = -1, ws = 0;
+    bool all() const { return x.c >= x.n && y.c >= y.n; }
+    long live_units() const;
+    long total_units() const;
+};
+
+std::vector<OpExtent> dead_skip_extents(const Plan& plan, int kept_w, int kept_h, bool force_all = false);
+
+}
diff --git a/waifu2x-tensorrt_amd/csrc/support.cpp b/waifu2x-tensorrt_amd/csrc/support.cpp
--- a/waifu2x-tensorrt_amd/csrc/support.cpp
+++ b/waifu2x-tensorrt_amd/csrc/support.cpp
@@ -46,6 +46,7 @@
     {"no_conv48", nullptr, &Switches::no_conv48, nullptr, 0, 1},
     {"no_stem", nullptr, &Switches::no_stem, nullptr, 0, 1},
     {"attn_valu", nullptr, &Switches::attn_valu, nullptr, 0, 1},
+    {"no_dead_skip", nullptr, &Switches::no_dead_skip, nullptr, 0, 1},
 };
 void assign(Switches& s, const Field& f, long v) {
     v = std::min<long>(f.hi, std::max<long>(f.lo, v));
diff --git a/waifu2x-tensorrt_amd/csrc/switches.h b/waifu2x-tensorrt_amd/csrc/switches.h
--- a/waifu2x-tensorrt_amd/csrc/switches.h
+++ b/waifu2x-tensorrt_amd/csrc/switches.h
@@ -21,6 +21,7 @@
     bool no_conv3h_walk = false;
     bool no_pixgemm = false, no_conv3 = false, no_conv3h = false, no_conv48 = false, no_stem = false;
     bool attn_valu = false;
+    bool no_dead_skip = false;
 };
 
 Switches& switches();
diff --git a/waifu2x-tensorrt_amd/engine.py b/waifu2x-tensorrt_amd/engine.py
--- a/waifu2x-tensorrt_amd/engine.py
+++ b/waifu2x-tensorrt_amd/engine.py
@@ -179,6 +179,7 @@
     L.w2x_sha256_hex.argtypes = [vp, C.c_size_t, C.c_char_p]
     L.w2x_version.restype = C.c_char_p
     L.w2x_debug_set.argtypes = [C.c_char_p, C.c_int]; L.w2x_debug_set.restype = C.c_int
+    L.w2x_dead_skip_extents.argtypes = [C.c_char_p] + [C.c_int] * 5 + [C.c_double, C.c_double, C.c_int, C.c_int, vp, C.c_int]; L.w2x_dead_skip_extents.restype = C.c_int
     _lib = L
     return L
 
@@ -188,7 +189,7 @@
     "w2x_render", "w2x_render16", "w2x_infer", "w2x_output_tile_size", "w2x_plan_flops", "w2x_pass_tiles", "w2x_last_render_ms", "w2x_bench_resident", "w2x_resident_output", "w2x_profile_frame", "w2x_op_times",
     "w2x_render_resized", "w2x_render16_resized", "w2x_render_sequence_resized", "w2x_resize_weights",
     "w2x_render_yuv", "w2x_render_sequence_yuv", "w2x_yuv_plane_sizes", "w2x_render_yuv_resized", "w2x_render_sequence_yuv_resized",
-    "w2x_render_rgba", "w2x_alpha_bleed_device", "w2x_alpha_bleed",
+    "w2x_render_rgba", "w2x_alpha_bleed_device", "w2x_alpha_bleed", "w2x_dead_skip_extents",
     "w2x_render_strip", "w2x_strip_plan", "w2x_render_sharded", "w2x_shard_plan", "w2x_shard_compute", "w2x_shard_slab", "w2x_shard_finish", "w2x_ipc_export", "w2x_ipc_open", "w2x_ipc_close", "w2x_render_sequence", "w2x_alloc_host", "w2x_free_host", "w2x_pin_host", "w2x_unpin_host", "w2x_calculate_tiles", "w2x_tile_weights", "w2x_describe_plan", "w2x_describe_plan_precision", "w2x_write_engine_file", "w2x_validate_engine_file", "w2x_device_pci_bus_id", "w2x_sha256_hex", "w2x_version", "w2x_debug_set"]
 
 
@@ -721,6 +722,21 @@
     return s
 
 
+EXTENT_FIELDS = ("kind", "W", "H", "cx", "wx", "cy", "wy", "rx", "ry", "ws", "t_in", "t_out", "t_res", "kh", "kw", "stride", "x0", "y0", "r",
+                 "in_W", "in_H", "out_W", "out_H", "live_units", "total_units")
+
+
+def dead_skip_extents(onnx_path, batch, tile, in_w, in_h, scaling, overlap, tile_index, tta=False) -> list[dict]:
+    L = lib()
+    n = -L.w2x_dead_skip_extents(os.fsencode(onnx_path), batch, tile, in_w, in_h, scaling, float(overlap[0]), float(overlap[1]), int(tile_index), int(bool(tta)), None, 0)
+    if n <= 0:
+        raise W2xError("w2x_dead_skip_extents failed")
+    out = np.zeros((n, len(EXTENT_FIELDS)), np.int32)
+    if L.w2x_dead_skip_extents(os.fsencode(onnx_path), batch, tile, in_w, in_h, scaling, float(overlap[0]), float(overlap[1]), int(tile_index), int(bool(tta)), out.ctypes.data, out.size) != n:
+        raise W2xError("w2x_dead_skip_extents failed")
+    return [dict(zip(EXTENT_FIELDS, (int(v) for v in row))) for row in out]
+
+
 def write_engine_file(onnx_path, batch, tile, out_path) -> bool:
     return bool(lib().w2x_write_engine_file(os.fsencode(onnx_path), batch, tile, os.fsencode(out_path)))
 
```

Measured after the change: 4575 MPix/s (median of 6 runs). 2.2% higher.
